# skamann/mcmc-dynamics

Hardware: AMD Instinct MI355X
Metric: star-walker log-L terms/sec (higher is better)
Workload: dtype f64; 1 GPU; C3: 1e6 synthetic stars x 256 walkers, rotation+dispersion + fixed single-Gaussian background mixture (ConstantFit + background.Gaussian), fixed centre; stars_per_gpu=1000000, stars_total=1000000, walkers=256, likelihood=bgfixed, parallelism=1 GPU

## Files before the change

### include/mcd.h

```cpp
#ifndef MCD_H
#define MCD_H

#include <stdint.h>

#ifdef __cplusplus
extern "C" {
#endif

#define MCD_ABI_VERSION 1
#define MCD_UNIQUE_ID_BYTES 128

typedef struct mcd_ctx mcd_ctx;
typedef struct mcd_catalog mcd_catalog;

typedef enum {
    MCD_OK = 0,
    MCD_ERR_INVALID = -1,
    MCD_ERR_HIP = -2,
    MCD_ERR_RCCL = -3,
    MCD_ERR_NO_DEVICE = -4,
    MCD_ERR_NONFINITE = -5,
    MCD_ERR_NOMEM = -6
} mcd_status;

// ... 104 lines not shown
int mcd_stretch_move_seeded(mcd_catalog* cat, const mcd_stretch_desc* desc, int64_t n_steps, double* pos, double* lnp,
                            uint64_t seed, int64_t step0, double* chain, double* lnprob_chain, int64_t* accepted);
int mcd_chain_numbers(uint64_t seed, int64_t step0, int64_t n_steps, int64_t n_bins, int64_t n_walkers, int32_t n_dim,
                      int32_t* order, double* zz, double* thr, int32_t* pick);

int mcd_stretch_info(const mcd_catalog* cat, int64_t* device_blocks, int64_t* host_blocks, int64_t* discarded_blocks,
                     int32_t* last_discard_status);

typedef struct {
    int32_t n_dim;
    const int32_t* kind;
    const double* p0;
    const double* p1;
} mcd_prior_desc;

int mcd_prior_eval(const mcd_prior_desc* prior, int64_t n_rows, const double* x, double* value, double* grad);
int mcd_stretch_move_prior(mcd_catalog* cat, const mcd_stretch_desc* desc, int64_t n_steps, double* pos, double* lnp,
                           const int32_t* order, const double* zz, const double* thr, const int32_t* pick, double* chain,
                           double* lnprob_chain, int64_t* accepted, const mcd_prior_desc* prior);
int mcd_stretch_move_seeded_prior(mcd_catalog* cat, const mcd_stretch_desc* desc, int64_t n_steps, double* pos, double* lnp,
                                  uint64_t seed, int64_t step0, double* chain, double* lnprob_chain, int64_t* accepted,
                                  const mcd_prior_desc* prior);

typedef struct {
    mcd_stretch_desc map;
    const double* chol;
    double step_size;
    double jitter;
    int32_t n_leap;
} mcd_hmc_desc;

int mcd_hmc_block(mcd_catalog* cat, const mcd_hmc_desc* desc, int64_t n_steps, double* pos, double* lnp, uint64_t seed,
                  int64_t step0, double* chain, double* lnprob_chain, int64_t* accepted, double* energy_error);
int mcd_hmc_block_prior(mcd_catalog* cat, const mcd_hmc_desc* desc, int64_t n_steps, double* pos, double* lnp, uint64_t seed,
                        int64_t step0, double* chain, double* lnprob_chain, int64_t* accepted, double* energy_error,
                        const mcd_prior_desc* prior);
int mcd_hmc_numbers(uint64_t seed, int64_t step0, int64_t n_steps, int64_t n_walkers, int32_t n_dim, double* z, double* thr,
                    double* eps_factor);
int mcd_hmc_info(const mcd_catalog* cat, int64_t* device_blocks, int64_t* host_blocks);

typedef struct {
    mcd_stretch_desc map;
    int32_t n_temps;
    const double* betas;
    int32_t n_chain_temps;
} mcd_temper_desc;

int mcd_temper_block(mcd_catalog* cat, const mcd_temper_desc* desc, int64_t n_steps, double* pos, double* lnlike,
                     double* lnprior, uint64_t seed, int64_t step0, double* chain, double* lnlike_chain, int64_t* accepted,
                     int64_t* swap_proposed, int64_t* swap_accepted);
int mcd_temper_block_prior(mcd_catalog* cat, const mcd_temper_desc* desc, int64_t n_steps, double* pos, double* lnlike,
                           double* lnprior, uint64_t seed, int64_t step0, double* chain, double* lnlike_chain,
                           int64_t* accepted, int64_t* swap_proposed, int64_t* swap_accepted,
                           const mcd_prior_desc* prior);
int mcd_temper_numbers(uint64_t seed, int64_t step0, int64_t n_steps, int32_t n_temps, int64_t n_walkers, double* swap_thr);
int mcd_temper_info(const mcd_catalog* cat, int64_t* device_blocks, int64_t* host_blocks);


typedef struct {
    int64_t n_steps, n_groups, n_walkers;
    int32_t n_dim;
    int64_t max_lag;
    double c;
    int64_t scratch_mb;
} mcd_diag_desc;

int mcd_chain_diagnostics(mcd_ctx* ctx, const mcd_diag_desc* d, const double* chain, double* tau, int64_t* window,
                          int32_t* found, double* rhat, double* mean, double* var, double* rho);
int mcd_chain_diagnostics_info(int64_t* tile_groups, int64_t* n_tiles, double* kernel_ms);


const char* mcd_last_error(void);
int mcd_abi_version(void);
double mcd_last_kernel_ms(const mcd_catalog* cat);
double mcd_last_device_ms(const mcd_catalog* cat);
int mcd_set_option(mcd_catalog* cat, const char* key, int64_t value);
int mcd_timing_collect(mcd_catalog* cat, double* total_kernel_ms, int64_t* n_launches);
int64_t mcd_rerun_count(const mcd_catalog* cat);
int mcd_last_prefetch(const mcd_catalog* cat);
int mcd_last_narrow_bounded(const mcd_catalog* cat);
int64_t mcd_last_series_chunks(const mcd_catalog* cat);
int64_t mcd_last_direct_chunks(const mcd_catalog* cat);
int mcd_last_exp_split(const mcd_catalog* cat);
int mcd_last_fast_level(const mcd_catalog* cat);

int mcd_last_f32_domain(const mcd_catalog* cat, double* kappa_v, double* kappa_theta);
int mcd_last_launch_info(const mcd_catalog* cat, int64_t* n_workgroups, int32_t* walker_tile,
                         int64_t* n_chunks, int32_t* record_bytes);

#ifdef __cplusplus
}
#endif
#endif
```

### mcmc_dynamics_amd/_native.py

```python
import atexit
import ctypes
import os
import weakref

import numpy as np

_HERE = os.path.dirname(os.path.abspath(__file__))
LIB_PATH = os.environ.get("MCD_LIB_PATH") or os.path.join(_HERE, "libmcd_hip.so")

MODEL_CONST, MODEL_CONST_BGFIXED, MODEL_CONST_BGGAUSS = 0, 1, 2
MODEL_PROFILE, MODEL_PROFILE_BGGAUSS, MODEL_PROFILE_BGDENS, MODEL_PROFILE_BGFIXED = 3, 4, 5, 6
CENTRE_FIXED, CENTRE_FREE = 0, 1
F64, F32, F32_ACC64 = 0, 1, 2
PRECISIONS = {"f64": F64, "f32": F32, "f32acc64": F32_ACC64}
UNIQUE_ID_BYTES = 128

_c_double_p = ctypes.POINTER(ctypes.c_double)
_c_int64_p = ctypes.POINTER(ctypes.c_int64)

SYMBOLS = {
    "mcd_ctx_create": (ctypes.c_int, [ctypes.c_int, ctypes.POINTER(ctypes.c_int), ctypes.POINTER(ctypes.c_void_p)]),
    "mcd_get_unique_id": (ctypes.c_int, [ctypes.c_void_p]),
    "mcd_ctx_create_rank": (ctypes.c_int, [ctypes.c_int, ctypes.c_int, ctypes.c_int, ctypes.c_void_p,
                                           ctypes.POINTER(ctypes.c_void_p)]),
    "mcd_ctx_destroy": (ctypes.c_int, [ctypes.c_void_p]),
    "mcd_ctx_set_option": (ctypes.c_int, [ctypes.c_void_p, ctypes.c_char_p, ctypes.c_int64]),
    "mcd_ctx_abort": (ctypes.c_int, [ctypes.c_void_p, ctypes.c_char_p]),
    "mcd_ctx_failed": (ctypes.c_int, [ctypes.c_void_p]),
    "mcd_ctx_n_devices": (ctypes.c_int, [ctypes.c_void_p]),
    "mcd_ctx_comm_info": (ctypes.c_int, [ctypes.c_void_p, ctypes.POINTER(ctypes.c_int), ctypes.POINTER(ctypes.c_int),
                                         ctypes.POINTER(ctypes.c_int)]),
    "mcd_catalog_create": (ctypes.c_int, [ctypes.c_void_p, ctypes.c_void_p, ctypes.POINTER(ctypes.c_void_p)]),
    "mcd_catalog_destroy": (ctypes.c_int, [ctypes.c_void_p]),
    "mcd_catalog_param_count": (ctypes.c_int, [ctypes.c_void_p]),
    "mcd_catalog_n_stars": (ctypes.c_int64, [ctypes.c_void_p]),
    "mcd_catalog_n_outputs": (ctypes.c_int64, [ctypes.c_void_p, ctypes.c_int64]),
    "mcd_loglike_batch": (ctypes.c_int, [ctypes.c_void_p, ctypes.c_int64, ctypes.c_int32, _c_double_p, _c_double_p]),
    "mcd_loglike_grad_batch": (ctypes.c_int, [ctypes.c_void_p, ctypes.c_int64, ctypes.c_int32, _c_double_p, _c_double_p,
                                              _c_double_p]),
    "mcd_params_upload": (ctypes.c_int, [ctypes.c_void_p, ctypes.c_int64, ctypes.c_int32, _c_double_p]),
    "mcd_loglike_enqueue": (ctypes.c_int, [ctypes.c_void_p]),
    "mcd_loglike_fetch": (ctypes.c_int, [ctypes.c_void_p, _c_double_p]),
    "mcd_sync": (ctypes.c_int, [ctypes.c_void_p]),
    "mcd_membership": (ctypes.c_int, [ctypes.c_void_p, ctypes.c_int32, _c_double_p, _c_double_p]),
    "mcd_loglike_per_star": (ctypes.c_int, [ctypes.c_void_p, ctypes.c_int32, _c_double_p, _c_double_p]),
    "mcd_pointwise_posterior": (ctypes.c_int, [ctypes.c_void_p, ctypes.c_int64, ctypes.c_int32, _c_double_p, _c_double_p,
                                               _c_double_p, _c_double_p, _c_double_p]),
    "mcd_psis_loo": (ctypes.c_int, [ctypes.c_void_p, ctypes.c_int64, ctypes.c_int32, _c_double_p, ctypes.c_double,
                                    _c_double_p, _c_double_p, _c_double_p, _c_double_p]),
    "mcd_posterior_predictive": (ctypes.c_int, [ctypes.c_void_p, ctypes.c_int64, ctypes.c_int32, _c_double_p, _c_double_p,
                                                _c_double_p]),
    "mcd_kde_background": (ctypes.c_int, [ctypes.c_void_p, ctypes.c_int64, _c_double_p, ctypes.c_int64, _c_double_p,
                                          _c_double_p, ctypes.c_double, _c_double_p, _c_double_p]),
    "mcd_stretch_move": (ctypes.c_int, [ctypes.c_void_p, ctypes.c_void_p, ctypes.c_int64, _c_double_p, _c_double_p,
                                        ctypes.POINTER(ctypes.c_int32), _c_double_p, _c_double_p,
                                        ctypes.POINTER(ctypes.c_int32), _c_double_p, _c_double_p, _c_int64_p]),
    "mcd_stretch_move_seeded": (ctypes.c_int, [ctypes.c_void_p, ctypes.c_void_p, ctypes.c_int64, _c_double_p, _c_double_p,
                                               ctypes.c_uint64, ctypes.c_int64, _c_double_p, _c_double_p, _c_int64_p]),
    "mcd_chain_numbers": (ctypes.c_int, [ctypes.c_uint64, ctypes.c_int64, ctypes.c_int64, ctypes.c_int64, ctypes.c_int64,
                                         ctypes.c_int32, ctypes.POINTER(ctypes.c_int32), _c_double_p, _c_double_p,
                                         ctypes.POINTER(ctypes.c_int32)]),
    "mcd_stretch_info": (ctypes.c_int, [ctypes.c_void_p, _c_int64_p, _c_int64_p, _c_int64_p, ctypes.POINTER(ctypes.c_int32)]),
    "mcd_hmc_block": (ctypes.c_int, [ctypes.c_void_p, ctypes.c_void_p, ctypes.c_int64, _c_double_p, _c_double_p,
                                     ctypes.c_uint64, ctypes.c_int64, _c_double_p, _c_double_p, _c_int64_p, _c_double_p]),
    "mcd_hmc_numbers": (ctypes.c_int, [ctypes.c_uint64, ctypes.c_int64, ctypes.c_int64, ctypes.c_int64, ctypes.c_int32,
                                       _c_double_p, _c_double_p, _c_double_p]),
    "mcd_hmc_info": (ctypes.c_int, [ctypes.c_void_p, _c_int64_p, _c_int64_p]),
    "mcd_prior_eval": (ctypes.c_int, [ctypes.c_void_p, ctypes.c_int64, _c_double_p, _c_double_p, _c_double_p]),
    "mcd_stretch_move_prior": (ctypes.c_int, [ctypes.c_void_p, ctypes.c_void_p, ctypes.c_int64, _c_double_p, _c_double_p,
                                              ctypes.POINTER(ctypes.c_int32), _c_double_p, _c_double_p,
                                              ctypes.POINTER(ctypes.c_int32), _c_double_p, _c_double_p, _c_int64_p,
                                              ctypes.c_void_p]),
    "mcd_stretch_move_seeded_prior": (ctypes.c_int, [ctypes.c_void_p, ctypes.c_void_p, ctypes.c_int64, _c_double_p,
                                                     _c_double_p, ctypes.c_uint64, ctypes.c_int64, _c_double_p, _c_double_p,
                                                     _c_int64_p, ctypes.c_void_p]),
    "mcd_hmc_block_prior": (ctypes.c_int, [ctypes.c_void_p, ctypes.c_void_p, ctypes.c_int64, _c_double_p, _c_double_p,
                                           ctypes.c_uint64, ctypes.c_int64, _c_double_p, _c_double_p, _c_int64_p, _c_double_p,
                                           ctypes.c_void_p]),
    "mcd_temper_block": (ctypes.c_int, [ctypes.c_void_p, ctypes.c_void_p, ctypes.c_int64, _c_double_p, _c_double_p, _c_double_p,
                                        ctypes.c_uint64, ctypes.c_int64, _c_double_p, _c_double_p, _c_int64_p, _c_int64_p,
                                        _c_int64_p]),
    "mcd_temper_block_prior": (ctypes.c_int, [ctypes.c_void_p, ctypes.c_void_p, ctypes.c_int64, _c_double_p, _c_double_p,
                                              _c_double_p, ctypes.c_uint64, ctypes.c_int64, _c_double_p, _c_double_p,
                                              _c_int64_p, _c_int64_p, _c_int64_p, ctypes.c_void_p]),
    "mcd_temper_numbers": (ctypes.c_int, [ctypes.c_uint64, ctypes.c_int64, ctypes.c_int64, ctypes.c_int32, ctypes.c_int64,
                                          _c_double_p]),
    "mcd_temper_info": (ctypes.c_int, [ctypes.c_void_p, _c_int64_p, _c_int64_p]),
    "mcd_chain_diagnostics": (ctypes.c_int, [ctypes.c_void_p, ctypes.c_void_p, _c_double_p, _c_double_p, _c_int64_p,
                                             ctypes.POINTER(ctypes.c_int32), _c_double_p, _c_double_p, _c_double_p,
                                             _c_double_p]),
    "mcd_chain_diagnostics_info": (ctypes.c_int, [_c_int64_p, _c_int64_p, _c_double_p]),
    "mcd_last_error": (ctypes.c_char_p, []),
    "mcd_abi_version": (ctypes.c_int, []),
    "mcd_last_kernel_ms": (ctypes.c_double, [ctypes.c_void_p]),
    "mcd_last_device_ms": (ctypes.c_double, [ctypes.c_void_p]),
    "mcd_timing_collect": (ctypes.c_int, [ctypes.c_void_p, _c_double_p, _c_int64_p]),
    "mcd_rerun_count": (ctypes.c_int64, [ctypes.c_void_p]),
    "mcd_last_prefetch": (ctypes.c_int, [ctypes.c_void_p]),
    "mcd_last_narrow_bounded": (ctypes.c_int, [ctypes.c_void_p]),
    "mcd_last_series_chunks": (ctypes.c_int64, [ctypes.c_void_p]),
    "mcd_last_direct_chunks": (ctypes.c_int64, [ctypes.c_void_p]),
    "mcd_last_exp_split": (ctypes.c_int, [ctypes.c_void_p]),
    "mcd_last_fast_level": (ctypes.c_int, [ctypes.c_void_p]),
    "mcd_last_f32_domain": (ctypes.c_int, [ctypes.c_void_p, _c_double_p, _c_double_p]),
    "mcd_set_option": (ctypes.c_int, [ctypes.c_void_p, ctypes.c_char_p, ctypes.c_int64]),
    "mcd_last_launch_info": (ctypes.c_int, [ctypes.c_void_p, _c_int64_p, ctypes.POINTER(ctypes.c_int32), _c_int64_p,
                                            ctypes.POINTER(ctypes.c_int32)]),
}


class NativeError(RuntimeError):
    """Raised when the HIP library is missing, fails to load, or a call returns an error status."""


class CatalogDesc(ctypes.Structure):
    _fields_ = [
        ("n_stars", ctypes.c_int64),
        ("ra", _c_double_p), ("dec", _c_double_p), ("v", _c_double_p), ("verr", _c_double_p),
        ("lnlike_bg", _c_double_p), ("pmember", _c_double_p), ("density", _c_double_p),
        ("model", ctypes.c_int32), ("centre", ctypes.c_int32), ("precision", ctypes.c_int32),
        ("reserved", ctypes.c_int32),
        ("ra_center", ctypes.c_double), ("dec_center", ctypes.c_double),
        ("n_bins", ctypes.c_int64), ("bin_offsets", _c_int64_p),
    ]


class StretchDesc(ctypes.Structure):
    _fields_ = [
        ("n_walkers", ctypes.c_int64), ("n_dim", ctypes.c_int32), ("k", ctypes.c_int32),
        ("col_source", ctypes.POINTER(ctypes.c_int32)), ("col_const", _c_double_p), ("col_factor", _c_double_p),
        ("lo", _c_double_p), ("hi", _c_double_p), ("fixed_ok", ctypes.c_int32), ("n_bins", ctypes.c_int32),
    ]


class PriorDesc(ctypes.Structure):
    _fields_ = [("n_dim", ctypes.c_int32), ("kind", ctypes.POINTER(ctypes.c_int32)), ("p0", _c_double_p), ("p1", _c_double_p)]


PRIOR_FLAT, PRIOR_NORMAL, PRIOR_LOGNORMAL = 0, 1, 2


def _prior_desc(prior):
    kind = np.ascontiguousarray(prior[0], dtype=np.int32)
    p0, p1 = _f64(prior[1]), _f64(prior[2])
    if kind.ndim != 1 or p0.shape != kind.shape or p1.shape != kind.shape:
        raise ValueError("a prior is three arrays of one length: kind, p0, p1")
    d = PriorDesc()
    d.n_dim = kind.size
    d.kind, d.p0, d.p1 = kind.ctypes.data_as(ctypes.POINTER(ctypes.c_int32)), _ptr(p0), _ptr(p1)
    return d, (kind, p0, p1)


def prior_eval(prior, x, want_grad=False):
    lib = load_library()
    x = _f64(np.atleast_2d(x))
    d, _keep = _prior_desc(prior)
    if x.shape[1] != d.n_dim:
        raise ValueError("prior_eval: x must have shape (n, {0})".format(d.n_dim))
    value = np.empty(x.shape[0])
    grad = np.empty(x.shape) if want_grad else None
    _check(lib, lib.mcd_prior_eval(ctypes.byref(d), x.shape[0], _ptr(x), _ptr(value), _ptr(grad)), "mcd_prior_eval")
    return (value, grad) if want_grad else value


class DiagDesc(ctypes.Structure):
    _fields_ = [("n_steps", ctypes.c_int64), ("n_groups", ctypes.c_int64), ("n_walkers", ctypes.c_int64),
                ("n_dim", ctypes.c_int32), ("max_lag", ctypes.c_int64), ("c", ctypes.c_double), ("scratch_mb", ctypes.c_int64)]


def chain_diagnostics(chain, max_lag, c=5.0, context=None, scratch_mb=0, want_rho=False):
    lib = load_library()
    chain = _f64(chain)
    if chain.ndim != 4:
        raise ValueError("chain_diagnostics: chain must have shape (steps, groups, walkers, parameters)")
    T, G, W, P = chain.shape
    d = DiagDesc(T, G, W, P, int(max_lag), float(c), int(scratch_mb))
    out = {"tau": np.empty((G, P)), "window": np.empty((G, P), dtype=np.int64), "found": np.empty((G, P), dtype=np.int32),
           "rhat": np.empty((G, P)), "mean": np.empty((G, P)), "var": np.empty((G, P))}
    if want_rho:
        out["rho"] = np.empty((G, P, max(int(max_lag), 0) + 1))
    handle = None
    if context is not None:
        handle = getattr(context, "handle", None)
        if not handle:
            raise NativeError("context is closed")
# ... 380 lines not shown
        return out

    def _stretch_args(self, name, plan, pos, lnp, n_steps, chain, lnprob_chain, accepted):
        self._alive()
        for a in (pos, lnp):
            if a.dtype != np.float64 or not a.flags.c_contiguous:
                raise ValueError(name + " needs C-contiguous arrays of the documented dtypes")
        if pos.ndim not in (2, 3) or lnp.shape != pos.shape[:-1]:
            raise ValueError(name + ": inconsistent array shapes")
        lead, (w, p) = pos.shape[:-2], pos.shape[-2:]
        cols = [np.ascontiguousarray(plan["col_source"], dtype=np.int32), _f64(plan["col_const"]), _f64(plan["col_factor"]),
                _f64(plan["lo"]), _f64(plan["hi"])]
        if cols[0].size != self.k or cols[1].size != self.k or cols[2].size != self.k or cols[3].size != p or cols[4].size != p:
            raise ValueError("stretch_move: plan does not match the catalogue / the number of free parameters")
        d = StretchDesc()
        d.n_walkers, d.n_dim, d.k, d.n_bins = w, p, self.k, lead[0] if lead else 1
        d.col_source = cols[0].ctypes.data_as(ctypes.POINTER(ctypes.c_int32))
        d.col_const, d.col_factor, d.lo, d.hi = (_ptr(c) for c in cols[1:])
        d.fixed_ok = 1 if plan.get("fixed_ok", True) else 0
        for a, shape in ((chain, (n_steps,) + lead + (w, p)), (lnprob_chain, (n_steps,) + lead + (w,))):
            if a is not None and (a.dtype != np.float64 or not a.flags.c_contiguous or a.shape != shape):
                raise ValueError("stretch_move: chain buffers must be C-contiguous float64 of shape (steps, [B,] W, P) / (steps, [B,] W)")
        if accepted is not None and (accepted.dtype != np.int64 or accepted.shape != lead + (w,) or not accepted.flags.c_contiguous):
            raise ValueError("stretch_move: accepted must be a C-contiguous int64 array of shape ([B,] W)")
        self._prior_arg = None
        if "prior" in plan:
            pd = None
            if plan["prior"] is not None:
                pd, keep = _prior_desc(plan["prior"])
                cols.append(keep)
            self._prior_arg = (ctypes.byref(pd) if pd is not None else None,)
        return ((self.handle, ctypes.byref(d), n_steps, _ptr(pos), _ptr(lnp)),
                (_ptr(chain), _ptr(lnprob_chain), accepted.ctypes.data_as(_c_int64_p) if accepted is not None else None), cols)

    def stretch_move(self, plan, pos, lnp, order, zz, thr, pick, chain=None, lnprob_chain=None, accepted=None):
        head, tail, _keep = self._stretch_args("stretch_move", plan, pos, lnp, order.shape[0], chain, lnprob_chain, accepted)
        for a, dt in ((zz, np.float64), (thr, np.float64), (order, np.int32), (pick, np.int32)):
            if a.dtype != dt or not a.flags.c_contiguous:
                raise ValueError("stretch_move needs C-contiguous arrays of the documented dtypes")
        half_shape = (order.shape[0], 2) + pos.shape[:-2] + (pos.shape[-2] // 2,)
        if order.shape != order.shape[:1] + lnp.shape or zz.shape != half_shape or thr.shape != half_shape or \
                pick.shape != half_shape:
            raise ValueError("stretch_move: inconsistent array shapes")
        numbers = (order.ctypes.data_as(ctypes.POINTER(ctypes.c_int32)), _ptr(zz), _ptr(thr),
                   pick.ctypes.data_as(ctypes.POINTER(ctypes.c_int32)))
        if self._prior_arg is not None:
            rc = self.lib.mcd_stretch_move_prior(*head, *numbers, *tail, *self._prior_arg)
        else:
            rc = self.lib.mcd_stretch_move(*head, *numbers, *tail)
        _check(self.lib, rc, "mcd_stretch_move")
        self._walkers = pos.shape[-2] // 2

    def stretch_move_seeded(self, plan, pos, lnp, seed, step0, n_steps, chain=None, lnprob_chain=None, accepted=None):
        if n_steps < 0 or step0 < 0:
            raise ValueError("stretch_move_seeded: inconsistent array shapes")
        head, tail, _keep = self._stretch_args("stretch_move_seeded", plan, pos, lnp, n_steps, chain, lnprob_chain, accepted)
        if self._prior_arg is not None:
            rc = self.lib.mcd_stretch_move_seeded_prior(*head, int(seed) & 0xFFFFFFFFFFFFFFFF, int(step0), *tail, *self._prior_arg)
        else:
            rc = self.lib.mcd_stretch_move_seeded(*head, int(seed) & 0xFFFFFFFFFFFFFFFF, int(step0), *tail)
        _check(self.lib, rc, "mcd_stretch_move_seeded")
        self._walkers = pos.shape[-2] // 2

    @property
    def last_prefetch(self):
        return self.lib.mcd_last_prefetch(self.handle)

    @property
    def last_narrow_bounded(self):
        return self.lib.mcd_last_narrow_bounded(self.handle)

    @property
    def last_series_chunks(self):
        return self.lib.mcd_last_series_chunks(self.handle)

    @property
    def last_direct_chunks(self):
        return self.lib.mcd_last_direct_chunks(self.handle)

    @property
    def last_exp_split(self):
        return self.lib.mcd_last_exp_split(self.handle)

    def hmc_block(self, plan, chol, step_size, n_leap, pos, lnp, seed, step0, n_steps, chain=None, lnprob_chain=None,
                  accepted=None, energy_error=None, jitter=0.1):
        if n_steps < 0 or step0 < 0 or pos.ndim != 2:
            raise ValueError("hmc_block: inconsistent array shapes")
        head, tail, _keep = self._stretch_args("hmc_block", plan, pos, lnp, n_steps, chain, lnprob_chain, accepted)
        chol = np.ascontiguousarray(chol, dtype=np.float64)
        if chol.shape != (pos.shape[1], pos.shape[1]):
            raise ValueError("hmc_block: chol must have shape (P, P)")
        if energy_error is not None and (energy_error.dtype != np.float64 or not energy_error.flags.c_contiguous or
                                         energy_error.shape != (n_steps, pos.shape[0])):
            raise ValueError("hmc_block: energy_error must be a C-contiguous float64 array of shape (steps, W)")
        d = HmcDesc()
        d.map = head[1]._obj
        d.chol, d.step_size, d.jitter, d.n_leap = _ptr(chol), float(step_size), float(jitter), int(n_leap)
        if self._prior_arg is not None:
            rc = self.lib.mcd_hmc_block_prior(self.handle, ctypes.byref(d), int(n_steps), head[3], head[4],
                                              int(seed) & 0xFFFFFFFFFFFFFFFF, int(step0), *tail, _ptr(energy_error),
                                              *self._prior_arg)
        else:
            rc = self.lib.mcd_hmc_block(self.handle, ctypes.byref(d), int(n_steps), head[3], head[4],
                                        int(seed) & 0xFFFFFFFFFFFFFFFF, int(step0), *tail, _ptr(energy_error))
        _check(self.lib, rc, "mcd_hmc_block")

    def hmc_info(self):
        a, b = ctypes.c_int64(), ctypes.c_int64()
        _check(self.lib, self.lib.mcd_hmc_info(self.handle, ctypes.byref(a), ctypes.byref(b)), "mcd_hmc_info")
        return {"device_blocks": a.value, "host_blocks": b.value}

    def temper_block(self, plan, betas, pos, lnlike, lnprior, seed, step0, n_steps, chain=None, lnlike_chain=None,
                     accepted=None, swap_proposed=None, swap_accepted=None):
        if n_steps < 0 or step0 < 0 or pos.ndim != 3 or lnlike.shape != pos.shape[:2] or lnprior.shape != pos.shape[:2]:
            raise ValueError("temper_block: inconsistent array shapes")
        t, w, p = pos.shape
        betas = _f64(betas)
        if betas.shape != (t,):
            raise ValueError("temper_block: betas must have one entry per rung")
        if lnprior.dtype != np.float64 or not lnprior.flags.c_contiguous or not pos.flags.c_contiguous or \
                not lnlike.flags.c_contiguous:
            raise ValueError("temper_block needs C-contiguous arrays of the documented dtypes")
        head, _tail, _keep = self._stretch_args("temper_block", plan, pos[0], lnlike[0], n_steps, None, None, None)
        n_chain = 1
        if chain is not None:
            if chain.dtype != np.float64 or not chain.flags.c_contiguous or chain.ndim != 4 or \
                    chain.shape[0] != n_steps or chain.shape[2:] != (w, p):
                raise ValueError("temper_block: chain must be a C-contiguous float64 array of shape (steps, C, W, P)")
            n_chain = chain.shape[1]
        if lnlike_chain is not None and (lnlike_chain.dtype != np.float64 or not lnlike_chain.flags.c_contiguous or
                                         lnlike_chain.shape != (n_steps, t, w)):
            raise ValueError("temper_block: lnlike_chain must be a C-contiguous float64 array of shape (steps, T, W)")
        for a, shape in ((accepted, (t, w)), (swap_proposed, (t - 1,)), (swap_accepted, (t - 1,))):
            if a is not None and (a.dtype != np.int64 or a.shape != shape or not a.flags.c_contiguous):
                raise ValueError("temper_block: accepted (T, W) and the swap counts (T - 1,) are C-contiguous int64 arrays")
        d = TemperDesc()
        d.map = head[1]._obj
        d.n_temps, d.betas, d.n_chain_temps = t, _ptr(betas), n_chain

        def ip(a):
            return a.ctypes.data_as(_c_int64_p) if a is not None else None
        args = (self.handle, ctypes.byref(d), int(n_steps), _ptr(pos), _ptr(lnlike), _ptr(lnprior),
                int(seed) & 0xFFFFFFFFFFFFFFFF, int(step0), _ptr(chain), _ptr(lnlike_chain), ip(accepted), ip(swap_proposed),
                ip(swap_accepted))
        if self._prior_arg is not None:
            rc = self.lib.mcd_temper_block_prior(*args, *self._prior_arg)
        else:
            rc = self.lib.mcd_temper_block(*args)
        _check(self.lib, rc, "mcd_temper_block")
        self._walkers = t * (w // 2)

    def temper_info(self):
        a, b = ctypes.c_int64(), ctypes.c_int64()
        _check(self.lib, self.lib.mcd_temper_info(self.handle, ctypes.byref(a), ctypes.byref(b)), "mcd_temper_info")
        return {"device_blocks": a.value, "host_blocks": b.value}

    def stretch_info(self):
        a, b, c, st = ctypes.c_int64(), ctypes.c_int64(), ctypes.c_int64(), ctypes.c_int32()
        _check(self.lib, self.lib.mcd_stretch_info(self.handle, ctypes.byref(a), ctypes.byref(b), ctypes.byref(c), ctypes.byref(st)),
               "mcd_stretch_info")
        return {"device_blocks": a.value, "host_blocks": b.value, "discarded_blocks": c.value, "last_discard_status": st.value}

    def set_option(self, key, value):
        _check(self.lib, self.lib.mcd_set_option(self.handle, key.encode(), int(value)), "mcd_set_option")
        self.__dict__.setdefault("_options", {})[key] = int(value)

    def get_option(self, key, default=None):
        return self.__dict__.get("_options", {}).get(key, default)

    @property
    def last_kernel_ms(self):
        return self.lib.mcd_last_kernel_ms(self.handle)

    @property
    def last_device_ms(self):
        return self.lib.mcd_last_device_ms(self.handle)

    def timing_collect(self):
        total, n = ctypes.c_double(), ctypes.c_int64()
        _check(self.lib, self.lib.mcd_timing_collect(self.handle, ctypes.byref(total), ctypes.byref(n)),
               "mcd_timing_collect")
        return total.value, n.value

    @property
    def rerun_count(self):
        return self.lib.mcd_rerun_count(self.handle)

    @property
    def fast_level(self):
        return self.lib.mcd_last_fast_level(self.handle)

    @property
    def f32_in_domain(self):
        return bool(self.lib.mcd_last_f32_domain(self.handle, None, None))

    @property
    def f32_condition(self):
        kv, kt = ctypes.c_double(), ctypes.c_double()
        self.lib.mcd_last_f32_domain(self.handle, ctypes.byref(kv), ctypes.byref(kt))
        return kv.value, kt.value

    def launch_info(self):
        wg, ch = ctypes.c_int64(), ctypes.c_int64()
        tile, rb = ctypes.c_int32(), ctypes.c_int32()
        _check(self.lib, self.lib.mcd_last_launch_info(self.handle, ctypes.byref(wg), ctypes.byref(tile),
                                                       ctypes.byref(ch), ctypes.byref(rb)), "mcd_last_launch_info")
        return {"workgroups": wg.value, "walker_tile": tile.value, "chunks": ch.value, "record_bytes": rb.value,
                "series_chunks": self.last_series_chunks, "direct_chunks": self.last_direct_chunks,
                "exp_split": self.last_exp_split}

    def close(self):
        if getattr(self, "handle", None):
            self.lib.mcd_catalog_destroy(self.handle)
            self.handle = None

    def __del__(self):
        try:
            self.close()
        except Exception:
            pass
```

### mcmc_dynamics_amd/csrc/mcd_api_catalog.hip

```cpp
#include "mcd_host.h"

using namespace mcd::host;

namespace {

int param_count(int model, bool free_centre) {
    int k = (mcd::is_profile(model) ? 6 : 4) + (free_centre ? 2 : 0);
    const int bg = mcd::bg_kind(model);
    if (bg == mcd::BG_GAUSS) k += 3;
    if (bg == mcd::BG_FIXED_DENSITY) k += 1;
    return k;
}

void free_workset(WorkSet& w) {
    if (w.d_chunks) (void)hipFree(w.d_chunks);
    if (w.d_offsets) (void)hipFree(w.d_offsets);
    if (w.d_chunk_general) (void)hipFree(w.d_chunk_general);
    if (w.d_split_const) (void)hipFree(w.d_split_const);
    if (w.d_params) (void)hipFree(w.d_params);
    if (w.d_wpar) (void)hipFree(w.d_wpar);
    if (w.d_partials) (void)hipFree(w.d_partials);
    if (w.d_out) (void)hipFree(w.d_out);
    if (w.d_out2) (void)hipFree(w.d_out2);
    if (w.d_partials2) (void)hipFree(w.d_partials2);
// ... 17 lines not shown
int balance_auto_m(const mcd_catalog* cat, int64_t n, int64_t n_walkers) {
    const int64_t n_wtiles = (n_walkers + 63) / 64;
    const double tiles = n_wtiles <= 4 ? (double)n_wtiles : 4.0 * (double)((n_wtiles + 3) / 4);
    const double work = (double)n * tiles / 4.0 * model_cost(cat->model, cat->free_centre);
    const double limit = mcd::bg_kind(cat->model) == mcd::BG_NONE ? 9.0e5 : 1.3e6;
    if (cat->n_psets != 1 || work > limit) return 0;
    return work < 6.0e4 ? 2 : (work <= 3.4e5 ? 4 : 8);
}

bool wants_prefetch(const mcd_catalog* cat, const Shard& sh) {
    if (cat->prefetch >= 0) return cat->prefetch != 0;
    const size_t bytes = (size_t)sh.n * (size_t)mcd::record_bytes(cat->model, cat->free_centre, cat->precision);
    if (mcd::bg_kind(cat->model) == mcd::BG_NONE) return cat->n_psets == 1 && bytes >= ((size_t)128 << 20);
    return bytes >= ((size_t)8 << 20);
}

bool wants_sorted(const mcd_catalog* cat, const Shard& sh) {
    if (cat->model != mcd::MODEL_BGFIXED || cat->free_centre || cat->precision != MCD_F64 || cat->n_psets != 1 || sh.n <= 0)
        return false;
    if (cat->verr_sorted >= 0) return cat->verr_sorted != 0;
    if (cat->chunk_len > 0) return false;
    return (size_t)sh.n * (size_t)mcd::record_bytes(cat->model, cat->free_centre, cat->precision) >= ((size_t)8 << 20);
}

int ensure_sorted_records(mcd_catalog* cat, Shard& sh) {
    if (sh.records_sorted) return MCD_OK;
    const DeviceSlot& slot = cat->ctx->slots[sh.slot];
    constexpr int ND = mcd::record_doubles(mcd::MODEL_BGFIXED, false);
    const size_t n = (size_t)sh.n, bytes = n * ND * sizeof(double);
    MCD_HIP(hipStreamSynchronize(slot.stream));
    std::vector<double> rec(n * ND), out(n * ND);
    MCD_HIP(hipMemcpy(rec.data(), sh.records, bytes, hipMemcpyDeviceToHost));
    const std::vector<int64_t> perm = mcd::verr_order(rec.data(), (int64_t)n, ND);
    sh.sorted_e2.resize(n);
    for (size_t i = 0; i < n; ++i) {
        std::memcpy(&out[i * ND], &rec[(size_t)perm[i] * ND], ND * sizeof(double));
        sh.sorted_e2[i] = out[i * ND + 1];
    }
    sh.sorted_exceptions = mcd::permuted_exceptions(cat->stats.narrow_exceptions, perm, sh.star_begin);
    sh.sorted_nbf.resize(n);
    mcd::exp_split_records(out.data(), (int64_t)n, rec.data(), sh.sorted_nbf.data());
    void* d[2] = {nullptr, nullptr};
    const double* src[2] = {out.data(), rec.data()};
    for (int a = 0; a < 2; ++a) {
        hipError_t e = hipMalloc(&d[a], bytes + 2048);
        if (e == hipSuccess) e = hipMemset(d[a], 0, bytes + 2048);
        if (e == hipSuccess) e = hipMemcpy(d[a], src[a], bytes, hipMemcpyHostToDevice);
        if (e != hipSuccess) {
            for (int b = 0; b <= a; ++b)
                if (d[b]) (void)hipFree(d[b]);
            MCD_HIP(e);
        }
    }
    sh.records_sorted = d[0];
    sh.records_split = d[1];
    return MCD_OK;
}

struct Option {
    const char* key;
    int64_t min, max;
    const char* message;
    bool sync, replan;
    void (*set)(mcd_catalog* c, int64_t v);
    bool (*accepts)(int64_t v) = nullptr;
};
constexpr int64_t kMin = std::numeric_limits<int64_t>::min(), kMax = std::numeric_limits<int64_t>::max();
#define MCD_SET(statement) [](mcd_catalog* c, int64_t v) { statement; }
const Option kOptions[] = {
    {"fast_path", 0, 2, "fast_path: 0 (plain), 1 (guarded, default) or 2 (guarded, no narrow variant)", false, false, MCD_SET(c->allow_fast = (int)v)},
    {"zero_copy", kMin, kMax, nullptr, false, false, MCD_SET(c->zero_copy = v != 0)},
    {"device_chain", 0, 2, "device_chain: 0 (host-driven blocks), 1 (default) or 2 (as 1 with the general step kernel, testing aid)", false, false,
     MCD_SET(c->device_chain = (int)v; c->chain_backoff = 0; c->chain_consecutive = 0; c->chain_hint = -1)},
    {"fused_reduce", kMin, kMax, nullptr, false, false, MCD_SET(c->fused_reduce = v != 0)},
    {"defer_guard", kMin, kMax, nullptr, false, false, MCD_SET(c->defer_guard = v != 0)},
    {"f32_domain", kMin, kMax, nullptr, false, false, MCD_SET(c->f32_domain = v != 0)},
    {"loo_scratch_mb", 1, kMax, "loo_scratch_mb must be >= 1", false, false, MCD_SET(c->loo_scratch_mb = v)},
    {"posterior_pass", 1, kMax, "posterior_pass must be >= 1", false, false, MCD_SET(c->posterior_pass = v)},
    {"two_lanes", kMin, kMax, nullptr, true, false, MCD_SET(c->two_lanes = v != 0)},
    {"narrow_bounded", 0, 1, "narrow_bounded: 1 (where the guard admits it, default) or 0 (never)", false, false, MCD_SET(c->narrow_bounded = (int)v)},
    {"verr_sorted", -1, 1, "verr_sorted: -1 (by record volume, default), 0 (catalogue order) or 1 (sorted by verr)", true, true, MCD_SET(c->verr_sorted = (int)v)},
    {"root_series", 0, 1, "root_series: 1 (series root on the narrow chunks of verr-sorted records, default) or 0 (never)", false, false, MCD_SET(c->root_series = (int)v)},
    {"exp_split", 0, 1, "exp_split: 1 (split exponent offset in the direct chunks where the guard admits it, default) or 0 (never)", false, false, MCD_SET(c->exp_split = (int)v)},
    {"root_direct", 0, 1, "root_direct: 1 (direct form of the series root where a chunk admits it, default) or 0 (delta form only)", false, false, MCD_SET(c->root_direct = (int)v)},
    {"prefetch", -1, 1, "prefetch: -1 (by record volume, default), 0 (off) or 1 (on)", false, false, MCD_SET(c->prefetch = (int)v)},
    {"spin_us", 0, kMax, "spin_us must be >= 0", false, false, MCD_SET(c->spin_us = v)},
    {"tail_split", kMin, kMax, nullptr, true, true, MCD_SET(c->tail_split = (int)v)},
    {"target_waves", 1, kMax, "target_waves must be positive", true, true, MCD_SET(c->target_waves = v)},
    {"chunk_len", 0, kMax, "chunk_len must be >= 0", true, true, MCD_SET(c->chunk_len = v)},
    {"balance", -1, 8, "balance: -1 (auto), 0 (off) or 1 .. 8 workgroups per CU", true, true, MCD_SET(c->balance = (int)v)},
    {"combine", 0, 16, "combine: 0 (never), 1 (largest workgroup the plan allows), 8 or 16 (waves per workgroup at most)", true, true,
     MCD_SET(c->combine = (int)v), [](int64_t v) { return v <= 1 || v == 8 || v == 16; }},
};
#undef MCD_SET
}

MCD_HOST_BEGIN

LaunchShape main_launch_shape(mcd_catalog* cat, const Shard& sh, const WorkSet& w, int level, bool coll, double* out_buf,
                              int64_t n_out) {
    LaunchShape shape{cat->model, cat->free_centre, cat->precision, level, w.uniform_len, sh.n};
    shape.uniform_extra = w.uniform_extra;
    shape.waves = w.waves;
    shape.chunk_general = w.d_chunk_general;
    shape.prefetch = wants_prefetch(cat, sh);
    cat->last_prefetch = shape.prefetch && shape.fast != 0;
    shape.rerun_flag = coll ? nullptr : out_buf + n_out;
    shape.root_series = w.sorted && cat->root_series != 0;
    shape.root_direct = shape.root_series && cat->root_direct != 0;
    return shape;
}

const void* main_records(const Shard& sh, const WorkSet& w) { return w.sorted ? sh.records_sorted : sh.records; }

int64_t series_chunk_count(const mcd_catalog* cat, const WorkSet& w, int level, const double* params, int64_t n_rows) {
    if (!w.sorted || !cat->root_series || level != 2 || w.series_need.empty()) return 0;
    const mcd::ParamRanges pr = mcd::table_ranges(cat->model, cat->free_centre, cat->k, params, n_rows);
    if (!pr.finite) return 0;
    return (int64_t)(std::upper_bound(w.series_need.begin(), w.series_need.end(), pr.s2_min) - w.series_need.begin());
}

int64_t direct_chunk_count(const mcd_catalog* cat, const WorkSet& w, int level, const double* params, int64_t n_rows) {
    if (!w.sorted || !cat->root_series || !cat->root_direct || level != 2 || w.direct_need.empty()) return 0;
    const mcd::ParamRanges pr = mcd::table_ranges(cat->model, cat->free_centre, cat->k, params, n_rows);
    if (!pr.finite) return 0;
    return (int64_t)(std::upper_bound(w.direct_need.begin(), w.direct_need.end(), pr.s2_min) - w.direct_need.begin());
}

const double* fast_pset_const(const mcd_catalog* cat, const Shard& sh, int level) {
    const int bgk = mcd::bg_kind(cat->model);
    return (level && (bgk == mcd::BG_FIXED || bgk == mcd::BG_FIXED_DENSITY)) ? sh.d_pset_const : nullptr;
}

int build_workset(mcd_catalog* cat, Shard& sh, int64_t n_walkers, WorkSet** out) {
    auto it = sh.work.find(n_walkers);
    if (it != sh.work.end()) { *out = &it->second; return MCD_OK; }
    if (sh.work.size() >= 8) {
        for (auto& kv : sh.work) free_workset(kv.second);
        sh.work.clear();
        cat->cur_walkers = 0;
    }
    const DeviceSlot& slot = cat->ctx->slots[sh.slot];
    MCD_HIP(hipSetDevice(slot.device));

    const bool sorted = wants_sorted(cat, sh);
    if (sorted)
        if (int rc = ensure_sorted_records(cat, sh)) return rc;
    const std::vector<int64_t>& exceptions = sorted ? sh.sorted_exceptions : cat->stats.narrow_exceptions;
    mcd::ChunkPlan plan;
    for (int m = cat->balance < 0 ? balance_auto_m(cat, sh.n, n_walkers) : cat->balance;; m /= 2) {
        plan = mcd::plan_chunks(cat->bin_offsets, sh.star_begin, sh.n, n_walkers, cat->target_waves, cat->tail_split,
                                exceptions, cat->chunk_len, m);
        if (m == 0 || plan.balanced_m > 0) break;
    }
    const std::vector<mcd::Chunk>& chunks = plan.chunks;
    const std::vector<int64_t>& offs = plan.offsets;
    const std::vector<uint8_t>& general = plan.general;

    WorkSet w;
    w.n_walkers = n_walkers;
    w.n_chunks = (int64_t)chunks.size();
    w.max_chunks_per_pset = plan.max_chunks_per_pset;
    w.uniform_len = plan.uniform_len;
    w.uniform_extra = plan.uniform_extra;
    w.sorted = sorted;
    if (sorted) {
        w.series_need = mcd::series_thresholds(plan, sh.sorted_e2.data());
        w.direct_need = mcd::direct_thresholds(plan, sh.sorted_e2.data());
    }
    const std::vector<double> split_const = sorted ? mcd::exp_split_chunk_consts(plan, sh.sorted_nbf.data()) : std::vector<double>();
    {
        const int64_t n_wtiles = (n_walkers + 63) / 64;
        const bool shape_ok = plan.balanced_m > 0 && plan.balanced_m % 2 == 0 && (n_wtiles == 1 || n_wtiles == 2 || n_wtiles == 4) &&
                              cat->precision == MCD_F64;
        w.waves = 4;
        if (cat->combine != 0 && shape_ok) {
            const bool can16 = mcd::bg_kind(cat->model) != mcd::BG_GAUSS;
            w.waves = 8;
            if (cat->combine == 16 && plan.balanced_m % 4 == 0 && can16) w.waves = 16;
            if (cat->combine == 1 && plan.balanced_m == 4 && can16) w.waves = 16;
        }
    }
    const int64_t n_out = cat->n_psets * n_walkers;
    const size_t term_bytes = cat->precision == MCD_F64 ? 8 : 4;
    auto allocate = [&]() -> hipError_t {
        hipError_t e;
        if (!general.empty()) {
            if ((e = hipMalloc(&w.d_chunk_general, general.size())) != hipSuccess) return e;
            if ((e = hipMemcpy(w.d_chunk_general, general.data(), general.size(), hipMemcpyHostToDevice)) != hipSuccess) return e;
        }
        if (!split_const.empty()) {
            if ((e = hipMalloc(&w.d_split_const, split_const.size() * sizeof(double))) != hipSuccess) return e;
            if ((e = hipMemcpy(w.d_split_const, split_const.data(), split_const.size() * sizeof(double), hipMemcpyHostToDevice)) != hipSuccess) return e;
        }
        if ((e = hipMalloc(&w.d_chunks, std::max<size_t>(1, chunks.size()) * sizeof(mcd::Chunk))) != hipSuccess) return e;
        if ((e = hipMalloc(&w.d_offsets, offs.size() * sizeof(int64_t))) != hipSuccess) return e;
        if ((e = hipMalloc(&w.d_params, (size_t)n_out * cat->k * sizeof(double))) != hipSuccess) return e;
        if ((e = hipMalloc(&w.d_wpar, (size_t)n_out * mcd::KD * term_bytes)) != hipSuccess) return e;
        if ((e = hipMalloc(&w.d_partials, std::max<size_t>(1, (size_t)mcd::padded_walkers(n_walkers) * w.n_chunks) * sizeof(double))) != hipSuccess) return e;
        if ((e = hipMalloc(&w.d_out, (size_t)(n_out + 1) * sizeof(double))) != hipSuccess) return e;
        if ((e = hipMemset(w.d_out, 0, (size_t)(n_out + 1) * sizeof(double))) != hipSuccess) return e;
        if ((e = hipMalloc(&w.d_out2, (size_t)(n_out + 1) * sizeof(double))) != hipSuccess) return e;
        if ((e = hipMemset(w.d_out2, 0, (size_t)(n_out + 1) * sizeof(double))) != hipSuccess) return e;
        if ((e = hipEventCreateWithFlags(&w.ev_staged, hipEventDisableTiming)) != hipSuccess) return e;
        for (int b = 0; b < 2; ++b) {
            if ((e = hipEventCreateWithFlags(&w.ev_reduced[b], hipEventDisableTiming)) != hipSuccess) return e;
            if ((e = hipEventCreateWithFlags(&w.ev_comm[b], hipEventDisableTiming)) != hipSuccess) return e;
        }
        if ((e = hipHostMalloc(&w.h_params, (size_t)n_out * cat->k * sizeof(double), hipHostMallocMapped)) != hipSuccess) return e;
        if ((e = hipHostMalloc(&w.h_out, (size_t)(n_out + 1) * sizeof(double), hipHostMallocMapped)) != hipSuccess) return e;
        std::memset(w.h_out, 0, (size_t)(n_out + 1) * sizeof(double));
        if ((e = hipHostGetDevicePointer((void**)&w.m_params, w.h_params, 0)) != hipSuccess) return e;
        if ((e = hipHostGetDevicePointer((void**)&w.m_out, w.h_out, 0)) != hipSuccess) return e;
        if (!chunks.empty() &&
            (e = hipMemcpy(w.d_chunks, chunks.data(), chunks.size() * sizeof(mcd::Chunk), hipMemcpyHostToDevice)) != hipSuccess)
            return e;
        return hipMemcpy(w.d_offsets, offs.data(), offs.size() * sizeof(int64_t), hipMemcpyHostToDevice);
    };
    const hipError_t err = allocate();
    if (err != hipSuccess) {
        free_workset(w);
        return fail(MCD_ERR_HIP, std::string("work buffers for this walker count: ") + hipGetErrorString(err));
    }
    auto ins = sh.work.emplace(n_walkers, w);
    *out = &ins.first->second;
    return MCD_OK;
}

MCD_HOST_END

extern "C" {

static int catalog_create_impl(mcd_ctx* ctx, const mcd_catalog_desc* d, std::unique_ptr<mcd_catalog>& cat);

int mcd_catalog_create(mcd_ctx* ctx, const mcd_catalog_desc* d, mcd_catalog** out) {
    try {
    if (!ctx || !d || !out) return fail(MCD_ERR_INVALID, "mcd_catalog_create: null argument");
    std::unique_ptr<mcd_catalog> cat;
    const int rc = catalog_create_impl(ctx, d, cat);
    if (rc != MCD_OK) {
        if (cat) {
            const std::string msg = g_last_error;
            mcd_catalog_destroy(cat.release());
            g_last_error = msg;
        }
        return rc;
    }
    *out = cat.release();
    return MCD_OK;
    } catch (...) { return on_exception("mcd_catalog_create"); }
}

static int catalog_create_impl(mcd_ctx* ctx, const mcd_catalog_desc* d, std::unique_ptr<mcd_catalog>& cat) {
// ... 136 lines not shown
        cat->timing_launches = 0;
        return MCD_OK;
    }
    if (!std::strcmp(key, "timing_stride")) {
        if (value < 1) return fail(MCD_ERR_INVALID, "timing_stride must be >= 1");
        int rc = sync_all(cat);
        if (rc != MCD_OK) return rc;
        cat->timing_stride = value;
        cat->timing_launches = 0;
        return MCD_OK;
    }
    if (!std::strcmp(key, "timing_reserve")) {
        if (value < 0 || value > ((int64_t)1 << 16)) return fail(MCD_ERR_INVALID, "timing_reserve: 0 .. 65536 launches");
        for (Shard& sh : cat->shards) {
            MCD_HIP(hipSetDevice(cat->ctx->slots[sh.slot].device));
            while ((int64_t)sh.ring.size() < value) {
                hipEvent_t a, b;
                MCD_HIP(hipEventCreate(&a));
                if (hipEventCreate(&b) != hipSuccess) { (void)hipEventDestroy(a); return fail(MCD_ERR_HIP, "hipEventCreate"); }
                sh.ring.emplace_back(a, b);
            }
        }
        return MCD_OK;
    }
    for (const Option& o : kOptions) {
        if (std::strcmp(key, o.key)) continue;
        if (value < o.min || value > o.max || (o.accepts && !o.accepts(value))) return fail(MCD_ERR_INVALID, o.message);
        if (o.sync)
            if (int rc = sync_all(cat)) return rc;
        o.set(cat, value);
        if (o.replan) {
            for (Shard& sh : cat->shards) {
                (void)hipSetDevice(cat->ctx->slots[sh.slot].device);
                for (auto& kv : sh.work) free_workset(kv.second);
                sh.work.clear();
            }
            cat->cur_walkers = 0;
        }
        return MCD_OK;
    }
    return fail(MCD_ERR_INVALID, std::string("unknown option: ") + key);
    } catch (...) { return on_exception("mcd_set_option"); }
}

int mcd_timing_collect(mcd_catalog* cat, double* total_kernel_ms, int64_t* n_launches) {
    try {
    if (!cat) return fail(MCD_ERR_INVALID, "null catalogue");
    int rc = sync_all(cat);
    if (rc != MCD_OK) return rc;
    Shard& sh = cat->shards[0];
    double total = 0.0;
    for (size_t i = 0; i < sh.ring_used; ++i) {
        float ms = 0.f;
        MCD_HIP(hipEventElapsedTime(&ms, sh.ring[i].first, sh.ring[i].second));
        total += ms;
    }
    if (total_kernel_ms) *total_kernel_ms = total;
    if (n_launches) *n_launches = (int64_t)sh.ring_used;
    for (Shard& s2 : cat->shards) s2.ring_used = 0;
    cat->timing_launches = 0;
    return MCD_OK;
    } catch (...) { return on_exception("mcd_timing_collect"); }
}

int64_t mcd_rerun_count(const mcd_catalog* cat) { return cat ? cat->n_reruns : MCD_ERR_INVALID; }

int mcd_stretch_info(const mcd_catalog* cat, int64_t* device_blocks, int64_t* host_blocks, int64_t* discarded_blocks,
                     int32_t* last_discard_status) {
    if (!cat) return fail(MCD_ERR_INVALID, "null catalogue");
    if (device_blocks) *device_blocks = cat->chain_device_blocks;
    if (host_blocks) *host_blocks = cat->chain_host_blocks;
    if (discarded_blocks) *discarded_blocks = cat->chain_discarded;
    if (last_discard_status) *last_discard_status = cat->chain_last_status;
    return MCD_OK;
}

int mcd_last_prefetch(const mcd_catalog* cat) { return cat ? cat->last_prefetch : -1; }

int64_t mcd_last_series_chunks(const mcd_catalog* cat) { return cat ? cat->last_series_chunks : -1; }
int64_t mcd_last_direct_chunks(const mcd_catalog* cat) { return cat ? cat->last_direct_chunks : -1; }

int mcd_last_narrow_bounded(const mcd_catalog* cat) { return cat ? cat->last_narrow_bounded : -1; }
int mcd_last_exp_split(const mcd_catalog* cat) { return cat ? cat->last_exp_split : -1; }

int mcd_last_f32_domain(const mcd_catalog* cat, double* kappa_v, double* kappa_theta) {
    if (!cat) return -1;
    if (kappa_v) *kappa_v = cat->last_f32.kappa_v;
    if (kappa_theta) *kappa_theta = cat->last_f32.kappa_theta;
    if (cat->precision == MCD_F64) return 1;
    return cat->last_f32.inside ? 1 : 0;
}

int mcd_last_fast_level(const mcd_catalog* cat) {
    if (!cat || cat->cur_walkers <= 0 || cat->shards.empty()) return -1;
    const auto it = cat->shards.front().work.find(cat->cur_walkers);
    return it == cat->shards.front().work.end() ? -1 : it->second.fast;
}

double mcd_last_kernel_ms(const mcd_catalog* cat) { return cat ? cat->last_kernel_ms : -1.0; }
double mcd_last_device_ms(const mcd_catalog* cat) { return cat ? cat->last_device_ms : -1.0; }

int mcd_last_launch_info(const mcd_catalog* cat, int64_t* n_workgroups, int32_t* walker_tile, int64_t* n_chunks,
                         int32_t* record_bytes) {
    if (!cat) return fail(MCD_ERR_INVALID, "null catalogue");
    if (n_workgroups) *n_workgroups = cat->last_grid;
    if (walker_tile) *walker_tile = 64;
    if (n_chunks) *n_chunks = cat->last_chunks;
    if (record_bytes) *record_bytes = mcd::record_bytes(cat->model, cat->free_centre, cat->precision);
    return MCD_OK;
}

}
```

### mcmc_dynamics_amd/csrc/mcd_api_chain.hip

```cpp
#include "mcd_host.h"
#include "mcd_prior.h"
#include "mcd_rng.h"
#include "mcd_stretch.h"
#include "mcd_grad.h"
#include "mcd_hmc.h"

using namespace mcd::host;

MCD_HOST_BEGIN

int prior_of(const mcd_prior_desc* p, int32_t n_dim, const char* who, PriorHost& out) {
    out.table = mcd::PriorTable();
    if (!p) return MCD_OK;
    if (p->n_dim != n_dim) return fail(MCD_ERR_INVALID, std::string(who) + ": the prior's n_dim differs from the descriptor's");
    if (n_dim < 1 || !p->kind || !p->p0 || !p->p1) return fail(MCD_ERR_INVALID, std::string(who) + ": null prior array");
    out.kind.assign(p->kind, p->kind + n_dim);
    out.loc.resize((size_t)n_dim); out.scale.resize((size_t)n_dim); out.c0.resize((size_t)n_dim);
    bool structured = false;
    if (!mcd::prior_derive(n_dim, p->kind, p->p0, p->p1, out.loc.data(), out.scale.data(), out.c0.data(), &structured))
        return fail(MCD_ERR_INVALID, std::string(who) + ": prior kinds are 0 (flat), 1 (normal: loc, scale > 0) or 2 (lognormal: mu, s > 0) with finite parameters");
    if (structured) {
        out.table.kind = out.kind.data(); out.table.loc = out.loc.data(); out.table.scale = out.scale.data(); out.table.c0 = out.c0.data();
    }
    return MCD_OK;
// ... 121 lines not shown
    std::memset(a.h + o_status, 0, 8);
    std::memcpy(a.h + o_src, d->col_source, (size_t)K * 4);
    std::memcpy(a.h + o_const, d->col_const, (size_t)K * 8);
    std::memcpy(a.h + o_fac, d->col_factor, (size_t)K * 8);
    std::memcpy(a.h + o_lo, d->lo, (size_t)P * 8);
    std::memcpy(a.h + o_hi, d->hi, (size_t)P * 8);
    if (with_prior) {
        std::memcpy(a.h + o_pkind, prior.kind, (size_t)P * 4);
        std::memcpy(a.h + o_ploc, prior.loc, (size_t)P * 8);
        std::memcpy(a.h + o_pscale, prior.scale, (size_t)P * 8);
        std::memcpy(a.h + o_pc0, prior.c0, (size_t)P * 8);
    }
    const size_t moved = (size_t)n_steps * BW * ((gen_device ? 0 : 24) + (chain ? (size_t)P * 8 : 0) + (lnprob_chain ? 8 : 0));
    size_t part_threshold = (size_t)16 << 20;
    if (const char* e = std::getenv("MCD_CHAIN_PART_BYTES")) part_threshold = (size_t)std::strtoull(e, nullptr, 10);
    int64_t max_parts = 16;
    if (const char* e = std::getenv("MCD_CHAIN_PARTS")) max_parts = std::max<long long>(1, std::atoll(e));
    const int64_t n_parts = moved >= part_threshold ? std::min<int64_t>(max_parts, n_steps) : 1;
    auto part_begin = [&](int64_t k) { return n_steps * k / n_parts; };
    auto copy_in = [&](int64_t i0, int64_t i1) {
        if (gen_device) return;
        const size_t at = (size_t)i0 * BW, n = (size_t)(i1 - i0) * BW;
        if (seeded) {
            std::vector<uint64_t> sorter;
            for (int64_t i = i0; i < i1; ++i)
                mcd::chain_numbers_of_step(*seed, step0 + i, B, W, P, (int32_t*)(a.h + o_order) + (size_t)i * BW,
                                           (double*)(a.h + o_zz) + (size_t)i * BW, (double*)(a.h + o_thr) + (size_t)i * BW,
                                           (int32_t*)(a.h + o_pick) + (size_t)i * BW, sorter);
            return;
        }
        big_copy(a.h + o_order + at * 4, order + at, n * 4);
        big_copy(a.h + o_zz + at * 8, zz + at, n * 8);
        big_copy(a.h + o_thr + at * 8, thr + at, n * 8);
        big_copy(a.h + o_pick + at * 4, pick + at, n * 4);
    };
    if (n_parts == 1) copy_in(0, n_steps);

    int level = cat->chain_hint;
    if (level < 0) {
        std::vector<double> table(BW * K);
        for (size_t j = 0; j < BW; ++j)
            for (int c = 0; c < K; ++c) {
                const int src = d->col_source[c];
                table[j * K + c] = src < 0 ? d->col_const[c]
                                           : (d->col_factor[c] == 1.0 ? pos[j * P + src] : pos[j * P + src] * d->col_factor[c]);
            }
        level = fast_level(cat, table.data(), (int64_t)BW);
    }

    mcd::StretchDevice sd;
    sd.n_bins = B;
    sd.n_walkers = W; sd.n_dim = P; sd.k = K; sd.fixed_ok = d->fixed_ok;
    sd.model = cat->model; sd.free_centre = cat->free_centre ? 1 : 0; sd.allow_fast = cat->allow_fast;
    sd.expected_level = level;
    sd.force_general = cat->device_chain == 2;
    sd.stats = cat->stats;
    sd.col_source = (const int32_t*)(a.d + o_src); sd.col_const = (const double*)(a.d + o_const);
    sd.col_factor = (const double*)(a.d + o_fac); sd.lo = (const double*)(a.d + o_lo); sd.hi = (const double*)(a.d + o_hi);
    sd.pos = (double*)(a.d + o_pos); sd.lnp = (double*)(a.d + o_lnp); sd.accepted = (long long*)(a.d + o_acc);
    sd.order = (const int32_t*)(a.d + o_order); sd.zz = (const double*)(a.d + o_zz); sd.thr = (const double*)(a.d + o_thr);
    sd.pick = (const int32_t*)(a.d + o_pick);
    sd.chain = chain ? (double*)(a.d + o_chain) : nullptr;
    sd.lnprob_chain = lnprob_chain ? (double*)(a.d + o_lnpc) : nullptr;
    sd.proposal = (double*)(a.d + o_prop); sd.ok = (uint8_t*)(a.d + o_ok); sd.meta = (int32_t*)(a.d + o_meta);
    sd.n_ok = (int32_t*)(a.d + o_nok); sd.ranges = (double*)(a.d + o_ranges);
    sd.table = w.d_params; sd.wpar = (double*)w.d_wpar;
    if (with_prior) {
        sd.prior.kind = (const int32_t*)(a.d + o_pkind); sd.prior.loc = (const double*)(a.d + o_ploc);
        sd.prior.scale = (const double*)(a.d + o_pscale); sd.prior.c0 = (const double*)(a.d + o_pc0);
        sd.prior_val = (double*)(a.d + o_pval);
    }
    if (defer) {
        sd.defer_guard = 1;
        sd.table_log = (double*)(a.d + o_table_log); sd.n_ok_log = (int32_t*)(a.d + o_nok_log); sd.level_log = (int32_t*)(a.d + o_levels);
    }

    const bool coll = ctx->n_ranks > 1 || ctx->force_collective;
    double* const out_buf = w.d_out;
    mcd::LaunchShape shape = main_launch_shape(cat, sh, w, level, coll, out_buf, (int64_t)Bh);
    cat->last_narrow_bounded = 0;
    cat->last_series_chunks = 0;
    cat->last_direct_chunks = 0;
    cat->last_exp_split = 0;
    const double* pset_const = fast_pset_const(cat, sh, level);
    const int64_t n_slots = mcd::partial_slots(shape, w.n_chunks, half);
    const int64_t max_slots = B == 1 ? n_slots : w.max_chunks_per_pset;
    const bool fused = cat->fused_reduce != 0 && !coll && max_slots <= mcd::kFusedReduceSlots && mcd::stretch_step_fuses(sd);
    sd.fused = fused ? 1 : 0;
    sd.partials = w.d_partials;
    sd.n_slots = n_slots;
    sd.slot_offsets = B == 1 ? nullptr : w.d_offsets;
    sd.pset_const = pset_const;
    cat->chain_last_fused = fused;
    double prev_tag = 0.0;
    int64_t acc_step = -1;
    int acc_h = 0;
#ifdef MCD_CHAIN_STAMPS
    static unsigned long long* d_stamps = nullptr;
    if (!d_stamps) MCD_HIP(hipMalloc((void**)&d_stamps, 8 * 8 * 4096));
    MCD_HIP(hipMemsetAsync(d_stamps, 0, 8 * 8 * 4096, slot.stream));
    sd.stamps = d_stamps;
#endif
    auto enqueue_steps = [&](int64_t i0, int64_t i1, hipEvent_t mark) -> int {
        for (int64_t i = i0; i < i1; ++i)
            for (int h = 0; h < 2; ++h) {
#ifdef MCD_CHAIN_STAMPS
                sd.launch_index = i * 2 + h;
#endif
                MCD_HIP(mcd::launch_stretch_step(slot.stream, sd, acc_step, acc_h, i, h, out_buf, prev_tag));
                if (mark && i == i0 && h == 0) MCD_HIP(hipEventRecord(mark, slot.stream));
                prev_tag = coll ? 0.0 : (double)(++cat->launch_seq);
                shape.launch_tag = prev_tag;
                MCD_HIP(mcd::launch_loglike(slot.stream, shape, main_records(sh, w), w.d_chunks, w.n_chunks, w.d_wpar, w.d_partials, half));
                if (!fused)
                    MCD_HIP(mcd::launch_reduce(slot.stream, w.d_partials, w.d_offsets, B, n_slots, max_slots, half, pset_const,
                                               out_buf));
                if (coll) {
                    if (!ctx->multi_process) MCD_NCCL(g_rccl.GroupStart());
                    MCD_NCCL(g_rccl.AllReduce(out_buf, out_buf, Bh, ncclDouble, ncclSum, slot.comm, slot.stream));
                    if (!ctx->multi_process) MCD_NCCL(g_rccl.GroupEnd());
                }
                acc_step = i;
                acc_h = h;
            }
        return MCD_OK;
    };
    auto finish = [&]() -> int {
        MCD_HIP(mcd::launch_stretch_step(slot.stream, sd, acc_step, acc_h, -1, 0, out_buf, prev_tag));
        if (defer) MCD_HIP(mcd::launch_stretch_judge(slot.stream, sd, (int64_t)n_launches));
        if (coll) {
            double* status = (double*)(a.d + o_status);
            MCD_HIP(mcd::launch_stretch_status(slot.stream, sd.meta, status));
            if (!ctx->multi_process) MCD_NCCL(g_rccl.GroupStart());
            MCD_NCCL(g_rccl.AllReduce(status, status, 1, ncclDouble, ncclSum, slot.comm, slot.stream));
            if (!ctx->multi_process) MCD_NCCL(g_rccl.GroupEnd());
        }
        return MCD_OK;
    };
    struct MidBlockGuard {
        mcd_ctx* ctx; bool armed; bool ok;
        ~MidBlockGuard() {
            if (armed && !ok && !ctx->failed.load()) {
                const std::string cause = g_last_error;
                (void)ctx_fail(ctx, "mcd_stretch_move: this rank failed in the middle of a resident block (" + cause + ")");
            }
        }
    } mid_block{ctx, coll, false};
    bool rows_delivered = false;
    auto generate = [&](hipStream_t s, int64_t i0, int64_t i1) {
        return mcd::launch_chain_numbers(s, *seed, step0, i0, i1, B, W, P, (int32_t*)(a.d + o_order), (double*)(a.d + o_zz),
                                         (double*)(a.d + o_thr), (int32_t*)(a.d + o_pick));
    };
    if (n_parts == 1) {
        MCD_HIP(hipMemcpyAsync(a.d, a.h, gen_device ? o_order : input_end, hipMemcpyHostToDevice, slot.stream));
        if (gen_device) MCD_HIP(generate(slot.stream, 0, n_steps));
        rc = enqueue_steps(0, n_steps, nullptr);
        if (rc != MCD_OK) return rc;
        rc = finish();
        if (rc != MCD_OK) return rc;
        MCD_HIP(hipMemcpyAsync(a.h, a.d, state_end, hipMemcpyDeviceToHost, slot.stream));
        if (total > o_chain)
            MCD_HIP(hipMemcpyAsync(a.h + o_chain, a.d + o_chain, total - o_chain, hipMemcpyDeviceToHost, slot.stream));
        MCD_WAIT(cat->ctx, slot.stream, cat->spin_us, "mcd_stretch_move (resident block)");
    } else {
        while ((int64_t)cat->chain_events.size() < 3 * n_parts) {
            hipEvent_t e;
// ... 466 lines not shown
```

### mcmc_dynamics_amd/csrc/mcd_api_eval.hip

```cpp
#include "mcd_host.h"
#include "mcd_grad.h"

using namespace mcd::host;

MCD_HOST_BEGIN

int fast_level(const mcd_catalog* cat, const double* params, int64_t n_rows) {
    if (!cat->allow_fast) return 0;
    const int level = mcd::fast_level(cat->stats, cat->model, cat->free_centre, cat->precision != MCD_F64, cat->k, params, n_rows);
    return cat->allow_fast == 2 && level > 1 ? 1 : level;
}

int sync_all(mcd_catalog* cat) {
    if (!cat) return fail(MCD_ERR_INVALID, "null catalogue");
    if (int rc = ctx_usable(cat->ctx)) return rc;
    for (Shard& sh : cat->shards) {
        const DeviceSlot& slot = cat->ctx->slots[sh.slot];
        MCD_HIP(hipSetDevice(slot.device));
        MCD_WAIT(cat->ctx, slot.stream, cat->spin_us, "mcd_sync / mcd_loglike_fetch (compute stream)");
        MCD_WAIT(cat->ctx, slot.stream2, cat->spin_us, "mcd_sync / mcd_loglike_fetch (second compute lane)");
        MCD_WAIT(cat->ctx, slot.comm_stream, cat->spin_us, "mcd_sync / mcd_loglike_fetch (communication stream)");
    }
    if (cat->timing && cat->timing_pending) {
        Shard& sh = cat->shards[0];
        float k_ms = 0.f, d_ms = 0.f;
        if (cat->timing_all) {
            if (sh.ring_used > 0)
                MCD_HIP(hipEventElapsedTime(&k_ms, sh.ring[sh.ring_used - 1].first, sh.ring[sh.ring_used - 1].second));
        } else {
            MCD_HIP(hipEventElapsedTime(&k_ms, sh.ev_k0, sh.ev_k1));
        }
        if (!cat->timing_all) MCD_HIP(hipEventElapsedTime(&d_ms, sh.ev_begin, sh.ev_end));
        cat->last_kernel_ms = k_ms;
        cat->last_device_ms = cat->timing_all ? -1.0 : d_ms;
        cat->timing_pending = false;
    }
    return MCD_OK;
}

MCD_HOST_END

namespace {

WorkSet* find_work(Shard& sh, int64_t W) {
    const auto it = sh.work.find(W);
    return it == sh.work.end() ? nullptr : &it->second;
}

bool all_staged(mcd_catalog* cat) {
    if (cat->cur_walkers <= 0) return false;
    for (Shard& sh : cat->shards) {
        const WorkSet* w = find_work(sh, cat->cur_walkers);
        if (!w || !w->staged) return false;
    }
    return true;
}

int stage_params_impl(mcd_catalog* cat, int64_t n_walkers, int32_t k, const double* params, bool zero_copy) {
    if (!cat || !params) return fail(MCD_ERR_INVALID, "null catalogue or params");
    if (int rc = ctx_usable(cat->ctx)) return rc;
    if (n_walkers <= 0) return fail(MCD_ERR_INVALID, "n_walkers must be positive");
    if (k != cat->k) {
        char buf[128];
        snprintf(buf, sizeof buf, "parameter table has %d columns, catalogue expects %d", (int)k, cat->k);
        return fail(MCD_ERR_INVALID, buf);
    }
    const int64_t n_rows = cat->n_psets * n_walkers;
    if (cat->precision != MCD_F64) {
        cat->last_f32 = mcd::f32_domain(cat->stats, cat->model, cat->free_centre, cat->k, params, n_rows);
        if (!cat->last_f32.inside && cat->f32_domain)
            return fail(MCD_ERR_INVALID, std::string("outside the float32 accuracy domain (use an MCD_F64 catalogue, or option "
                                                     "f32_domain = 0 to evaluate regardless): ") + cat->last_f32.reason);
    }
    const int fast = fast_level(cat, params, n_rows);
    const int narrow_rescale = fast == 2 && cat->precision == MCD_F64
                                   ? mcd::bounded_rescale(cat->stats, cat->model, cat->free_centre, cat->k, params, n_rows) : 0;
    for (Shard& sh : cat->shards) {
        WorkSet* w = nullptr;
        int rc = build_workset(cat, sh, n_walkers, &w);
        if (rc != MCD_OK) return rc;
        const DeviceSlot& slot = cat->ctx->slots[sh.slot];
        MCD_HIP(hipSetDevice(slot.device));
        MCD_WAIT(cat->ctx, slot.stream, cat->spin_us, "mcd_params_upload (previous evaluation)");
        if (w->lane1_used) {
            MCD_WAIT(cat->ctx, slot.stream2, cat->spin_us, "mcd_params_upload (previous evaluation, second lane)");
            w->lane1_used = false;
        }
        std::memcpy(w->h_params, params, (size_t)n_rows * k * sizeof(double));
        w->mapped = zero_copy;
        const double* src = w->m_params;
        if (!zero_copy) {
            MCD_HIP(hipMemcpyAsync(w->d_params, w->h_params, (size_t)n_rows * k * sizeof(double), hipMemcpyHostToDevice,
                                   slot.stream));
            src = w->d_params;
        }
        MCD_HIP(mcd::launch_prepare_walkers(slot.stream, src, n_rows, k, cat->model, cat->free_centre,
                                            cat->precision, w->d_wpar));
        MCD_HIP(hipEventRecord(w->ev_staged, slot.stream));
        w->lane1_knows_staging = false;
        w->fast = fast;
        w->narrow_rescale = narrow_rescale;
        for (int b = 0; b < 2; ++b)
            w->exp_split[b] = fast == 2 && cat->precision == MCD_F64 && (b == 0 || narrow_rescale != 0) &&
                              mcd::exp_split_admitted(cat->stats, cat->model, cat->free_centre, cat->k, params, n_rows,
                                                      b ? narrow_rescale : 0);
        w->series_chunks = series_chunk_count(cat, *w, fast, params, n_rows);
        w->direct_chunks = direct_chunk_count(cat, *w, fast, params, n_rows);
        w->staged = true;
    }
    cat->cur_walkers = n_walkers;
    return MCD_OK;
}

int stage_params(mcd_catalog* cat, int64_t n_walkers, int32_t k, const double* params, bool zero_copy) {
    const int rc = stage_params_impl(cat, n_walkers, k, params, zero_copy);
    if (rc != MCD_OK && cat) cat->cur_walkers = 0;
    return rc;
}

int timing_pair(const mcd_catalog* cat, Shard& sh, bool sampled, hipEvent_t* k0, hipEvent_t* k1) {
    *k0 = sh.ev_k0;
    *k1 = sh.ev_k1;
    if (!(cat->timing_all && sampled)) return MCD_OK;
    if (sh.ring_used >= (size_t)1 << 16) sh.ring_used = 0;
    if (sh.ring_used == sh.ring.size()) {
        hipEvent_t a, b;
        MCD_HIP(hipEventCreate(&a));
        MCD_HIP(hipEventCreate(&b));
        sh.ring.emplace_back(a, b);
    }
    *k0 = sh.ring[sh.ring_used].first;
    *k1 = sh.ring[sh.ring_used].second;
    ++sh.ring_used;
    return MCD_OK;
}

int timing_end(mcd_catalog* cat) {
    if (cat->timing_all) ++cat->timing_launches;
    if (!cat->timing) return MCD_OK;
    if (!cat->timing_all) {
        for (Shard& sh : cat->shards) {
            const DeviceSlot& slot = cat->ctx->slots[sh.slot];
            MCD_HIP(hipSetDevice(slot.device));
            MCD_HIP(hipEventRecord(sh.ev_end, slot.stream));
        }
    }
    cat->timing_pending = true;
    return MCD_OK;
}

int enqueue(mcd_catalog* cat, bool pipelined) {
    if (!cat) return fail(MCD_ERR_INVALID, "null catalogue");
    if (int rc = ctx_usable(cat->ctx)) return rc;
    if (cat->cur_walkers <= 0) return fail(MCD_ERR_INVALID, "no parameters staged (call mcd_params_upload first)");
    if (!all_staged(cat)) return fail(MCD_ERR_INVALID, "no parameters staged for this walker count (the last upload failed?)");
    const int64_t W = cat->cur_walkers;
    const int64_t n_out = cat->n_psets * W;
    mcd_ctx* ctx = cat->ctx;
    for (Shard& sh : cat->shards) {
        WorkSet& w = (*find_work(sh, W));
        const DeviceSlot& slot = ctx->slots[sh.slot];
        MCD_HIP(hipSetDevice(slot.device));
        const bool coll = ctx->has_comm();
        double* out_buf = w.mapped ? w.m_out : w.d_out;
        const bool two_lanes = pipelined && cat->two_lanes && !(cat->timing && !cat->timing_all);
        hipStream_t lane_stream = slot.stream;
        double* lane_partials = w.d_partials;
        if (coll || two_lanes) {
            w.buf ^= 1;
            out_buf = w.buf ? w.d_out2 : w.d_out;
            if (two_lanes && w.buf) {
                if (!w.d_partials2) {
                    MCD_HIP(hipMalloc(&w.d_partials2, std::max<size_t>(1, (size_t)mcd::padded_walkers(W) * w.n_chunks) * sizeof(double)));
                }
                if (!w.lane1_knows_staging) {
                    MCD_HIP(hipStreamWaitEvent(slot.stream2, w.ev_staged, 0));
                    w.lane1_knows_staging = true;
                }
                lane_stream = slot.stream2;
                lane_partials = w.d_partials2;
                w.lane1_used = true;
            }
        } else {
            w.buf = 0;
        }
        mcd::LaunchShape shape = main_launch_shape(cat, sh, w, w.fast, coll, out_buf, n_out);
        shape.narrow_rescale = cat->narrow_bounded ? w.narrow_rescale : 0;
        cat->last_narrow_bounded = mcd::narrow_bounded_launch(shape) ? shape.narrow_rescale : 0;
        if (cat->exp_split && w.sorted && w.d_split_const && w.exp_split[cat->last_narrow_bounded ? 1 : 0]) {
            shape.records_split = sh.records_split;
            shape.split_const = w.d_split_const;
        }
        cat->last_exp_split = mcd::exp_split_launch(shape) ? 1 : 0;
        if (&sh == &cat->shards.front()) cat->last_series_chunks = cat->last_direct_chunks = 0;
        cat->last_series_chunks += shape.root_series && shape.fast == 2 ? w.series_chunks : 0;
        cat->last_direct_chunks += shape.root_direct && shape.fast == 2 ? w.direct_chunks : 0;
        w.launch_tag = coll ? 0.0 : (double)(++cat->launch_seq);
        shape.launch_tag = w.launch_tag;
        const bool sampled = !cat->timing_all || (cat->timing_launches % cat->timing_stride) == 0;
        hipEvent_t k0, k1;
        if (int rc = timing_pair(cat, sh, sampled, &k0, &k1)) return rc;
        if (cat->timing && !cat->timing_all) MCD_HIP(hipEventRecord(sh.ev_begin, slot.stream));
        if (cat->timing && sampled) MCD_HIP(hipEventRecord(k0, lane_stream));
        MCD_HIP(mcd::launch_loglike(lane_stream, shape, main_records(sh, w), w.d_chunks, w.n_chunks, w.d_wpar, lane_partials, W));
        if (cat->timing && sampled) MCD_HIP(hipEventRecord(k1, lane_stream));
        const double* pset_const = fast_pset_const(cat, sh, w.fast);
        if (coll && w.comm_pending[w.buf]) {
            MCD_HIP(hipStreamWaitEvent(lane_stream, w.ev_comm[w.buf], 0));
            w.comm_pending[w.buf] = false;
        }
        {
            const int64_t n_slots = mcd::partial_slots(shape, w.n_chunks, W);
            MCD_HIP(mcd::launch_reduce(lane_stream, lane_partials, w.d_offsets, cat->n_psets, n_slots,
                                       cat->n_psets == 1 ? n_slots : w.max_chunks_per_pset, W, pset_const, out_buf));
        }
        if (coll && pipelined) MCD_HIP(hipEventRecord(w.ev_reduced[w.buf], lane_stream));
    }
    if (ctx->has_comm()) {
        if (!ctx->multi_process) MCD_NCCL(g_rccl.GroupStart());
        for (Shard& sh : cat->shards) {
            WorkSet& w = (*find_work(sh, W));
            const DeviceSlot& slot = ctx->slots[sh.slot];
            MCD_HIP(hipSetDevice(slot.device));
            double* buf = w.buf ? w.d_out2 : w.d_out;
            if (pipelined) {
                MCD_HIP(hipStreamWaitEvent(slot.comm_stream, w.ev_reduced[w.buf], 0));
                MCD_NCCL(g_rccl.AllReduce(buf, buf, (size_t)n_out, ncclDouble, ncclSum, slot.comm, slot.comm_stream));
            } else {
                if (w.comm_pending[w.buf ^ 1]) {
                    MCD_HIP(hipStreamWaitEvent(slot.stream, w.ev_comm[w.buf ^ 1], 0));
                    w.comm_pending[w.buf ^ 1] = false;
                }
                MCD_NCCL(g_rccl.AllReduce(buf, buf, (size_t)n_out, ncclDouble, ncclSum, slot.comm, slot.stream));
            }
        }
        if (!ctx->multi_process) MCD_NCCL(g_rccl.GroupEnd());
        if (pipelined) {
            for (Shard& sh : cat->shards) {
                WorkSet& w = (*find_work(sh, W));
                const DeviceSlot& slot = ctx->slots[sh.slot];
                MCD_HIP(hipSetDevice(slot.device));
                MCD_HIP(hipEventRecord(w.ev_comm[w.buf], slot.comm_stream));
                w.comm_pending[w.buf] = true;
            }
        }
    }
    if (int rc = timing_end(cat)) return rc;
    {
        WorkSet& w0 = (*find_work(cat->shards[0], W));
        cat->last_chunks = w0.n_chunks;
        mcd::LaunchShape sh0{cat->model, cat->free_centre, cat->precision, w0.fast};
        sh0.waves = w0.waves;
        const int64_t slots = mcd::partial_slots(sh0, w0.n_chunks, W);
        cat->last_grid = slots != w0.n_chunks ? slots : mcd::main_grid(w0.n_chunks, W);
    }
    return MCD_OK;
}

int fetch_once(mcd_catalog* cat, bool* rerun) {
    const int64_t W = cat->cur_walkers;
    const int64_t n_out = cat->n_psets * W;
    *rerun = false;
    const bool coll = cat->ctx->has_comm();
    bool any_fast = false;
    for (Shard& sh : cat->shards) {
        WorkSet& w = (*find_work(sh, W));
        any_fast = any_fast || w.fast != 0;
        const DeviceSlot& slot = cat->ctx->slots[sh.slot];
        MCD_HIP(hipSetDevice(slot.device));
        if (!w.mapped && &sh == &cat->shards[0]) {
            const double* res = w.buf ? w.d_out2 : w.d_out;
            if (w.comm_pending[w.buf]) MCD_HIP(hipStreamWaitEvent(slot.stream, w.ev_comm[w.buf], 0));
            hipStream_t copy_stream = (!coll && w.buf && w.lane1_used) ? slot.stream2 : slot.stream;
            MCD_HIP(hipMemcpyAsync(w.h_out, res, (size_t)(n_out + 1) * sizeof(double), hipMemcpyDeviceToHost, copy_stream));
        }
    }
    int rc = sync_all(cat);
// ... 172 lines not shown
```

### mcmc_dynamics_amd/csrc/mcd_api_temper.hip

```cpp
#include "mcd_host.h"
#include "mcd_prior.h"
#include "mcd_rng.h"
#include "mcd_temper.h"

using namespace mcd::host;

namespace {

constexpr size_t kTemperResidentMaxBytes = (size_t)512 << 20;

size_t temper_block_bytes(int64_t T, int64_t W, int P, int64_t n_steps, int32_t n_chain_temps, bool chain, bool lnlike_chain) {
    return (size_t)n_steps * ((size_t)T * W * 24 + (chain ? (size_t)n_chain_temps * W * P * 8 : 0) + (lnlike_chain ? (size_t)T * W * 8 : 0));
}

bool temper_resident_covers(const mcd_catalog* cat, int64_t T, int64_t W, int P, int64_t n_steps, int32_t n_chain_temps,
                            bool chain, bool lnlike_chain) {
    if (!cat->device_chain || cat->shards.size() != 1 || cat->ctx->has_comm() || cat->timing || n_steps < 1) return false;
    if (!mcd::chain_numbers_on_device(W)) return false;
    return temper_block_bytes(T, W, P, n_steps, n_chain_temps, chain, lnlike_chain) <= kTemperResidentMaxBytes;
}

int temper_block_device(mcd_catalog* cat, const mcd::TemperShared& ts, int64_t n_steps, double* pos, double* ll, double* lp,
                        uint64_t seed, int64_t step0, int32_t n_chain_temps, double* chain, double* lnlike_chain,
                        int64_t* accepted, int64_t* swap_proposed, int64_t* swap_accepted, bool* done) {
// ... 42 lines not shown
        a = ChainArena();
        const size_t want = total + total / 2;
        if (hipMalloc((void**)&a.d, want) != hipSuccess) { (void)hipGetLastError(); a = ChainArena(); return MCD_OK; }
        if (hipHostMalloc((void**)&a.h, want, hipHostMallocDefault) != hipSuccess) {
            (void)hipGetLastError();
            (void)hipFree(a.d);
            a = ChainArena();
            return MCD_OK;
        }
        a.bytes = want;
    }
    std::memcpy(a.h + o_pos, pos, TW * P * 8);
    std::memcpy(a.h + o_ll, ll, TW * 8);
    std::memcpy(a.h + o_lp, lp0.data(), TW * 8);
    std::memset(a.h + o_acc, 0, TW * 8);
    std::memset(a.h + o_swap, 0, TW * 8);
    std::memset(a.h + o_status, 0, 8);
    std::memcpy(a.h + o_src, ts.col_source, (size_t)K * 4);
    std::memcpy(a.h + o_const, ts.col_const, (size_t)K * 8);
    std::memcpy(a.h + o_fac, ts.col_factor, (size_t)K * 8);
    std::memcpy(a.h + o_lo, ts.lo, (size_t)P * 8);
    std::memcpy(a.h + o_hi, ts.hi, (size_t)P * 8);
    std::memcpy(a.h + o_betas, ts.betas, (size_t)T * 8);
    if (with_prior) {
        std::memcpy(a.h + o_pkind, ts.prior.kind, (size_t)P * 4);
        std::memcpy(a.h + o_ploc, ts.prior.loc, (size_t)P * 8);
        std::memcpy(a.h + o_pscale, ts.prior.scale, (size_t)P * 8);
        std::memcpy(a.h + o_pc0, ts.prior.c0, (size_t)P * 8);
    }

    mcd::TemperDevice td;
    td.s = ts;
    td.s.col_source = (const int32_t*)(a.d + o_src); td.s.col_const = (const double*)(a.d + o_const);
    td.s.col_factor = (const double*)(a.d + o_fac); td.s.lo = (const double*)(a.d + o_lo); td.s.hi = (const double*)(a.d + o_hi);
    td.s.betas = (const double*)(a.d + o_betas);
    if (with_prior) {
        td.s.prior.kind = (const int32_t*)(a.d + o_pkind); td.s.prior.loc = (const double*)(a.d + o_ploc);
        td.s.prior.scale = (const double*)(a.d + o_pscale); td.s.prior.c0 = (const double*)(a.d + o_pc0);
    }
    td.seed = seed;
    td.pos = (double*)(a.d + o_pos); td.ll = (double*)(a.d + o_ll); td.lp = (double*)(a.d + o_lp);
    td.accepted = (long long*)(a.d + o_acc); td.swap_accepted = (long long*)(a.d + o_swap); td.status = (int32_t*)(a.d + o_status);
    td.order = (const int32_t*)(a.d + o_order); td.zz = (const double*)(a.d + o_zz); td.thr = (const double*)(a.d + o_thr);
    td.pick = (const int32_t*)(a.d + o_pick);
    td.proposal = (double*)(a.d + o_prop); td.ok = (uint8_t*)(a.d + o_ok); td.lp_new = (double*)(a.d + o_lpn);
    td.table = w.d_params;
    td.out = w.d_out;
    td.chain = chain ? (double*)(a.d + o_chain) : nullptr;
    td.lnlike_chain = lnlike_chain ? (double*)(a.d + o_llc) : nullptr;
    td.n_chain_temps = n_chain_temps;

    w.staged = false;
    mcd::LaunchShape shape = main_launch_shape(cat, sh, w, 0, false, w.d_out, rows);
    const int64_t n_slots = mcd::partial_slots(shape, w.n_chunks, rows);
    MCD_HIP(hipMemcpyAsync(a.d, a.h, input_end, hipMemcpyHostToDevice, slot.stream));
    MCD_HIP(mcd::launch_chain_numbers(slot.stream, seed, step0, 0, n_steps, T, W, P, (int32_t*)(a.d + o_order),
                                      (double*)(a.d + o_zz), (double*)(a.d + o_thr), (int32_t*)(a.d + o_pick)));
    auto evaluate = [&]() -> int {
        MCD_HIP(mcd::launch_prepare_walkers(slot.stream, w.d_params, rows, K, cat->model, cat->free_centre, cat->precision, w.d_wpar));
        MCD_HIP(mcd::launch_loglike(slot.stream, shape, main_records(sh, w), w.d_chunks, w.n_chunks, w.d_wpar, w.d_partials, rows));
        MCD_HIP(mcd::launch_reduce(slot.stream, w.d_partials, w.d_offsets, 1, n_slots, n_slots, rows, nullptr, w.d_out));
        return MCD_OK;
    };
    for (int64_t i = 0; i < n_steps; ++i) {
        MCD_HIP(mcd::launch_temper_step(slot.stream, td, -1, 0, i, 0));
        if ((rc = evaluate()) != MCD_OK) return rc;
        MCD_HIP(mcd::launch_temper_step(slot.stream, td, i, 0, i, 1));
        if ((rc = evaluate()) != MCD_OK) return rc;
        MCD_HIP(mcd::launch_temper_step(slot.stream, td, i, 1, -1, 0));
        MCD_HIP(mcd::launch_temper_swap(slot.stream, td, step0 + i, i));
    }
    MCD_HIP(hipMemcpyAsync(a.h, a.d, state_end, hipMemcpyDeviceToHost, slot.stream));
    if (total > o_rows) MCD_HIP(hipMemcpyAsync(a.h + o_rows, a.d + o_rows, total - o_rows, hipMemcpyDeviceToHost, slot.stream));
    MCD_WAIT(cat->ctx, slot.stream, cat->spin_us, "mcd_temper_block (resident block)");

    w.fast = 0;
    cat->cur_walkers = rows;
    cat->last_chunks = w.n_chunks;
    cat->last_grid = n_slots != w.n_chunks ? n_slots : mcd::main_grid(w.n_chunks, rows);
    cat->last_narrow_bounded = 0;
    cat->last_series_chunks = 0;
    cat->last_direct_chunks = 0;
    cat->last_exp_split = 0;
    if (*(const int32_t*)(a.h + o_status) != 0)
        return fail(MCD_ERR_NONFINITE, "mcd_temper_block: the log-likelihood returned NaN");
    ++cat->temper_device_blocks;
    std::memcpy(pos, a.h + o_pos, TW * P * 8);
    std::memcpy(ll, a.h + o_ll, TW * 8);
    std::memcpy(lp, a.h + o_lp, TW * 8);
    const int64_t* acc = (const int64_t*)(a.h + o_acc);
    if (accepted) for (size_t x = 0; x < TW; ++x) accepted[x] += acc[x];
    const int64_t* sw = (const int64_t*)(a.h + o_swap);
    for (int64_t t = 0; t + 1 < T; ++t) {
        if (swap_proposed) swap_proposed[t] += mcd::temper_swaps_proposed(step0, n_steps, t, T, W);
        if (!swap_accepted) continue;
        for (int64_t x = 0; x < W; ++x) swap_accepted[t] += sw[t * W + x];
    }
    if (chain) big_copy(chain, a.h + o_chain, n_in * (size_t)n_chain_temps * W * P * 8);
    if (lnlike_chain) big_copy(lnlike_chain, a.h + o_llc, n_in * TW * 8);
    *done = true;
    return MCD_OK;
}

int run_temper(mcd_catalog* cat, const mcd_temper_desc* d, int64_t n_steps, double* pos, double* lnlike, double* lnprior,
               uint64_t seed, int64_t step0, double* chain, double* lnlike_chain, int64_t* accepted, int64_t* swap_proposed,
               int64_t* swap_accepted, const mcd_prior_desc* prior) {
    if (!cat || !d || !pos || !lnlike || !lnprior) return fail(MCD_ERR_INVALID, "mcd_temper_block: null argument");
    if (int urc = ctx_usable(cat->ctx)) return urc;
    const mcd_stretch_desc& m = d->map;
    if (m.n_bins > 1 || cat->n_psets != 1)
        return fail(MCD_ERR_INVALID, "mcd_temper_block: binned catalogues are not covered (the rungs take the ensemble index of the bins)");
    if (cat->precision != MCD_F64) return fail(MCD_ERR_INVALID, "mcd_temper_block: tempered blocks need an MCD_F64 catalogue");
    if (m.k != cat->k) return fail(MCD_ERR_INVALID, "mcd_temper_block: descriptor has the wrong number of kernel columns");
    if (n_steps < 0 || step0 < 0) return fail(MCD_ERR_INVALID, "mcd_temper_block: steps non-negative");
    if (!m.col_source || !m.col_const || !m.col_factor || !m.lo || !m.hi || !d->betas) return fail(MCD_ERR_INVALID, "mcd_temper_block: null descriptor array");
    for (int c = 0; c < m.k; ++c)
        if (m.col_source[c] >= m.n_dim) return fail(MCD_ERR_INVALID, "mcd_temper_block: col_source outside the free parameters");
    mcd::TemperShared ts;
    ts.n_dim = m.n_dim; ts.k = m.k; ts.col_source = m.col_source; ts.col_const = m.col_const; ts.col_factor = m.col_factor;
    ts.lo = m.lo; ts.hi = m.hi; ts.fixed_ok = m.fixed_ok; ts.n_temps = d->n_temps; ts.n_walkers = m.n_walkers; ts.betas = d->betas;
    PriorHost ph;
    if (int prc = prior_of(prior, m.n_dim, "mcd_temper_block", ph)) return prc;
    ts.prior = ph.table;
    if (!mcd::temper_args_ok(ts, d->n_chain_temps))
        return fail(MCD_ERR_INVALID, "mcd_temper_block: n_walkers even and >= 2, 1 <= n_dim <= 12, n_temps >= 1, betas[0] == 1 and "
                                     "strictly decreasing within [0, 1], 1 <= n_chain_temps <= n_temps");
    if (temper_resident_covers(cat, ts.n_temps, ts.n_walkers, ts.n_dim, n_steps, d->n_chain_temps, chain != nullptr, lnlike_chain != nullptr)) {
        bool done = false;
        const int rc = temper_block_device(cat, ts, n_steps, pos, lnlike, lnprior, seed, step0, d->n_chain_temps, chain, lnlike_chain,
                                           accepted, swap_proposed, swap_accepted, &done);
        if (rc != MCD_OK) return rc;
        if (done) return MCD_OK;
    }
    struct PlainKernels {
        mcd_catalog* cat; int saved;
        explicit PlainKernels(mcd_catalog* c) : cat(c), saved(c->allow_fast) { c->allow_fast = 0; }
        ~PlainKernels() { cat->allow_fast = saved; }
    } plain(cat);
    int eval_rc = MCD_OK;
    const int rc = mcd::temper_block(ts, n_steps, pos, lnlike, lnprior, seed, step0, d->n_chain_temps, chain, lnlike_chain, accepted,
                                     swap_proposed, swap_accepted, [&](const double* table, int64_t n, double* out) {
                                         eval_rc = mcd_loglike_batch(cat, n, m.k, table, out);
                                         return eval_rc;
                                     });
    if (rc == mcd::TEMPER_EVAL_FAILED) return eval_rc;
    if (rc == mcd::TEMPER_OUTSIDE)
        return fail(MCD_ERR_NONFINITE, "mcd_temper_block: a walker starts outside the prior or with a non-finite log-likelihood");
    if (rc == mcd::TEMPER_NAN) return fail(MCD_ERR_NONFINITE, "mcd_temper_block: the log-likelihood returned NaN");
    if (rc != mcd::TEMPER_OK) return fail(MCD_ERR_INVALID, "mcd_temper_block: bad arguments");
    ++cat->temper_host_blocks;
    return MCD_OK;
}

}

extern "C" {

int mcd_temper_block(mcd_catalog* cat, const mcd_temper_desc* d, int64_t n_steps, double* pos, double* lnlike, double* lnprior,
                     uint64_t seed, int64_t step0, double* chain, double* lnlike_chain, int64_t* accepted,
                     int64_t* swap_proposed, int64_t* swap_accepted) {
    try {
    return run_temper(cat, d, n_steps, pos, lnlike, lnprior, seed, step0, chain, lnlike_chain, accepted, swap_proposed,
                      swap_accepted, nullptr);
    } catch (...) { return on_exception("mcd_temper_block"); }
}

// ... 31 lines not shown
```

### mcmc_dynamics_amd/csrc/mcd_chunks.h

```cpp
#pragma once

#include <algorithm>
#include <cmath>
#include <cstdint>
#include <limits>
#include <vector>

namespace mcd {

struct Chunk {
    int64_t begin;
    int32_t count;
    int32_t pset;
};

struct ShardRange { int64_t begin, n; };
inline ShardRange shard_range(int64_t n_stars, int i, int n_shards) {
    const int64_t b = n_stars * i / n_shards;
    return ShardRange{b, n_stars * (i + 1) / n_shards - b};
}

constexpr int64_t kMaxChunkLen = (int64_t)1 << 20;

struct ChunkPlan {
// ... 89 lines not shown
        }
        plan.max_chunks_per_pset = std::max<int64_t>(plan.max_chunks_per_pset, (int64_t)plan.chunks.size() - plan.offsets[p]);
    }
    plan.offsets[n_psets] = (int64_t)plan.chunks.size();
    if (n_psets == 1 && !plan.chunks.empty() && len < (int64_t)1 << 30) {
        bool uniform = true;
        for (size_t i = 0; i < plan.chunks.size() && uniform; ++i) {
            const Chunk u = uniform_chunk((int64_t)i, len, 0, n, (int64_t)plan.chunks.size());
            uniform = plan.chunks[i].begin == u.begin && plan.chunks[i].count == u.count;
        }
        if (uniform) plan.uniform_len = (int)len;
    }
    }
    if (!narrow_exceptions.empty()) {
        plan.general.assign(plan.chunks.size(), 0);
        bool any = false;
        for (size_t i = 0; i < plan.chunks.size(); ++i) {
            const int64_t lo = star_begin + plan.chunks[i].begin, hi = lo + plan.chunks[i].count;
            const auto it = std::lower_bound(narrow_exceptions.begin(), narrow_exceptions.end(), lo);
            if (it != narrow_exceptions.end() && *it < hi) { plan.general[i] = 1; any = true; }
        }
        if (!any) plan.general.clear();
    }
    return plan;
}

inline std::vector<int64_t> verr_order(const double* records, int64_t n, int nd) {
    std::vector<int64_t> perm((size_t)n);
    for (int64_t i = 0; i < n; ++i) perm[(size_t)i] = i;
    std::stable_sort(perm.begin(), perm.end(), [&](int64_t a, int64_t b) {
        const double x = records[a * nd + 1], y = records[b * nd + 1];
        return x < y || (y != y && x == x);
    });
    return perm;
}

inline std::vector<int64_t> permuted_exceptions(const std::vector<int64_t>& narrow_exceptions, const std::vector<int64_t>& perm,
                                                int64_t star_begin) {
    std::vector<int64_t> out;
    if (narrow_exceptions.empty()) return out;
    const int64_t n = (int64_t)perm.size();
    std::vector<int64_t> inverse((size_t)n);
    for (int64_t i = 0; i < n; ++i) inverse[(size_t)perm[(size_t)i]] = i;
    for (int64_t g : narrow_exceptions)
        if (g >= star_begin && g < star_begin + n) out.push_back(star_begin + inverse[(size_t)(g - star_begin)]);
    std::sort(out.begin(), out.end());
    return out;
}

inline double series_threshold(double e_first, double e_last) {
    const double need = 0.5 * (e_last - e_first) * 0x1p13 - (0.5 * e_first + 0.5 * e_last);
    return need == need ? need : std::numeric_limits<double>::infinity();
}

inline std::vector<double> series_thresholds(const ChunkPlan& plan, const double* sorted_e2) {
    std::vector<double> need;
    need.reserve(plan.chunks.size());
    for (size_t c = 0; c < plan.chunks.size(); ++c) {
        const Chunk& ch = plan.chunks[c];
        if (ch.count <= 0 || (!plan.general.empty() && plan.general[c])) continue;
        need.push_back(series_threshold(sorted_e2[ch.begin], sorted_e2[ch.begin + ch.count - 1]));
    }
    std::sort(need.begin(), need.end());
    return need;
}

inline double direct_threshold(double e_first, double e_last) {
    const double need = std::max(series_threshold(e_first, e_last), 7.0 * (0.5 * e_first + 0.5 * e_last));
    return need == need ? need : std::numeric_limits<double>::infinity();
}

inline std::vector<double> direct_thresholds(const ChunkPlan& plan, const double* sorted_e2) {
    std::vector<double> need;
    need.reserve(plan.chunks.size());
    for (size_t c = 0; c < plan.chunks.size(); ++c) {
        const Chunk& ch = plan.chunks[c];
        if (ch.count <= 0 || (!plan.general.empty() && plan.general[c])) continue;
        need.push_back(direct_threshold(sorted_e2[ch.begin], sorted_e2[ch.begin + ch.count - 1]));
    }
    std::sort(need.begin(), need.end());
    return need;
}

inline std::vector<double> pset_background_sums(const double* lnlike_bg, const std::vector<int64_t>& bin_offsets,
                                                int64_t star_begin, int64_t n) {
    const int64_t n_psets = (int64_t)bin_offsets.size() - 1;
    std::vector<double> sums(n_psets, 0.0);
    for (int64_t p = 0; p < n_psets; ++p) {
        const int64_t b0 = std::max(bin_offsets[p], star_begin);
        const int64_t b1 = std::min(bin_offsets[p + 1], star_begin + n);
        double sum = 0.0, comp = 0.0;
        for (int64_t i = b0; i < b1; ++i) {
            const double x = lnlike_bg[i], t = sum + x;
            comp += (std::fabs(sum) >= std::fabs(x)) ? (sum - t) + x : (x - t) + sum;
            sum = t;
        }
        sums[p] = sum + comp;
    }
    return sums;
}

inline int64_t main_grid(int64_t n_chunks, int64_t n_walkers) {
    const int64_t n_wtiles = (n_walkers + 63) / 64;
    if (n_wtiles <= 4) return (n_chunks * n_wtiles + 3) / 4;
    return (n_chunks + 7) / 8 * 8 * ((n_wtiles + 3) / 4);
}

}
```

### mcmc_dynamics_amd/csrc/mcd_exp_split.h

```cpp
#pragma once

#include <cmath>
#include <cstdint>
#include <vector>

#include "mcd_chunks.h"
#include "mcd_math.h"

namespace mcd {

constexpr long double kExpSplitInvStepL = 1.44269504088896340735992468100189214L * kExpTabSize;
constexpr long double kExpSplitStepL = 0.693147180559945309417232121458176568L / kExpTabSize;
constexpr double kExpSplitMagic = 6755399441055744.0;

struct ExpSplitRecord {
    double M, ompk, nbf;
};
inline ExpSplitRecord exp_split_record(double nbp, double omp) {
    const long double t = (long double)nbp * kExpSplitInvStepL;
    const long double nbi = rintl(t);
    const double nbf = (double)(t - nbi);
    const long double kappa = ((long double)kExpSplitC / (1 << kExpSplitShift)) * expl(-(long double)nbf * kExpSplitStepL);
    ExpSplitRecord out;
    out.M = (double)((long double)kExpSplitMagic + (nbi - (long double)(kExpSplitShift * kExpTabSize)));
    out.ompk = (double)((long double)omp * kappa);
    out.nbf = nbf;
    return out;
}

inline double exp_split_chunk_const(const double* nbf, int64_t count) {
    long double s = 0.0L;
    for (int64_t i = 0; i < count; ++i) s += (long double)nbf[i];
    return (double)(s * kExpSplitStepL - (long double)count * logl((long double)kExpSplitC / (1 << kExpSplitShift)));
}

inline void exp_split_records(const double* rec, int64_t n, double* out, double* nbf) {
    constexpr int ND = record_doubles(MODEL_BGFIXED, false), XB = geometry_doubles(MODEL_BGFIXED, false);
    for (int64_t i = 0; i < n; ++i) {
        const double* r = rec + i * ND;
        double* o = out + i * ND;
        for (int j = 0; j < XB; ++j) o[j] = r[j];
        const ExpSplitRecord s = exp_split_record(r[XB + 3], r[XB + 2]);
        o[XB] = s.M;
        o[XB + 1] = s.ompk;
        o[XB + 2] = o[XB + 3] = 0.0;
        nbf[i] = s.nbf;
    }
}

inline std::vector<double> exp_split_chunk_consts(const ChunkPlan& plan, const double* nbf) {
    std::vector<double> out(plan.chunks.size());
    for (size_t c = 0; c < plan.chunks.size(); ++c)
        out[c] = exp_split_chunk_const(nbf + plan.chunks[c].begin, plan.chunks[c].count);
    return out;
}

}
```

### mcmc_dynamics_amd/csrc/mcd_host.h

```cpp
#pragma once

#include <hip/hip_runtime.h>
#include <rccl/rccl.h>

#include <algorithm>
#include <atomic>
#include <chrono>
#include <cmath>
#include <cstdio>
#include <cstdlib>
#include <cstring>
#include <limits>
#include <map>
#include <memory>
#include <mutex>
#include <string>
#include <thread>
#include <vector>

#include "../../include/mcd.h"
#include "mcd_exp_split.h"
#include "mcd_internal.h"
#include "mcd_guard.h"
#include "mcd_math.h"
// ... 11 lines not shown

#define MCD_HIP(call)                                                                                   \
    do {                                                                                                \
        hipError_t e_ = (call);                                                                         \
        if (e_ != hipSuccess)                                                                           \
            return ::mcd::host::fail(MCD_ERR_HIP, std::string(#call) + ": " + hipGetErrorString(e_));   \
    } while (0)

struct Rccl {
    void* handle = nullptr;
    decltype(&ncclGetUniqueId) GetUniqueId = nullptr;
    decltype(&ncclCommInitRank) CommInitRank = nullptr;
    decltype(&ncclCommInitAll) CommInitAll = nullptr;
    decltype(&ncclCommDestroy) CommDestroy = nullptr;
    decltype(&ncclAllReduce) AllReduce = nullptr;
    decltype(&ncclGroupStart) GroupStart = nullptr;
    decltype(&ncclGroupEnd) GroupEnd = nullptr;
    decltype(&ncclGetErrorString) GetErrorString = nullptr;
    decltype(&ncclCommCount) CommCount = nullptr;
    decltype(&ncclCommUserRank) CommUserRank = nullptr;
    decltype(&ncclGetVersion) GetVersion = nullptr;
};
extern Rccl g_rccl;
int load_rccl();

#define MCD_NCCL(call)                                                                                  \
    do {                                                                                                \
        ncclResult_t r_ = (call);                                                                       \
        if (r_ != ncclSuccess)                                                                          \
            return ::mcd::host::fail(MCD_ERR_RCCL,                                                      \
                                   std::string(#call) + ": " + ::mcd::host::g_rccl.GetErrorString(r_)); \
    } while (0)

struct DeviceSlot {
    int device = 0;
    hipStream_t stream = nullptr;
    hipStream_t stream2 = nullptr;
    hipStream_t comm_stream = nullptr;
    ncclComm_t comm = nullptr;
};

struct WorkSet {
    int64_t n_walkers = 0;
    int64_t n_chunks = 0;
    int64_t max_chunks_per_pset = 0;
    int uniform_len = 0;
    int uniform_extra = 0;
    int waves = 4;
    mcd::Chunk* d_chunks = nullptr;
    int64_t* d_offsets = nullptr;
    uint8_t* d_chunk_general = nullptr;
    double* d_split_const = nullptr;
    double* d_params = nullptr;
    void* d_wpar = nullptr;
    double* d_partials = nullptr;
    double* d_out = nullptr;
    double* d_out2 = nullptr;
    int buf = 0;
    double* d_partials2 = nullptr;
    double* d_grad_partials = nullptr;
    double* d_grad_out = nullptr;
    double* h_grad_out = nullptr;
    hipEvent_t ev_staged = nullptr;
    bool lane1_knows_staging = false;
    bool lane1_used = false;
    hipEvent_t ev_reduced[2] = {nullptr, nullptr};
    hipEvent_t ev_comm[2] = {nullptr, nullptr};
    bool comm_pending[2] = {false, false};
    double* h_params = nullptr;
    double* h_out = nullptr;
    double* m_params = nullptr;
    double* m_out = nullptr;
    bool mapped = false;
    double launch_tag = 0.0;
    int fast = 0;
    int narrow_rescale = 0;
    bool exp_split[2] = {false, false};
    bool staged = false;
    bool sorted = false;
    std::vector<double> series_need;
    int64_t series_chunks = 0;
    std::vector<double> direct_need;
    int64_t direct_chunks = 0;
};

struct ChainArena {
    char* d = nullptr;
    char* h = nullptr;
    size_t bytes = 0;
};

struct Shard {
    int slot = 0;
    int64_t star_begin = 0;
    int64_t n = 0;
    void* records = nullptr;
    void* records_sorted = nullptr;
    std::vector<double> sorted_e2;
    void* records_split = nullptr;
    std::vector<double> sorted_nbf;
    std::vector<int64_t> sorted_exceptions;
    double* d_pset_const = nullptr;
    std::map<int64_t, WorkSet> work;
    hipEvent_t ev_begin = nullptr, ev_k0 = nullptr, ev_k1 = nullptr, ev_end = nullptr;
    std::vector<std::pair<hipEvent_t, hipEvent_t>> ring;
    size_t ring_used = 0;
};

struct DeviceScratch {
    std::vector<void*> blocks;
    hipEvent_t e0 = nullptr, e1 = nullptr;
    DeviceScratch() = default;
    DeviceScratch(const DeviceScratch&) = delete;
    template <class T>
    hipError_t malloc(T** p, size_t bytes) {
        blocks.push_back(nullptr);
        const hipError_t e = hipMalloc(&blocks.back(), bytes);
        *p = static_cast<T*>(blocks.back());
        return e;
    }
    hipError_t create_events() {
        const hipError_t e = hipEventCreate(&e0);
        return e != hipSuccess ? e : hipEventCreate(&e1);
    }
    ~DeviceScratch() {
        for (void* p : blocks) (void)hipFree(p);
        if (e0) (void)hipEventDestroy(e0);
        if (e1) (void)hipEventDestroy(e1);
    }
};

struct PriorHost {
    std::vector<int32_t> kind;
    std::vector<double> loc, scale, c0;
    mcd::PriorTable table;
};

int ctx_fail(mcd_ctx* ctx, const std::string& what);
int ctx_usable(mcd_ctx* ctx);
int wait_ctx_stream(mcd_ctx* ctx, hipStream_t s, int64_t spin_us, const char* stage);
int build_workset(mcd_catalog* cat, Shard& sh, int64_t n_walkers, WorkSet** out);
LaunchShape main_launch_shape(mcd_catalog* cat, const Shard& sh, const WorkSet& w, int level, bool coll, double* out_buf,
                              int64_t n_out);
const double* fast_pset_const(const mcd_catalog* cat, const Shard& sh, int level);
const void* main_records(const Shard& sh, const WorkSet& w);
int64_t series_chunk_count(const mcd_catalog* cat, const WorkSet& w, int level, const double* params, int64_t n_rows);
int64_t direct_chunk_count(const mcd_catalog* cat, const WorkSet& w, int level, const double* params, int64_t n_rows);
int prior_of(const mcd_prior_desc* p, int32_t n_dim, const char* who, PriorHost& out);
void big_copy(void* dst, const void* src, size_t bytes);
int fast_level(const mcd_catalog* cat, const double* params, int64_t n_rows);
int sync_all(mcd_catalog* cat);

MCD_HOST_END

struct mcd_ctx {
    std::vector<mcd::host::DeviceSlot> slots;
    int rank = 0;
    int n_ranks = 1;
    bool multi_process = false;
    bool force_collective = false;
    int64_t collective_timeout_ms = 120000;
    std::atomic<int> abort_flag{0};
    std::atomic<int> failed{0};
    std::mutex note_mutex;
    std::string abort_reason;
    std::string failure;
    bool has_comm() const { return n_ranks > 1 || slots.size() > 1 || force_collective; }
};

struct mcd_catalog {
    mcd_ctx* ctx = nullptr;
    int model = 0;
    bool free_centre = false;
    int precision = 0;
    int k = 4;
    int64_t n_stars = 0;
    int64_t n_psets = 1;
    std::vector<int64_t> bin_offsets;
    std::vector<mcd::host::Shard> shards;
    mcd::CatalogStats stats;
    bool timing = false;
    bool timing_all = false;
    int allow_fast = 1;
    bool zero_copy = true;
    int64_t timing_stride = 1;
    int64_t timing_launches = 0;
    int64_t spin_us = 20000;
    int tail_split = 1;
    int64_t target_waves = 10240;
    int64_t chunk_len = 0;
    int prefetch = -1;
    int narrow_bounded = 1;
    int verr_sorted = -1;
    int root_series = 1;
    int exp_split = 1;
    int root_direct = 1;
    int balance = -1;
    int two_lanes = 1;
    int f32_domain = 1;
    mcd::F32Domain last_f32;
    int64_t posterior_pass = 65536;
    int64_t loo_scratch_mb = 2048;
    int combine = 1;
    int64_t cur_walkers = 0;
    double last_kernel_ms = -1.0, last_device_ms = -1.0;
    bool timing_pending = false;
    int64_t last_grid = 0, last_chunks = 0;
    uint64_t launch_seq = 0;
    int64_t n_reruns = 0;
    int device_chain = 1;
    int fused_reduce = 1;
    int defer_guard = 1;
    bool chain_last_fused = false;
    mcd::host::ChainArena chain;
    int chain_hint = -1;
    int64_t chain_backoff = 0;
    int chain_consecutive = 0;
    int64_t chain_device_blocks = 0, chain_host_blocks = 0, chain_discarded = 0;
    int chain_last_status = 0;
    std::vector<hipEvent_t> chain_events;
    mcd::host::ChainArena hmc;
    int64_t hmc_device_blocks = 0, hmc_host_blocks = 0;
    mcd::host::ChainArena temper;
    int64_t temper_device_blocks = 0, temper_host_blocks = 0;
    int last_prefetch = -1;
    int64_t last_series_chunks = -1;
    int64_t last_direct_chunks = -1;
    int last_exp_split = -1;
    int last_narrow_bounded = -1;
};

#define MCD_WAIT(ctx, stream, spin, stage)                                                              \
    do {                                                                                                \
        const int w_rc_ = ::mcd::host::wait_ctx_stream((ctx), (stream), (spin), (stage));               \
        if (w_rc_ != MCD_OK) return w_rc_;                                                              \
    } while (0)
```

### mcmc_dynamics_amd/csrc/mcd_internal.h

```cpp
#pragma once

#include <hip/hip_runtime.h>
#include <cstdint>

#include "mcd_chunks.h"
#include "mcd_guard.h"
#include "mcd_launch.h"
#include "mcd_prior.h"

namespace mcd {

struct LaunchShape {
    int model;
    bool free_centre;
    int precision;
    int fast;
    int uniform_len = 0;
    int64_t n_records = 0;
    int uniform_extra = 0;
    int waves = 4;
    const uint8_t* chunk_general = nullptr;
    bool prefetch = false;
    int narrow_rescale = 0;
    bool root_series = false;
    bool root_direct = false;
    const void* records_split = nullptr;
    const double* split_const = nullptr;
    double* rerun_flag = nullptr;
    double launch_tag = 0.0;
};

struct RawColumns {
    const double* ra;
    const double* dec;
    const double* v;
    const double* verr;
    const double* lnbg;
    const double* pmember;
    const double* density;
};

hipError_t launch_prepare_records(hipStream_t s, const RawColumns& raw, int64_t n, int model, bool free_centre,
                                  int precision, double ra_c_deg, double dec_c_deg, void* records);

hipError_t launch_prepare_walkers(hipStream_t s, const double* params, int64_t n_rows, int k, int model,
                                  bool free_centre, int precision, void* wpar);

inline bool narrow_bounded_launch(const LaunchShape& sh) {
    return sh.fast == 2 && sh.model == MODEL_BGFIXED && !sh.free_centre && sh.precision == 0 && sh.prefetch &&
           (sh.narrow_rescale == 16 || sh.narrow_rescale == 32);
}

inline bool exp_split_launch(const LaunchShape& sh) {
    return sh.fast == 2 && sh.model == MODEL_BGFIXED && !sh.free_centre && sh.precision == 0 && sh.root_series &&
           sh.root_direct && sh.records_split != nullptr && sh.split_const != nullptr;
}

hipError_t launch_loglike(hipStream_t s, const LaunchShape& shape, const void* records, const Chunk* chunks,
                          int64_t n_chunks, const void* wpar, double* partials, int64_t n_walkers);

hipError_t launch_reduce(hipStream_t s, const double* partials, const int64_t* pset_slot_offsets,
                         int64_t n_psets, int64_t n_slots, int64_t max_slots_per_pset, int64_t n_walkers,
                         const double* pset_const, double* out);
int64_t partial_slots(const LaunchShape& shape, int64_t n_chunks, int64_t n_walkers);
constexpr int64_t kFusedReduceSlots = 256;

hipError_t launch_per_star(hipStream_t s, const LaunchShape& shape, const void* records, int64_t n,
                           const void* wpar_row, int mode, double* out);

int record_bytes(int model, bool free_centre, int precision);

enum ChainMeta : int { META_N_OK = 0, META_STATUS = 1, META_LEVEL = 2, META_WORDS = 4 };
enum ChainStatus : int {
    CHAIN_NAN = 1,
    CHAIN_RERUN = 2,
    CHAIN_LEVEL = 4,
    CHAIN_NO_PROPOSAL = 8
};
struct StretchDevice {
    int64_t n_bins = 1;
    int64_t n_walkers = 0;
    int32_t n_dim = 0, k = 0;
    int32_t fixed_ok = 1;
    int32_t model = 0, free_centre = 0;
    int32_t allow_fast = 1;
    int32_t expected_level = 0;
#ifdef MCD_CHAIN_STAMPS
    unsigned long long* stamps = nullptr;
    long long launch_index = 0;
#endif
    int32_t force_general = 0;
    int32_t fused = 0;
    const double* partials = nullptr;
    int64_t n_slots = 0;
    const int64_t* slot_offsets = nullptr;
    const double* pset_const = nullptr;
    StatsScalars stats;
    const int32_t* col_source = nullptr;
    const double* col_const = nullptr;
    const double* col_factor = nullptr;
    const double* lo = nullptr;
    const double* hi = nullptr;
    PriorTable prior;
    double* prior_val = nullptr;
    double* pos = nullptr;
    double* lnp = nullptr;
    long long* accepted = nullptr;
    const int32_t* order = nullptr;
    const double* zz = nullptr;
    const double* thr = nullptr;
    const int32_t* pick = nullptr;
    double* chain = nullptr;
    double* lnprob_chain = nullptr;
    double* proposal = nullptr;
    uint8_t* ok = nullptr;
    int32_t* meta = nullptr;
    int32_t* n_ok = nullptr;
    double* ranges = nullptr;
    double* table = nullptr;
    int32_t defer_guard = 0;
    double* table_log = nullptr;
    int32_t* n_ok_log = nullptr;
    int32_t* level_log = nullptr;
    double* wpar = nullptr;
};

hipError_t launch_stretch_step(hipStream_t s, const StretchDevice& d, int64_t acc_step, int acc_h, int64_t prop_step,
                               int prop_h, const double* ll, double rerun_tag);
hipError_t launch_stretch_status(hipStream_t s, const int32_t* meta, double* out);
hipError_t launch_stretch_judge(hipStream_t s, const StretchDevice& d, int64_t n_launches);
bool chain_numbers_on_device(int64_t n_walkers);
hipError_t launch_chain_numbers(hipStream_t s, uint64_t seed, int64_t step0, int64_t i0, int64_t i1, int64_t n_bins,
                                int64_t n_walkers, int n_dim, int32_t* order, double* zz, double* thr, int32_t* pick);
bool stretch_step_handles(const StretchDevice& d);
bool stretch_step_fuses(const StretchDevice& d);

int kde_slices(int64_t n, int64_t m, int* slice_len);
hipError_t launch_kde(hipStream_t s, const double* comp, int64_t m, const double* v, const double* verr, int64_t n,
                      double sigma_int, int slice_len, int n_slices, double* part_dmin, double* part_sum,
// ... 4 lines not shown
```

### mcmc_dynamics_amd/csrc/mcd_kernels.hip

```cpp
#include <type_traits>

#include "mcd_internal.h"
#include "mcd_dispatch.h"
#include "mcd_math.h"
#include "mcd_prep.h"
#include "mcd_reduce.h"

namespace mcd {

namespace {

constexpr double kR0Arcmin = 3437.7467707849392526;

template <class T>
__global__ __launch_bounds__(kBlock) void prepare_records_kernel(RawColumns raw, int64_t n, int model,
                                                                  int free_centre, double ra_c, double dec_c,
                                                                  T* __restrict__ rec) {
    int64_t i = (int64_t)blockIdx.x * kBlock + threadIdx.x;
    if (i >= n) return;
    const int nd = record_doubles(model, free_centre != 0);
    T* r = rec + i * nd;
    const double verr = raw.verr[i];
    r[0] = (T)raw.v[i];
    r[1] = (T)(verr * verr);
    const double ra = raw.ra[i], dec = raw.dec[i];
    const int k = geometry_doubles(model, free_centre != 0);
    if (free_centre) {
        double sa, ca, sd, cd;
        sincos(ra * kDeg2Rad, &sa, &ca);
        sincos(dec * kDeg2Rad, &sd, &cd);
        r[2] = (T)(cd * sa); r[3] = (T)(cd * ca); r[4] = (T)sd; r[5] = (T)0;
    } else {
        const double dra = (ra - ra_c) * kDeg2Rad;
        const double dec_r = dec * kDeg2Rad, dec_cr = dec_c * kDeg2Rad;
        const double dx = -kR0Arcmin * cos(dec_r) * sin(dra);
        const double dy = kR0Arcmin * (sin(dec_r) * cos(dec_cr) - cos(dec_r) * sin(dec_cr) * cos(dra));
        if (is_profile(model)) {
            const double xs = 60.0 * dx, ys = 60.0 * dy;
            r[2] = (T)xs; r[3] = (T)ys; r[4] = (T)(xs * xs + ys * ys); r[5] = (T)0;
        } else {
            const double rr = hypot(dx, dy);
            double s, c;
            if (rr > 0.0) { s = dy / rr; c = dx / rr; }
            else { s = 0.0; c = signbit(dx) ? -1.0 : 1.0; }
            r[2] = (T)s; r[3] = (T)c;
        }
    }
    const int bg = bg_kind(model);
    if (bg == BG_FIXED) {
        const double b = raw.lnbg[i], pm = raw.pmember[i];
        r[k] = (T)b; r[k + 1] = (T)pm; r[k + 2] = (T)(1.0 - pm); r[k + 3] = (T)fmax(log(pm) - (b + kHalfLn2Pi), -2000.0);
    } else if (bg == BG_GAUSS) {
        r[k] = (T)raw.density[i]; r[k + 1] = (T)0;
    } else if (bg == BG_FIXED_DENSITY) {
        const double b = raw.lnbg[i];
        r[k] = (T)b; r[k + 1] = (T)fmax(log(raw.density[i]) - (b + kHalfLn2Pi), -2000.0); r[k + 2] = (T)raw.density[i];
        r[k + 3] = (T)0;
    }
}

template <class T>
__global__ __launch_bounds__(kBlock) void prepare_walkers_kernel(const double* __restrict__ params, int64_t n_rows,
                                                                  int k, int model, int free_centre,
                                                                  T* __restrict__ wpar) {
    int64_t i = (int64_t)blockIdx.x * kBlock + threadIdx.x;
    if (i >= n_rows) return;
    walker_constants<T>(params + i * k, model, free_centre != 0, wpar + i * KD);
}

#ifdef MCD_MAIN_STAMPS
constexpr int kStampBlocks = 1 << 16;
__device__ unsigned long long g_main_stamps[kStampBlocks][4];
#endif

__device__ const double kExpTabDevice[kExpTabSize] = {MCD_EXP_TABLE_VALUES};
__device__ const double kExpTabSqrt2Device[kExpTabSize] = {MCD_EXP_TABLE_SQRT2_VALUES};

template <int MODEL, bool FREE, class T, class A, int FAST, bool PF, int WAVES, bool BOUNDED = false>
__global__ __launch_bounds__(WAVES * kWave, WAVES > 4 ? 4 : 1) void loglike_kernel(const T* __restrict__ recs,
                                                                 const Chunk* __restrict__ chunks,
                                                                 const T* __restrict__ wpar,
                                                                 double* __restrict__ partials, int64_t n_tasks,
                                                                 int n_wtiles, int64_t n_walkers, int64_t n_chunks,
                                                                 int uniform_len, int uniform_extra, int64_t n_records,
                                                                 double* __restrict__ rerun_flag, double launch_tag,
                                                                 const uint8_t* __restrict__ chunk_general,
                                                                 int64_t n_slots, int narrow_iters, int root_series,
                                                                 const T* __restrict__ recs_split,
                                                                 const double* __restrict__ split_const) {
    constexpr int ND = record_doubles(MODEL, FREE);
    constexpr int kThreads = WAVES * kWave;
    constexpr bool kCombine = WAVES > kWavesPerBlock;
#ifdef MCD_MAIN_STAMPS
    const unsigned long long stamp_entry = __builtin_amdgcn_s_memrealtime();
#endif
    constexpr bool kUsesExpTab = FAST && bg_kind(MODEL) != BG_NONE && sizeof(T) == 8;
    __shared__ double exptab_lds[kUsesExpTab ? kExpTabSize : 1];
    constexpr bool kTabBiased = kUsesExpTab && FAST == 2 && MODEL == MODEL_BGFIXED;
    __shared__ double combine_lds[kCombine ? WAVES : 1][kCombine ? kWave : 1];
    if constexpr (kUsesExpTab) {
        static_assert(kExpTabSize % kThreads == 0, "whole table entries per thread");
        const double* __restrict__ src = exp_table_is_sqrt2_scaled(MODEL) ? kExpTabSqrt2Device : kExpTabDevice;
#pragma unroll
        for (int i = 0; i < kExpTabSize / kThreads; ++i) {
            const int j = i * kThreads + threadIdx.x;
            exptab_lds[j] = kTabBiased ? exp_tab_bias(src[j], j) : src[j];
        }
        __syncthreads();
    }
    const int wave = __builtin_amdgcn_readfirstlane((int)(threadIdx.x >> 6));
    const int lane = threadIdx.x & (kWave - 1);
    int64_t chunk_id;
    int wtile;
    bool live = true;
    if (kCombine || n_wtiles <= kWavesPerBlock) {
        const int64_t task = (int64_t)blockIdx.x * WAVES + wave;
        if (task >= n_tasks) {
            if constexpr (!kCombine) return;
            live = false;
        }
        chunk_id = task / n_wtiles;
        wtile = (int)(task - chunk_id * n_wtiles);
        if (!live) { chunk_id = 0; wtile = wave % n_wtiles; }
    } else {
        const int m = (n_wtiles + kWavesPerBlock - 1) / kWavesPerBlock;
        const int64_t group = blockIdx.x / (8 * m);
        const int j = (int)(blockIdx.x - group * (8 * m));
        chunk_id = group * 8 + (j & 7);
        wtile = (j >> 3) * kWavesPerBlock + wave;
        if (chunk_id >= n_chunks || wtile >= n_wtiles) return;
    }
    Chunk ch;
    if (uniform_len > 0) {
        const int64_t shifted = chunk_id < (int64_t)uniform_extra ? chunk_id : (int64_t)uniform_extra;
        ch.begin = chunk_id * uniform_len + 8 * shifted;
        const int64_t left = n_records - ch.begin;
        ch.count = chunk_id == n_chunks - 1 ? (int32_t)left : uniform_len + (chunk_id < (int64_t)uniform_extra ? 8 : 0);
        ch.pset = 0;
    } else {
        ch = chunks[chunk_id];
    }
    const int64_t w_raw = (int64_t)wtile * kWave + lane;
    const bool active = w_raw < n_walkers;
    const int64_t w_idx = active ? w_raw : n_walkers - 1;

    double result = 0.0;
    if (live) {
        const T* __restrict__ wp = wpar + ((int64_t)ch.pset * n_walkers + w_idx) * KD;
        WalkerConsts<T> w;
        w.load(wp);

        const RecPtr<T> chunk_recs = (RecPtr<T>)(recs + ch.begin * ND);
        bool denormal;
        if constexpr (FAST == 2) {
            const bool general = bg_kind(MODEL) != BG_NONE && chunk_general != nullptr && chunk_general[chunk_id] != 0;
            if (general) result = chunk_loglike<MODEL, FREE, T, A, 1, PF, kTabBiased>(chunk_recs, ch.count, w, denormal, exptab_lds);
            else result = chunk_loglike<MODEL, FREE, T, A, 2, PF, kTabBiased, BOUNDED>(
                     chunk_recs, ch.count, w, denormal, exptab_lds, narrow_iters, root_series != 0, root_series > 1,
                     recs_split ? (RecPtr<T>)(recs_split + ch.begin * ND) : (RecPtr<T>) nullptr, split_const + chunk_id);
        } else {
            result = chunk_loglike<MODEL, FREE, T, A, FAST, PF>(chunk_recs, ch.count, w, denormal, exptab_lds);
        }
        if (FAST && denormal && active) {
            if (rerun_flag) *rerun_flag = launch_tag;
            else result = __builtin_nan("");
        }
    }
    if constexpr (kCombine) {
        combine_lds[wave][lane] = result;
        __syncthreads();
        if (wave < n_wtiles) {
            double sum = combine_lds[wave][lane];
            for (int c = n_wtiles; c < WAVES; c += n_wtiles) sum += combine_lds[c + wave][lane];
            partials[partial_index(w_raw, n_slots, blockIdx.x)] = sum;
        }
    } else {
        partials[partial_index(w_raw, n_slots, chunk_id)] = result;
    }
#ifdef MCD_MAIN_STAMPS
    if (threadIdx.x == 0 && blockIdx.x < kStampBlocks) {
        g_main_stamps[blockIdx.x][0] = stamp_entry;
        g_main_stamps[blockIdx.x][1] = __builtin_amdgcn_s_memrealtime();
        g_main_stamps[blockIdx.x][2] = ((unsigned long long)__builtin_amdgcn_s_getreg((31 << 11) | 20) << 32) |
                                       (unsigned)__builtin_amdgcn_s_getreg((31 << 11) | 4);
        g_main_stamps[blockIdx.x][3] = (unsigned long long)ch.count;
    }
#endif
}

template <int SUB, int U, bool ONE_ROUND, bool SEVERAL>
__global__ __launch_bounds__(kPartialGroup * SUB) void reduce_group_kernel(const double* __restrict__ partials,
                                                                            const int64_t* __restrict__ offs,
                                                                            int64_t n_slots, int64_t n_walkers,
                                                                            int64_t n_groups,
                                                                            const double* __restrict__ pset_const,
                                                                            double* __restrict__ out, int64_t single0) {
    constexpr int kThreads = kPartialGroup * SUB;
    constexpr int kWaves = kThreads / kWave;
    __shared__ double lds[kWaves > 1 ? kWaves : 1][kPartialGroup];
    const int64_t pset = blockIdx.x / n_groups, g = blockIdx.x - pset * n_groups;
    const int q = threadIdx.x & 3, s = threadIdx.x >> 2;
    const int64_t c0 = single0 >= 0 ? 0 : offs[pset], c1 = single0 >= 0 ? single0 : offs[pset + 1];
    const double add = pset_const ? pset_const[pset] : 0.0;
    const double2* __restrict__ col = reinterpret_cast<const double2*>(partials + g * n_slots * kPartialGroup) + q;
    double ax = 0.0, ay = 0.0;
    const int64_t count = c1 - c0;
    if (SEVERAL && SUB > 8 && count <= 2 * 8 * U) {
        if (s < 2 * 8) reduce_sublane_sum<8, U, true>(col, c0, c1, s, ax, ay);
    } else if (SEVERAL && SUB > 32 && count <= 2 * 32 * U) {
        if (s < 2 * 32) reduce_sublane_sum<32, U, true>(col, c0, c1, s, ax, ay);
    } else if (SEVERAL && !ONE_ROUND && count <= 2 * SUB * U) {
        reduce_sublane_sum<SUB, U, true>(col, c0, c1, s, ax, ay);
    } else {
        reduce_sublane_sum<SUB, U, ONE_ROUND>(col, c0, c1, s, ax, ay);
    }
    reduce_wave_combine(ax, ay);
    const int lane = threadIdx.x & (kWave - 1);
    if constexpr (kWaves > 1) {
        if (lane < 4) { lds[threadIdx.x >> 6][2 * q] = ax; lds[threadIdx.x >> 6][2 * q + 1] = ay; }
        __syncthreads();
        if (threadIdx.x < kPartialGroup) {
            double acc = lds[0][threadIdx.x];
#pragma unroll
            for (int w = 1; w < kWaves; ++w) acc += lds[w][threadIdx.x];
            const int64_t w = g * kPartialGroup + threadIdx.x;
            if (w < n_walkers) out[pset * n_walkers + w] = acc + add;
        }
    } else {
        if (lane < 4) {
            const int64_t w = g * kPartialGroup + 2 * q;
            if (w < n_walkers) out[pset * n_walkers + w] = ax + add;
            if (w + 1 < n_walkers) out[pset * n_walkers + w + 1] = ay + add;
        }
    }
}

template <int MODEL, bool FREE, class T>
__global__ __launch_bounds__(kBlock) void per_star_kernel(const T* __restrict__ recs, int64_t n,
                                                           const T* __restrict__ wp, int mode,
                                                           double* __restrict__ out) {
    constexpr int ND = record_doubles(MODEL, FREE);
    const int64_t i = (int64_t)blockIdx.x * kBlock + threadIdx.x;
    if (i >= n) return;
    WalkerConsts<T> w;
    w.load(wp);
    T lc, lb, m;
    star_components<MODEL, FREE, T>((RecPtr<T>)(recs + i * ND), w, lc, lb, m);
    if (mode == 1) { out[i] = (double)mixture_lnl(lc, lb, m); return; }
    const T shift = is_profile(MODEL) ? max_(lc, lb) : T(0);
    const T ec = m * exp_(lc - shift), eb = (T(1) - m) * exp_(lb - shift);
    out[i] = (double)(ec / (ec + eb));
}

template <int MODEL, bool FREE, class T, class A, int FAST>
hipError_t launch_one(hipStream_t s, const LaunchShape& sh, const void* records, const Chunk* chunks, int64_t n_chunks,
                      const void* wpar, double* partials, int64_t n_walkers) {
    const int n_wtiles = (int)((n_walkers + kWave - 1) / kWave);
    const int64_t n_tasks = n_chunks * n_wtiles;
    constexpr bool kCanCombine = FAST != 0 && sizeof(T) == 8 && sizeof(A) == 8;
    const bool combine = kCanCombine && sh.waves > kWavesPerBlock;
    const int64_t grid = combine ? (n_tasks + sh.waves - 1) / sh.waves
                                 : main_grid(n_chunks, n_walkers);
    if (grid <= 0) return hipSuccess;
    const int64_t n_slots = combine ? grid : n_chunks;
    constexpr bool kCanBound = FAST == 2 && MODEL == MODEL_BGFIXED && !FREE && sizeof(T) == 8 && sizeof(A) == 8;
    const bool bounded = kCanBound && sh.prefetch && narrow_bounded_launch(sh);
    const int narrow_iters = bounded ? sh.narrow_rescale / 8 : 1;
#define MCD_LAUNCH_MAIN(PF_, WAVES_, BOUNDED_)                                                                               \
    hipLaunchKernelGGL((loglike_kernel<MODEL, FREE, T, A, FAST, PF_, WAVES_, BOUNDED_>), dim3((unsigned)grid),               \
                       dim3(WAVES_ * kWave), 0, s, (const T*)records, chunks, (const T*)wpar, partials, n_tasks, n_wtiles,   \
                       n_walkers, n_chunks, sh.uniform_len, sh.uniform_extra, sh.n_records, sh.rerun_flag, sh.launch_tag,    \
                       sh.chunk_general, n_slots, narrow_iters, sh.root_series ? (sh.root_direct ? 2 : 1) : 0,                \
                       (const T*)(exp_split_launch(sh) ? sh.records_split : nullptr), sh.split_const)
    auto launch = [&](auto waves) {
        constexpr int W = decltype(waves)::value;
        if (bounded) MCD_LAUNCH_MAIN(true, W, kCanBound);
        else if (FAST != 0 && sh.prefetch) MCD_LAUNCH_MAIN((FAST != 0), W, false);
        else MCD_LAUNCH_MAIN(false, W, false);
        return hipGetLastError();
    };
#undef MCD_LAUNCH_MAIN
    if constexpr (kCanCombine) {
        if (combine && sh.waves == 8) return launch(std::integral_constant<int, 8>());
        if constexpr (bg_kind(MODEL) != BG_GAUSS) {
            if (combine && sh.waves == 16) return launch(std::integral_constant<int, 16>());
        }
        if (combine) return hipErrorInvalidValue;
    }
    return launch(std::integral_constant<int, kWavesPerBlock>());
}

template <int MODEL, bool FREE>
hipError_t launch_precision(hipStream_t s, const LaunchShape& sh, const void* records, const Chunk* chunks,
                            int64_t n_chunks, const void* wpar, double* partials, int64_t n_walkers) {
    switch (sh.precision) {
        case 0:
            if constexpr (bg_kind(MODEL) != BG_NONE || (MODEL == MODEL_PROFILE && !FREE)) {
                if (sh.fast == 2)
                    return launch_one<MODEL, FREE, double, double, 2>(s, sh, records, chunks, n_chunks, wpar, partials, n_walkers);
            }
            if (sh.fast) return launch_one<MODEL, FREE, double, double, 1>(s, sh, records, chunks, n_chunks, wpar, partials, n_walkers);
            return launch_one<MODEL, FREE, double, double, 0>(s, sh, records, chunks, n_chunks, wpar, partials, n_walkers);
        case 1:
            if (sh.fast) return launch_one<MODEL, FREE, float, float, 1>(s, sh, records, chunks, n_chunks, wpar, partials, n_walkers);
            return launch_one<MODEL, FREE, float, float, 0>(s, sh, records, chunks, n_chunks, wpar, partials, n_walkers);
        case 2:
            if (sh.fast) return launch_one<MODEL, FREE, float, double, 1>(s, sh, records, chunks, n_chunks, wpar, partials, n_walkers);
            return launch_one<MODEL, FREE, float, double, 0>(s, sh, records, chunks, n_chunks, wpar, partials, n_walkers);
    }
    return hipErrorInvalidValue;
}

}

#ifdef MCD_MAIN_STAMPS
extern "C" int mcd_debug_main_stamps(unsigned long long* out, long long n_blocks) {
    if (n_blocks > kStampBlocks) n_blocks = kStampBlocks;
    return (int)hipMemcpyFromSymbol(out, HIP_SYMBOL(g_main_stamps), (size_t)n_blocks * 4 * sizeof(unsigned long long));
}
#endif

int record_bytes(int model, bool free_centre, int precision) {
    return record_doubles(model, free_centre) * (precision == 0 ? 8 : 4);
}

hipError_t launch_prepare_records(hipStream_t s, const RawColumns& raw, int64_t n, int model, bool free_centre,
                                  int precision, double ra_c_deg, double dec_c_deg, void* records) {
    if (n <= 0) return hipSuccess;
    const unsigned grid = (unsigned)((n + kBlock - 1) / kBlock);
    return dispatch_term_type(precision, [&](auto t) {
        using T = decltype(t);
        hipLaunchKernelGGL(prepare_records_kernel<T>, dim3(grid), dim3(kBlock), 0, s, raw, n, model, (int)free_centre,
                           ra_c_deg, dec_c_deg, (T*)records);
        return hipGetLastError();
    });
}

hipError_t launch_prepare_walkers(hipStream_t s, const double* params, int64_t n_rows, int k, int model,
                                  bool free_centre, int precision, void* wpar) {
    if (n_rows <= 0) return hipSuccess;
    const unsigned grid = (unsigned)((n_rows + kBlock - 1) / kBlock);
    return dispatch_term_type(precision, [&](auto t) {
        using T = decltype(t);
        hipLaunchKernelGGL(prepare_walkers_kernel<T>, dim3(grid), dim3(kBlock), 0, s, params, n_rows, k, model,
                           (int)free_centre, (T*)wpar);
        return hipGetLastError();
    });
}

hipError_t launch_loglike(hipStream_t s, const LaunchShape& sh, const void* records, const Chunk* chunks,
                          int64_t n_chunks, const void* wpar, double* partials, int64_t n_walkers) {
    return dispatch_model(sh.model, sh.free_centre, [&](auto M, auto FREE) {
        return launch_precision<decltype(M)::value, decltype(FREE)::value>(s, sh, records, chunks, n_chunks, wpar, partials,
                                                                           n_walkers);
    }, hipErrorInvalidValue);
// ... 50 lines not shown
```

### mcmc_dynamics_amd/csrc/mcd_math.h

```cpp
#pragma once

#include <cmath>
#include <cstdint>
#include <cstring>
#include <type_traits>

#include "mcd_exp_table.h"

#if defined(__HIPCC__)
#define MCD_HD __host__ __device__ __forceinline__
#else
#define MCD_HD inline
#endif
#if defined(__HIP_DEVICE_COMPILE__)
#define MCD_CONST_AS __attribute__((address_space(4)))
#else
#define MCD_CONST_AS
#endif
namespace mcd { template <class T> using RecPtr = const T MCD_CONST_AS*; }

#if defined(__HIP_DEVICE_COMPILE__)
#define MCD_KEEP_BRANCH() asm volatile("")
#else
#define MCD_KEEP_BRANCH() ((void)0)
// ... 399 lines not shown
    }
};

struct RootSeries {
    static constexpr double kMaxT = 0x1p-13;
    double eb, b0, b1, b2, b3;
    MCD_HD bool setup(double eb_, double half, double s2) {
        eb = eb_;
        RootCentre c;
        c.setup(eb, s2);
        const double m0 = c.m0, G0 = c.G0, q = c.q;
        b0 = fma_(G0, c.corr, G0);
        b1 = -0.5 * (G0 * q);
        b2 = -0.75 * (b1 * q);
        b3 = (-5.0 / 6.0) * (b2 * q);
        return half >= 0.0 && 8.0 * half <= kMaxT * m0;
    }
    MCD_HD bool setup_chunk(double e_first, double e_last, double s2) {
        return setup(0.5 * e_first + 0.5 * e_last, 0.5 * (e_last - e_first), s2);
    }
    MCD_HD double g(double e) const {
        const double delta = e - eb;
        return fma_(fma_(fma_(b3, delta, b2), delta, b1), delta, b0);
    }
};

MCD_HD double fma_sgpr_factor(double a, double s, double c) {
#if defined(__HIP_DEVICE_COMPILE__)
    double r;
    asm("v_fma_f64 %0, %1, %2, %3" : "=v"(r) : "v"(a), "s"(s), "v"(c));
    return r;
#else
    return std::fma(a, s, c);
#endif
}

struct RootDirect {
    static constexpr double kRhoMax = 0.125;
    static constexpr double kErrorBound = 4.6e-16;
    double c0, c1, c2, c3;
    static MCD_HD bool direct_ok(double eb, double s2) { return (1.0 / kRhoMax - 1.0) * eb <= s2; }
    MCD_HD void setup(double eb, double s2) {
        RootCentre c;
        c.setup(eb, s2);
        const double G0 = c.G0, q = c.q;
        const double rho = c.p * c.inv;
        const double P = rho * fma_(rho, fma_(rho, 0.3125, 0.375), 0.5);
        c0 = fma_(G0, c.corr + P, G0);
        const double gq = G0 * q;
        c1 = -gq * fma_(rho, fma_(rho, 0.9375, 0.75), 0.5);
        const double gq2 = gq * q;
        c2 = gq2 * fma_(rho, 0.9375, 0.375);
        c3 = -0.3125 * (gq2 * q);
    }
    MCD_HD double g_direct(double e) const {
        return fma_sgpr_factor(fma_sgpr_factor(fma_sgpr_factor(c3, e, c2), e, c1), e, c0);
    }
};

static_assert(kExpTabBits == 10 || kExpTabBits == 8, "kExpSplitC is written for N = 1024 (and halved exactly for N = 256)");
constexpr double kExpSplitC = 0x1.337cc2183b050p+5 / (kExpTabBits == 10 ? 1.0 : 2.0);
constexpr int kExpSplitShift = 5;
constexpr double kExpSplitS1 = kExpTabStepHi + kExpTabStepLo;
constexpr double kExpSplitS2 = kExpPolyC2 * kExpSplitS1 * kExpSplitS1;
constexpr double kExpSplitS3 = kExpPolyC3 * kExpSplitS1 * kExpSplitS1 * kExpSplitS1;
constexpr double kExpSplitS4 = kExpPolyC4 * kExpSplitS1 * kExpSplitS1 * kExpSplitS1 * kExpSplitS1;
MCD_HD double exp_split_reduce(double dgs, double M, int& k) {
    const double shifted = fnma_sgpr_addend(dgs, dgs, M);
    const double w = shifted - M;
    uint64_t bits;
    std::memcpy(&bits, &shifted, sizeof bits);
    k = (int)(uint32_t)bits;
    return fma_(-dgs, dgs, -w);
}
MCD_HD double exp_poly_steps(double rv, double s1) {
    double p;
    if constexpr (kExpPolyDegree == 4) p = fma_(fma_(rv, kExpSplitS4, kExpSplitS3), rv, kExpSplitS2);
    else p = fma_(rv, kExpSplitS3, kExpSplitS2);
    p = fma_sgpr_addend(p, rv, s1);
    return fma_(p, rv, 1.0);
}

struct RootDirectSplit : RootDirect {
    MCD_HD void setup_scaled(double eb, double s2, double scale) {
        RootCentre c;
        c.setup(eb, s2);
        const double q = c.q;
        const double G0s = c.G0 * scale;
        const double eg = fma_(c.G0, scale, -G0s);
        const double rho = c.p * c.inv;
        const double P = rho * fma_(rho, fma_(rho, 0.3125, 0.375), 0.5);
        c0 = fma_(G0s, (c.corr + P) + eg * ((0.25 / scale) * (c.m0 * c.G0)), G0s);
        const double gq = G0s * q;
        c1 = -gq * fma_(rho, fma_(rho, 0.9375, 0.75), 0.5);
        const double gq2 = gq * q;
        c2 = gq2 * fma_(rho, 0.9375, 0.375);
        c3 = -0.3125 * (gq2 * q);
    }
};

MCD_HD bool wave_all(bool ok) {
#if defined(__HIP_DEVICE_COMPILE__)
    return __builtin_amdgcn_ballot_w64(!ok) == 0;
#else
    return ok;
#endif
}

MCD_HD bool is_zero_bits(double x) {
    uint64_t b;
    __builtin_memcpy(&b, &x, sizeof b);
    return (b << 1) == 0;
}

struct BgFixedAcc {
    LogProduct l;
    LogProduct lden;
    int emin;
    MCD_HD void init() { l.init(); lden.init(); emin = LogProduct::kTrackInit; }
    MCD_HD bool denormal() const { return emin < LogProduct::kTrackFloor; }
    template <bool NARROW = false>
    MCD_HD void add_density(double d, double n, double rho, double f, double nbp, const double* __restrict__ exptab) {
        add<false, false, NARROW>(d, n, f, nbp, exptab);
        lden.mul(rho + f);
    }
    template <bool UNIFORM_OMP = true, bool HALVED = false, bool NARROW = false, bool TAB_BIASED = false, bool CLAMP = true>
    MCD_HD void add(double d, double n, double omp, double nbp, const double* __restrict__ exptab) {
        const double g = (NARROW && HALVED) ? rsqrt2_newton(n) : rsqrt_nr(n);
        add_g<UNIFORM_OMP, HALVED, NARROW, TAB_BIASED, CLAMP>(d, g, omp, nbp, exptab);
    }
    template <bool UNIFORM_OMP = true, bool HALVED = false, bool NARROW = false, bool TAB_BIASED = false, bool CLAMP = true>
    MCD_HD void add_g(double d, double g, double omp, double nbp, const double* __restrict__ exptab) {
        const double dg = d * g;
        const double u0 = HALVED ? fnma_sgpr_addend(dg, dg, nbp) : fma_sgpr_addend(-0.5 * dg, dg, nbp);
        const double u = NARROW ? u0 : fmax_raw(u0, -1100.0);
        if constexpr (NARROW && TAB_BIASED) {
            const double es = exp_tab_scaled<false, CLAMP>(u, exptab);
            const double y = UNIFORM_OMP ? fma_sgpr_addend(g, es, omp) : fma_(g, es, omp);
            l.mul(y);
            return;
        }
        int k;
        const double er = exp_tab<!NARROW, TAB_BIASED>(u, k, exptab);
        if constexpr (NARROW) {
            const double y = UNIFORM_OMP ? fma_sgpr_addend(g, ldexp_(er, k), omp) : fma_(g, ldexp_(er, k), omp);
            l.mul(y);
            return;
        }
        const int kc = k > 1000 ? 1000 : k;
        const double y = UNIFORM_OMP ? fma_sgpr_addend(g, ldexp_(er, kc), omp) : fma_(g, ldexp_(er, kc), omp);
        l.mul_any_track(y, emin);
        l.e32 += k - kc;
    }
    template <bool TAB_BIASED = false, bool CLAMP = true>
    MCD_HD void add_gs(double d, double gs, double M, double ompk, double s1, const double* __restrict__ exptab) {
        int k;
        const double p = exp_poly_steps(exp_split_reduce(d * gs, M, k), s1);
        if constexpr (CLAMP) k = k > kExpTabKMin ? k : kExpTabKMin;
        double es;
        if constexpr (TAB_BIASED) {
            const double t = exptab[k & (kExpTabSize - 1)];
            const int32_t kh = (int32_t)((uint32_t)k << kExpTabHiShift);
#if defined(__HIP_DEVICE_COMPILE__)
            typedef uint32_t word2 __attribute__((ext_vector_type(2)));
            word2 tw = __builtin_bit_cast(word2, t);
            tw.y += (uint32_t)kh;
            es = __builtin_bit_cast(double, tw) * p;
#else
            es = add_hi_word(t, kh) * p;
#endif
        } else {
            es = ldexp_(exptab[k & (kExpTabSize - 1)] * p, k >> kExpTabBits);
        }
        l.mul(fma_sgpr_addend(gs, es, ompk));
    }
    MCD_HD void rescale() { l.rescale(); }
    MCD_HD void rescale_density() { l.rescale(); lden.rescale(); }
    MCD_HD void rescale_narrow() { l.rescale_narrow(); }
    MCD_HD void rescale_density_narrow() { l.rescale_narrow(); lden.rescale_narrow(); }
    MCD_HD double finish() { return l.value(); }
    MCD_HD double finish_density() { return l.value() - lden.value(); }
};
// ... 315 lines not shown
    }
    return acc.finish(count);
}

template <bool PF>
MCD_HD double chunk_profile_narrow(RecPtr<double> r, int count, const WalkerConsts<double>& w) {
    constexpr int ND = record_doubles(MODEL_PROFILE, false);
    ProfileNarrowAcc acc;
    acc.init();
    const double hs2a = 0.5 * w.s2a;
    auto one = [&](RecPtr<double> rr, double& q1, double& n1, double& m1) {
        m1 = w.rp2 + rr[4];
        const double t2 = rsqrt2_newton(w.a2 + rr[4]);
        const double n = fma_(hs2a, t2, rr[1]);
        const double cross = fma_(w.vx, rr[3], -(w.vy * rr[2]));
        const double nd = fma_(rr[0] - w.vsys, m1, -(w.rp_2 * cross));
        q1 = nd * nd;
        n1 = (m1 * m1) * n;
    };
    const int n8 = count >> 3;
    for (int g = 0; g < n8; ++g, r += 8 * ND) {
        RecordPrefetch<8 * ND * 8, PF> pf;
        pf.issue(r + 8 * ND);
        double qq[8], nn[8], mm[8];
#pragma unroll
        for (int j = 0; j < 8; ++j) one(r + j * ND, qq[j], nn[j], mm[j]);
        const double m_prod = ((mm[0] * mm[1]) * (mm[2] * mm[3])) * ((mm[4] * mm[5]) * (mm[6] * mm[7]));
        acc.add8(qq, nn, m_prod);
        pf.retire(acc.q);
    }
    for (int j = count & ~7; j < count; ++j, r += ND) {
        double q1, n1, m1;
        one(r, q1, n1, m1);
        acc.add1(q1, n1, m1);
    }
    return acc.finish(count);
}

template <int MODEL, bool FREE, bool PF>
MCD_HD double chunk_const_fast(RecPtr<double> r, int count, const WalkerConsts<double>& w) {
    constexpr int ND = record_doubles(MODEL, FREE);
    ConstAcc acc;
    acc.init();
    constexpr bool TREE16 = MODEL == MODEL_CONST && !FREE;
    const int n16 = TREE16 ? count >> 4 : 0;
    for (int g = 0; g < n16; ++g, r += 16 * ND) {
        RecordPrefetch<16 * ND * 8, PF> pf;
        pf.issue(r + 16 * ND);
        double qq[16], nn[16];
#pragma unroll
        for (int j = 0; j < 16; ++j) {
            double d;
            star_d_n<MODEL, double, FREE, true>(r + j * ND, w, d, nn[j]);
            qq[j] = d * d;
        }
        acc.add16(qq, nn);
        pf.retire(acc.q);
    }
    const int n8 = TREE16 ? (count >> 3) & 1 : count >> 3;
    for (int g = 0; g < n8; ++g, r += 8 * ND) {
        RecordPrefetch<8 * ND * 8, PF> pf;
        pf.issue(r + 8 * ND);
        double qq[8], nn[8];
#pragma unroll
        for (int j = 0; j < 8; ++j) {
            double d;
            star_d_n<MODEL, double, FREE, true>(r + j * ND, w, d, nn[j]);
            qq[j] = d * d;
        }
        acc.add8(qq, nn);
        pf.retire(acc.q);
    }
    for (int j = count & ~7; j < count; ++j, r += ND) {
        double d, n;
        star_d_n<MODEL, double, FREE, true>(r, w, d, n);
        acc.add1(d * d, n);
    }
    return acc.finish(count);
}

template <int MODEL, bool FREE, int FAST, bool PF, bool TAB_BIASED, bool BOUNDED>
MCD_HD double chunk_bgfixed_fast(RecPtr<double> r, int count, const WalkerConsts<double>& w, bool& denormal,
                                 const double* __restrict__ exptab, int rescale_iters, bool series, bool direct,
                                 RecPtr<double> r_split, const double* __restrict__ split_const) {
    constexpr int ND = record_doubles(MODEL, FREE);
    constexpr int XB = geometry_doubles(MODEL, FREE);
    constexpr bool HALVED = MODEL == MODEL_BGFIXED;
    constexpr bool NARROW = FAST == 2 && MODEL == MODEL_BGFIXED;
    constexpr double kScale = NARROW ? 8.0 : 2.0;
    const double s2x = kScale * w.s2;
    const double scale = BOUNDED ? vgpr_constant(kScale) : kScale;
    BgFixedAcc acc;
    acc.init();
    RootSeries sr;
    auto one = [&](RecPtr<double> rr, auto SERIES, double sc) {
        double d, n;
        star_d_n<MODEL, double, FREE, true>(rr, w, d, n);
        if constexpr (std::is_same<decltype(SERIES), RootDirectSplit>::value) {
            acc.add_gs<TAB_BIASED, !BOUNDED>(d, SERIES.g_direct(rr[1]), rr[XB], rr[XB + 1], sc, exptab);
        } else if constexpr (std::is_same<decltype(SERIES), RootDirect>::value) {
            acc.add_g<true, HALVED, NARROW, TAB_BIASED, !BOUNDED>(d, SERIES.g_direct(rr[1]), rr[XB + 2], rr[XB + 3], exptab);
        } else if constexpr (decltype(SERIES)::value) {
            acc.add_g<true, HALVED, NARROW, TAB_BIASED, !BOUNDED>(d, sr.g(rr[1]), rr[XB + 2], rr[XB + 3], exptab);
        } else {
            if constexpr (HALVED) n = fma_(sc, rr[1], s2x);
            acc.add<true, HALVED, NARROW, TAB_BIASED, !BOUNDED>(d, n, rr[XB + 2], rr[XB + 3], exptab);
        }
    };
    const int n4 = count >> 2;
    static_assert(!BOUNDED || (NARROW && PF && TAB_BIASED && !FREE), "the bounded loop is the prefetching BGFIXED one");
    auto four = [&](RecPtr<double> r4, auto SERIES) {
        if constexpr (std::is_same<decltype(SERIES), RootDirectSplit>::value) {
#pragma unroll
            for (int j = 0; j < 4; ++j) one(r4 + j * ND, SERIES, kExpSplitS1);
        } else {
#pragma unroll
            for (int j = 0; j < 4; ++j) one(r4 + j * ND, SERIES, scale);
        }
    };
    auto run = [&](auto SERIES) {
        if constexpr (BOUNDED) {
            int until = rescale_iters;
            for (int g = 0; g < (count >> 3); ++g, r += 8 * ND) {
                RecordPrefetch<8 * ND * 8, PF> pf;
                pf.issue(r + 8 * ND);
                four(r, SERIES);
                four(r + 4 * ND, SERIES);
                pf.retire(acc.l.p);
                if (--until == 0) { until = rescale_iters; MCD_KEEP_BRANCH(); acc.rescale_narrow(); }
            }
            acc.rescale_narrow();
            if (n4 & 1) {
                four(r, SERIES);
                r += 4 * ND;
                acc.rescale_narrow();
            }
        } else if constexpr (NARROW && PF) {
            for (int g = 0; g < (count >> 3); ++g, r += 8 * ND) {
                RecordPrefetch<8 * ND * 8, PF> pf;
                pf.issue(r + 8 * ND);
                four(r, SERIES);
                four(r + 4 * ND, SERIES);
                pf.retire(acc.l.p);
                acc.rescale_narrow();
            }
            if (n4 & 1) {
                four(r, SERIES);
                r += 4 * ND;
                acc.rescale_narrow();
            }
        } else if constexpr (NARROW) {
            for (int g = 0; g < n4; ++g, r += 4 * ND) {
                four(r, SERIES);
                if (g & 1) { MCD_KEEP_BRANCH(); acc.rescale_narrow(); }
            }
            if (n4 & 1) acc.rescale_narrow();
        } else {
            for (int g = 0; g < n4; ++g, r += 4 * ND) {
                RecordPrefetch<4 * ND * 8, PF> pf;
                pf.issue(r + 4 * ND);
                four(r, SERIES);
                pf.retire(acc.l.p);
                acc.rescale();
            }
        }
        for (int j = n4 * 4; j < count; ++j, r += ND) {
            one(r, SERIES, std::is_same<decltype(SERIES), RootDirectSplit>::value ? kExpSplitS1 : kScale);
            acc.rescale();
        }
    };
    constexpr bool kCanSeries = NARROW && MODEL == MODEL_BGFIXED && !FREE;
    bool use_series = false, use_direct = false;
    const bool split = kCanSeries && r_split != nullptr;
    if constexpr (kCanSeries) {
        if (series && count > 0) {
            RootSeries vote;
            const RecPtr<double> rv = split ? r_split : r;
            const bool ok = vote.setup_chunk(rv[1], rv[(int64_t)(count - 1) * ND + 1], w.s2);
            use_series = wave_all(ok);
            if (use_series && direct) use_direct = wave_all(RootDirect::direct_ok(vote.eb, w.s2));
        }
    }
    if constexpr (kCanSeries) {
        if (use_direct && split) {
            r = r_split;
            const double e_first = vgpr_pinned(r[1]), e_last = vgpr_pinned(r[(int64_t)(count - 1) * ND + 1]);
            RootDirectSplit sd;
            sd.setup_scaled(0.5 * e_first + 0.5 * e_last, vgpr_pinned((1.0 / kScale) * s2x), kExpSplitC);
            run(sd);
            const double result = acc.finish() + *split_const;
            denormal = acc.denormal();
            return result;
        } else if (use_direct) {
            const double e_first = vgpr_pinned(r[1]), e_last = vgpr_pinned(r[(int64_t)(count - 1) * ND + 1]);
            RootDirect sd;
            sd.setup(0.5 * e_first + 0.5 * e_last, vgpr_pinned((1.0 / kScale) * s2x));
            run(sd);
        } else if (use_series) {
            const double e_first = vgpr_pinned(r[1]), e_last = vgpr_pinned(r[(int64_t)(count - 1) * ND + 1]);
            sr.setup_chunk(e_first, e_last, vgpr_pinned((1.0 / kScale) * s2x));
            run(std::true_type());
        }
        else run(std::false_type());
    } else {
        run(std::false_type());
    }
    const double result = acc.finish();
    denormal = acc.denormal();
    return result;
}

template <int MODEL, bool FREE, class T, class A, int FAST, bool PF = false, bool TAB_BIASED = false, bool BOUNDED = false>
MCD_HD double chunk_loglike(RecPtr<T> r, int count, const WalkerConsts<T>& w, bool& denormal,
                            const double* __restrict__ exptab, int rescale_iters = 1, bool series = false, bool direct = false,
                            RecPtr<T> r_split = nullptr, const double* __restrict__ split_const = nullptr) {
    constexpr int BG = bg_kind(MODEL);
    denormal = false;
    if constexpr (!FAST) {
        if constexpr (BG == BG_NONE) return chunk_plain<MODEL, FREE, T, A>(r, count, w);
        else return chunk_plain_mixture<MODEL, FREE, T, A>(r, count, w);
    } else if constexpr (sizeof(T) == 4) {
        if constexpr (BG == BG_NONE) return chunk_const_f32<MODEL, FREE, A, PF>(r, count, w);
        else return chunk_mixture_f32<MODEL, FREE, A, PF>(r, count, w);
    } else if constexpr (BG == BG_NONE) {
        if constexpr (FAST == 2 && MODEL == MODEL_PROFILE && !FREE) return chunk_profile_narrow<PF>(r, count, w);
        else return chunk_const_fast<MODEL, FREE, PF>(r, count, w);
    } else if constexpr (BG == BG_FIXED) {
        return chunk_bgfixed_fast<MODEL, FREE, FAST, PF, TAB_BIASED, BOUNDED>(r, count, w, denormal, exptab, rescale_iters, series, direct, r_split, split_const);
    } else if constexpr (BG == BG_FIXED_DENSITY) {
        constexpr int ND = record_doubles(MODEL, FREE);
        constexpr int XB = geometry_doubles(MODEL, FREE);
        constexpr bool NARROW = FAST == 2;
        BgFixedAcc acc;
        acc.init();
        auto four = [&](RecPtr<double> r4) {
#pragma unroll
            for (int j = 0; j < 4; ++j) {
                RecPtr<double> rr = r4 + j * ND;
                double d, n;
                star_d_n<MODEL, double, FREE, true, NARROW>(rr, w, d, n);
                acc.add_density<NARROW>(d, n, rr[XB + 2], w.fb, rr[XB + 1], exptab);
            }
        };
        const int n4 = count >> 2;
        if constexpr (NARROW) {
            for (int g = 0; g < n4; ++g, r += 4 * ND) {
                RecordPrefetch<4 * ND * 8, PF> pf;
                pf.issue(r + 4 * ND);
                four(r);
                pf.retire(acc.l.p);
                if (g & 1) { MCD_KEEP_BRANCH(); acc.rescale_density_narrow(); }
            }
            if (n4 & 1) acc.rescale_density_narrow();
        } else {
            for (int g = 0; g < n4; ++g, r += 4 * ND) {
                RecordPrefetch<4 * ND * 8, PF> pf;
                pf.issue(r + 4 * ND);
                four(r);
                pf.retire(acc.l.p);
                acc.rescale_density();
            }
        }
        for (int j = n4 * 4; j < count; ++j, r += ND) {
            double d, n;
            star_d_n<MODEL, double, FREE, true, NARROW>(r, w, d, n);
            acc.add_density<NARROW>(d, n, r[XB + 2], w.fb, r[XB + 1], exptab);
            acc.rescale_density();
        }
        const double result = acc.finish_density();
        denormal = acc.denormal();
        return result;
    } else {
        constexpr int ND = record_doubles(MODEL, FREE);
        constexpr int XB = geometry_doubles(MODEL, FREE);
        constexpr bool HALVED = MODEL == MODEL_BGGAUSS;
        constexpr bool NARROW = FAST == 2;
        constexpr double kScale = NARROW ? 8.0 : 2.0;
        const double s2x = kScale * w.s2, sb2x = kScale * w.sb2;
        BgGaussAcc acc;
        acc.init();
        auto one = [&](RecPtr<double> rr) {
            double d, n;
            star_d_n<MODEL, double, FREE, true, NARROW>(rr, w, d, n);
            if constexpr (HALVED) acc.add<true, NARROW>(d, fma_(kScale, rr[1], s2x), rr[0] - w.vb, fma_(kScale, rr[1], sb2x), rr[XB], w.fb, exptab);
            else acc.add<false, NARROW>(d, n, rr[0] - w.vb, rr[1] + w.sb2, rr[XB], w.fb, exptab);
        };
        auto four = [&](RecPtr<double> r4) {
#pragma unroll
            for (int j = 0; j < 4; ++j) one(r4 + j * ND);
        };
        const int n4 = count >> 2;
        if constexpr (NARROW) {
            for (int g = 0; g < n4; ++g, r += 4 * ND) {
                RecordPrefetch<4 * ND * 8, PF> pf;
                pf.issue(r + 4 * ND);
                four(r);
                pf.retire(acc.ly.p);
                if (g & 1) { MCD_KEEP_BRANCH(); acc.rescale_narrow(); }
            }
            if (n4 & 1) acc.rescale_narrow();
        } else {
            for (int g = 0; g < n4; ++g, r += 4 * ND) {
                RecordPrefetch<4 * ND * 8, PF> pf;
                pf.issue(r + 4 * ND);
                four(r);
                pf.retire(acc.ly.p);
                acc.rescale();
            }
        }
        for (int j = n4 * 4; j < count; ++j, r += ND) {
            one(r);
// ... 23 lines not shown
```

Before: 1716 billion terms/s.

## Add quadratic series root on 32-star bands for direct bgfixed chunks

Adds a quadratic-polynomial form of the series root for the split-exponent direct path. The host precomputes per-32-star band coefficients into the split records and derives per-chunk width thresholds. The kernel picks this path when every lane of the wave admits it, parks per-lane centre constants in LDS, and refolds at band boundaries. The aim is to cut the per-star root arithmetic, at the cost of extra LDS, boundary bookkeeping, one more vote, and possible register pressure.

```diff
diff --git a/include/mcd.h b/include/mcd.h
--- a/include/mcd.h
+++ b/include/mcd.h
@@ -210,6 +210,8 @@
 int64_t mcd_last_series_chunks(const mcd_catalog* cat);
 int64_t mcd_last_direct_chunks(const mcd_catalog* cat);
 int mcd_last_exp_split(const mcd_catalog* cat);
+int mcd_last_root_quad(const mcd_catalog* cat);
+int64_t mcd_last_quad_chunks(const mcd_catalog* cat);
 int mcd_last_fast_level(const mcd_catalog* cat);
 
 int mcd_last_f32_domain(const mcd_catalog* cat, double* kappa_v, double* kappa_theta);
diff --git a/mcmc_dynamics_amd/_native.py b/mcmc_dynamics_amd/_native.py
--- a/mcmc_dynamics_amd/_native.py
+++ b/mcmc_dynamics_amd/_native.py
@@ -101,6 +101,8 @@
     "mcd_last_series_chunks": (ctypes.c_int64, [ctypes.c_void_p]),
     "mcd_last_direct_chunks": (ctypes.c_int64, [ctypes.c_void_p]),
     "mcd_last_exp_split": (ctypes.c_int, [ctypes.c_void_p]),
+    "mcd_last_root_quad": (ctypes.c_int, [ctypes.c_void_p]),
+    "mcd_last_quad_chunks": (ctypes.c_int64, [ctypes.c_void_p]),
     "mcd_last_fast_level": (ctypes.c_int, [ctypes.c_void_p]),
     "mcd_last_f32_domain": (ctypes.c_int, [ctypes.c_void_p, _c_double_p, _c_double_p]),
     "mcd_set_option": (ctypes.c_int, [ctypes.c_void_p, ctypes.c_char_p, ctypes.c_int64]),
@@ -647,6 +649,14 @@
     def last_exp_split(self):
         return self.lib.mcd_last_exp_split(self.handle)
 
+    @property
+    def last_root_quad(self):
+        return self.lib.mcd_last_root_quad(self.handle)
+
+    @property
+    def last_quad_chunks(self):
+        return self.lib.mcd_last_quad_chunks(self.handle)
+
     def hmc_block(self, plan, chol, step_size, n_leap, pos, lnp, seed, step0, n_steps, chain=None, lnprob_chain=None,
                   accepted=None, energy_error=None, jitter=0.1):
         if n_steps < 0 or step0 < 0 or pos.ndim != 2:
@@ -772,7 +782,7 @@
                                                        ctypes.byref(ch), ctypes.byref(rb)), "mcd_last_launch_info")
         return {"workgroups": wg.value, "walker_tile": tile.value, "chunks": ch.value, "record_bytes": rb.value,
                 "series_chunks": self.last_series_chunks, "direct_chunks": self.last_direct_chunks,
-                "exp_split": self.last_exp_split}
+                "exp_split": self.last_exp_split, "root_quad": self.last_root_quad, "quad_chunks": self.last_quad_chunks}
 
     def close(self):
         if getattr(self, "handle", None):
diff --git a/mcmc_dynamics_amd/csrc/mcd_api_catalog.hip b/mcmc_dynamics_amd/csrc/mcd_api_catalog.hip
--- a/mcmc_dynamics_amd/csrc/mcd_api_catalog.hip
+++ b/mcmc_dynamics_amd/csrc/mcd_api_catalog.hip
@@ -123,6 +123,7 @@
     {"verr_sorted", -1, 1, "verr_sorted: -1 (by record volume, default), 0 (catalogue order) or 1 (sorted by verr)", true, true, MCD_SET(c->verr_sorted = (int)v)},
     {"root_series", 0, 1, "root_series: 1 (series root on the narrow chunks of verr-sorted records, default) or 0 (never)", false, false, MCD_SET(c->root_series = (int)v)},
     {"exp_split", 0, 1, "exp_split: 1 (split exponent offset in the direct chunks where the guard admits it, default) or 0 (never)", false, false, MCD_SET(c->exp_split = (int)v)},
+    {"root_quad", 0, 1, "root_quad: 1 (quadratic series root on 32-star bands where a direct chunk admits it, default) or 0 (never)", false, false, MCD_SET(c->root_quad = (int)v)},
     {"root_direct", 0, 1, "root_direct: 1 (direct form of the series root where a chunk admits it, default) or 0 (delta form only)", false, false, MCD_SET(c->root_direct = (int)v)},
     {"prefetch", -1, 1, "prefetch: -1 (by record volume, default), 0 (off) or 1 (on)", false, false, MCD_SET(c->prefetch = (int)v)},
     {"spin_us", 0, kMax, "spin_us must be >= 0", false, false, MCD_SET(c->spin_us = v)},
@@ -149,6 +150,7 @@
     shape.rerun_flag = coll ? nullptr : out_buf + n_out;
     shape.root_series = w.sorted && cat->root_series != 0;
     shape.root_direct = shape.root_series && cat->root_direct != 0;
+    shape.root_quad = shape.root_direct && cat->root_quad != 0;
     return shape;
 }
 
@@ -166,6 +168,13 @@
     const mcd::ParamRanges pr = mcd::table_ranges(cat->model, cat->free_centre, cat->k, params, n_rows);
     if (!pr.finite) return 0;
     return (int64_t)(std::upper_bound(w.direct_need.begin(), w.direct_need.end(), pr.s2_min) - w.direct_need.begin());
+}
+
+int64_t quad_chunk_count(const mcd_catalog* cat, const WorkSet& w, int level, const double* params, int64_t n_rows) {
+    if (!w.sorted || !cat->root_series || !cat->root_direct || !cat->root_quad || level != 2 || w.quad_need.empty()) return 0;
+    const mcd::ParamRanges pr = mcd::table_ranges(cat->model, cat->free_centre, cat->k, params, n_rows);
+    if (!pr.finite) return 0;
+    return (int64_t)(std::upper_bound(w.quad_need.begin(), w.quad_need.end(), pr.s2_min) - w.quad_need.begin());
 }
 
 const double* fast_pset_const(const mcd_catalog* cat, const Shard& sh, int level) {
@@ -209,7 +218,9 @@
         w.series_need = mcd::series_thresholds(plan, sh.sorted_e2.data());
         w.direct_need = mcd::direct_thresholds(plan, sh.sorted_e2.data());
     }
-    const std::vector<double> split_const = sorted ? mcd::exp_split_chunk_consts(plan, sh.sorted_nbf.data()) : std::vector<double>();
+    const std::vector<double> split_const =
+        sorted ? mcd::exp_split_chunk_consts(plan, sh.sorted_nbf.data(), sh.sorted_e2.data(), sh.n) : std::vector<double>();
+    if (sorted) w.quad_need = mcd::quad_thresholds(plan, sh.sorted_e2.data(), split_const.data() + 1, 2);
     {
         const int64_t n_wtiles = (n_walkers + 63) / 64;
         const bool shape_ok = plan.balanced_m > 0 && plan.balanced_m % 2 == 0 && (n_wtiles == 1 || n_wtiles == 2 || n_wtiles == 4) &&
@@ -512,6 +523,8 @@
 
 int mcd_last_narrow_bounded(const mcd_catalog* cat) { return cat ? cat->last_narrow_bounded : -1; }
 int mcd_last_exp_split(const mcd_catalog* cat) { return cat ? cat->last_exp_split : -1; }
+int mcd_last_root_quad(const mcd_catalog* cat) { return cat ? cat->last_root_quad : -1; }
+int64_t mcd_last_quad_chunks(const mcd_catalog* cat) { return cat ? cat->last_quad_chunks : -1; }
 
 int mcd_last_f32_domain(const mcd_catalog* cat, double* kappa_v, double* kappa_theta) {
     if (!cat) return -1;
diff --git a/mcmc_dynamics_amd/csrc/mcd_api_chain.hip b/mcmc_dynamics_amd/csrc/mcd_api_chain.hip
--- a/mcmc_dynamics_amd/csrc/mcd_api_chain.hip
+++ b/mcmc_dynamics_amd/csrc/mcd_api_chain.hip
@@ -227,6 +227,8 @@
     cat->last_series_chunks = 0;
     cat->last_direct_chunks = 0;
     cat->last_exp_split = 0;
+    cat->last_root_quad = 0;
+    cat->last_quad_chunks = 0;
     const double* pset_const = fast_pset_const(cat, sh, level);
     const int64_t n_slots = mcd::partial_slots(shape, w.n_chunks, half);
     const int64_t max_slots = B == 1 ? n_slots : w.max_chunks_per_pset;
diff --git a/mcmc_dynamics_amd/csrc/mcd_api_eval.hip b/mcmc_dynamics_amd/csrc/mcd_api_eval.hip
--- a/mcmc_dynamics_amd/csrc/mcd_api_eval.hip
+++ b/mcmc_dynamics_amd/csrc/mcd_api_eval.hip
@@ -106,6 +106,7 @@
                                                       b ? narrow_rescale : 0);
         w->series_chunks = series_chunk_count(cat, *w, fast, params, n_rows);
         w->direct_chunks = direct_chunk_count(cat, *w, fast, params, n_rows);
+        w->quad_chunks = quad_chunk_count(cat, *w, fast, params, n_rows);
         w->staged = true;
     }
     cat->cur_walkers = n_walkers;
@@ -192,7 +193,9 @@
             shape.split_const = w.d_split_const;
         }
         cat->last_exp_split = mcd::exp_split_launch(shape) ? 1 : 0;
-        if (&sh == &cat->shards.front()) cat->last_series_chunks = cat->last_direct_chunks = 0;
+        cat->last_root_quad = mcd::root_quad_launch(shape) ? 1 : 0;
+        if (&sh == &cat->shards.front()) cat->last_series_chunks = cat->last_direct_chunks = cat->last_quad_chunks = 0;
+        cat->last_quad_chunks += cat->last_root_quad && shape.fast == 2 ? w.quad_chunks : 0;
         cat->last_series_chunks += shape.root_series && shape.fast == 2 ? w.series_chunks : 0;
         cat->last_direct_chunks += shape.root_direct && shape.fast == 2 ? w.direct_chunks : 0;
         w.launch_tag = coll ? 0.0 : (double)(++cat->launch_seq);
diff --git a/mcmc_dynamics_amd/csrc/mcd_api_temper.hip b/mcmc_dynamics_amd/csrc/mcd_api_temper.hip
--- a/mcmc_dynamics_amd/csrc/mcd_api_temper.hip
+++ b/mcmc_dynamics_amd/csrc/mcd_api_temper.hip
@@ -148,6 +148,8 @@
     cat->last_series_chunks = 0;
     cat->last_direct_chunks = 0;
     cat->last_exp_split = 0;
+    cat->last_root_quad = 0;
+    cat->last_quad_chunks = 0;
     if (*(const int32_t*)(a.h + o_status) != 0)
         return fail(MCD_ERR_NONFINITE, "mcd_temper_block: the log-likelihood returned NaN");
     ++cat->temper_device_blocks;
diff --git a/mcmc_dynamics_amd/csrc/mcd_chunks.h b/mcmc_dynamics_amd/csrc/mcd_chunks.h
--- a/mcmc_dynamics_amd/csrc/mcd_chunks.h
+++ b/mcmc_dynamics_amd/csrc/mcd_chunks.h
@@ -195,6 +195,24 @@
     return need;
 }
 
+inline double quad_threshold(double e_first, double e_last, double H) {
+    const double need = std::max(direct_threshold(e_first, e_last), H * 0x1.6a09e667f3bcdp+17 - (0.5 * e_first + 0.5 * e_last));
+    return need == need ? need : std::numeric_limits<double>::infinity();
+}
+
+inline std::vector<double> quad_thresholds(const ChunkPlan& plan, const double* sorted_e2, const double* chunk_width,
+                                           size_t width_stride = 1) {
+    std::vector<double> need;
+    need.reserve(plan.chunks.size());
+    for (size_t c = 0; c < plan.chunks.size(); ++c) {
+        const Chunk& ch = plan.chunks[c];
+        if (ch.count <= 0 || (!plan.general.empty() && plan.general[c])) continue;
+        need.push_back(quad_threshold(sorted_e2[ch.begin], sorted_e2[ch.begin + ch.count - 1], chunk_width[c * width_stride]));
+    }
+    std::sort(need.begin(), need.end());
+    return need;
+}
+
 inline std::vector<double> pset_background_sums(const double* lnlike_bg, const std::vector<int64_t>& bin_offsets,
                                                 int64_t star_begin, int64_t n) {
     const int64_t n_psets = (int64_t)bin_offsets.size() - 1;
diff --git a/mcmc_dynamics_amd/csrc/mcd_exp_split.h b/mcmc_dynamics_amd/csrc/mcd_exp_split.h
--- a/mcmc_dynamics_amd/csrc/mcd_exp_split.h
+++ b/mcmc_dynamics_amd/csrc/mcd_exp_split.h
@@ -1,7 +1,9 @@
 #pragma once
 
+#include <algorithm>
 #include <cmath>
 #include <cstdint>
+#include <limits>
 #include <vector>
 
 #include "mcd_chunks.h"
@@ -34,6 +36,47 @@
     return (double)(s * kExpSplitStepL - (long double)count * logl((long double)kExpSplitC / (1 << kExpSplitShift)));
 }
 
+constexpr int64_t kQuadBlock = 32;
+inline int64_t quad_blocks(int64_t n) { return n / kQuadBlock; }
+inline int64_t quad_block_of(int64_t i, int64_t n) { return std::min(i / kQuadBlock, quad_blocks(n) - 1); }
+struct QuadBlock {
+    double a2, a1, a0, h;
+};
+inline QuadBlock quad_block(double e_lo, double e_hi) {
+    const long double m = 0.5L * ((long double)e_lo + (long double)e_hi), h = 0.5L * ((long double)e_hi - (long double)e_lo);
+    QuadBlock out;
+    out.a2 = (double)(3.0L * m);
+    out.a1 = (double)(0.75L * h * h - 3.0L * m * m);
+    out.a0 = (double)(m * m * m - 0.75L * h * h * m);
+    out.h = (double)h;
+    return out;
+}
+inline QuadBlock quad_block_consts(const double* e2, int64_t n, int64_t b) {
+    const int64_t last = b == quad_blocks(n) - 1 ? n - 1 : kQuadBlock * b + kQuadBlock - 1;
+    return quad_block(e2[kQuadBlock * b], e2[last]);
+}
+inline void quad_fill_records(double* split, int64_t n) {
+    constexpr int ND = record_doubles(MODEL_BGFIXED, false), XB = geometry_doubles(MODEL_BGFIXED, false);
+    for (int64_t b = 0; b < quad_blocks(n); ++b) {
+        const int64_t first = kQuadBlock * b, last = b == quad_blocks(n) - 1 ? n - 1 : first + kQuadBlock - 1;
+        const QuadBlock q = quad_block(split[first * ND + 1], split[last * ND + 1]);
+        split[first * ND + XB + 2] = q.a2;
+        split[first * ND + XB + 3] = q.a1;
+        split[(first + 1) * ND + XB + 2] = q.a0;
+    }
+}
+inline double quad_chunk_width(const double* e2, int64_t n, int64_t begin, int64_t count) {
+    const double inf = std::numeric_limits<double>::infinity();
+    if (quad_blocks(n) <= 0 || count <= 0 || begin % 8 != 0) return inf;
+    double H = 0.0;
+    for (int64_t b = quad_block_of(begin, n); b <= quad_block_of(begin + count - 1, n); ++b) {
+        const double h = quad_block_consts(e2, n, b).h;
+        if (!(h >= 0.0)) return inf;
+        H = std::max(H, h);
+    }
+    return H;
+}
+
 inline void exp_split_records(const double* rec, int64_t n, double* out, double* nbf) {
     constexpr int ND = record_doubles(MODEL_BGFIXED, false), XB = geometry_doubles(MODEL_BGFIXED, false);
     for (int64_t i = 0; i < n; ++i) {
@@ -46,12 +89,15 @@
         o[XB + 2] = o[XB + 3] = 0.0;
         nbf[i] = s.nbf;
     }
+    quad_fill_records(out, n);
 }
 
-inline std::vector<double> exp_split_chunk_consts(const ChunkPlan& plan, const double* nbf) {
-    std::vector<double> out(plan.chunks.size());
-    for (size_t c = 0; c < plan.chunks.size(); ++c)
-        out[c] = exp_split_chunk_const(nbf + plan.chunks[c].begin, plan.chunks[c].count);
+inline std::vector<double> exp_split_chunk_consts(const ChunkPlan& plan, const double* nbf, const double* e2, int64_t n) {
+    std::vector<double> out(2 * plan.chunks.size());
+    for (size_t c = 0; c < plan.chunks.size(); ++c) {
+        out[2 * c] = exp_split_chunk_const(nbf + plan.chunks[c].begin, plan.chunks[c].count);
+        out[2 * c + 1] = quad_chunk_width(e2, n, plan.chunks[c].begin, plan.chunks[c].count);
+    }
     return out;
 }
 
diff --git a/mcmc_dynamics_amd/csrc/mcd_host.h b/mcmc_dynamics_amd/csrc/mcd_host.h
--- a/mcmc_dynamics_amd/csrc/mcd_host.h
+++ b/mcmc_dynamics_amd/csrc/mcd_host.h
@@ -117,6 +117,8 @@
     int64_t series_chunks = 0;
     std::vector<double> direct_need;
     int64_t direct_chunks = 0;
+    std::vector<double> quad_need;
+    int64_t quad_chunks = 0;
 };
 
 struct ChainArena {
@@ -181,6 +183,7 @@
 const void* main_records(const Shard& sh, const WorkSet& w);
 int64_t series_chunk_count(const mcd_catalog* cat, const WorkSet& w, int level, const double* params, int64_t n_rows);
 int64_t direct_chunk_count(const mcd_catalog* cat, const WorkSet& w, int level, const double* params, int64_t n_rows);
+int64_t quad_chunk_count(const mcd_catalog* cat, const WorkSet& w, int level, const double* params, int64_t n_rows);
 int prior_of(const mcd_prior_desc* p, int32_t n_dim, const char* who, PriorHost& out);
 void big_copy(void* dst, const void* src, size_t bytes);
 int fast_level(const mcd_catalog* cat, const double* params, int64_t n_rows);
@@ -230,6 +233,7 @@
     int root_series = 1;
     int exp_split = 1;
     int root_direct = 1;
+    int root_quad = 1;
     int balance = -1;
     int two_lanes = 1;
     int f32_domain = 1;
@@ -262,6 +266,8 @@
     int64_t last_series_chunks = -1;
     int64_t last_direct_chunks = -1;
     int last_exp_split = -1;
+    int last_root_quad = -1;
+    int64_t last_quad_chunks = -1;
     int last_narrow_bounded = -1;
 };
 
diff --git a/mcmc_dynamics_amd/csrc/mcd_internal.h b/mcmc_dynamics_amd/csrc/mcd_internal.h
--- a/mcmc_dynamics_amd/csrc/mcd_internal.h
+++ b/mcmc_dynamics_amd/csrc/mcd_internal.h
@@ -26,6 +26,7 @@
     bool root_direct = false;
     const void* records_split = nullptr;
     const double* split_const = nullptr;
+    bool root_quad = false;
     double* rerun_flag = nullptr;
     double launch_tag = 0.0;
 };
@@ -55,6 +56,8 @@
     return sh.fast == 2 && sh.model == MODEL_BGFIXED && !sh.free_centre && sh.precision == 0 && sh.root_series &&
            sh.root_direct && sh.records_split != nullptr && sh.split_const != nullptr;
 }
+
+inline bool root_quad_launch(const LaunchShape& sh) { return sh.root_quad && exp_split_launch(sh); }
 
 hipError_t launch_loglike(hipStream_t s, const LaunchShape& shape, const void* records, const Chunk* chunks,
                           int64_t n_chunks, const void* wpar, double* partials, int64_t n_walkers);
diff --git a/mcmc_dynamics_amd/csrc/mcd_kernels.hip b/mcmc_dynamics_amd/csrc/mcd_kernels.hip
--- a/mcmc_dynamics_amd/csrc/mcd_kernels.hip
+++ b/mcmc_dynamics_amd/csrc/mcd_kernels.hip
@@ -98,6 +98,8 @@
     __shared__ double exptab_lds[kUsesExpTab ? kExpTabSize : 1];
     constexpr bool kTabBiased = kUsesExpTab && FAST == 2 && MODEL == MODEL_BGFIXED;
     __shared__ double combine_lds[kCombine ? WAVES : 1][kCombine ? kWave : 1];
+    constexpr bool kQuad = kTabBiased && !FREE && FAST == 2;
+    __shared__ double quad_lds[kQuad ? 5 * kThreads : 1];
     if constexpr (kUsesExpTab) {
         static_assert(kExpTabSize % kThreads == 0, "whole table entries per thread");
         const double* __restrict__ src = exp_table_is_sqrt2_scaled(MODEL) ? kExpTabSqrt2Device : kExpTabDevice;
@@ -154,10 +156,19 @@
         bool denormal;
         if constexpr (FAST == 2) {
             const bool general = bg_kind(MODEL) != BG_NONE && chunk_general != nullptr && chunk_general[chunk_id] != 0;
-            if (general) result = chunk_loglike<MODEL, FREE, T, A, 1, PF, kTabBiased>(chunk_recs, ch.count, w, denormal, exptab_lds);
-            else result = chunk_loglike<MODEL, FREE, T, A, 2, PF, kTabBiased, BOUNDED>(
-                     chunk_recs, ch.count, w, denormal, exptab_lds, narrow_iters, root_series != 0, root_series > 1,
-                     recs_split ? (RecPtr<T>)(recs_split + ch.begin * ND) : (RecPtr<T>) nullptr, split_const + chunk_id);
+            if (general) {
+                result = chunk_loglike<MODEL, FREE, T, A, 1, PF, kTabBiased>(chunk_recs, ch.count, w, denormal, exptab_lds);
+            } else {
+                QuadArgs quad;
+                if constexpr (kQuad) {
+                    quad = quad_args(ch.begin, n_records, root_series > 2);
+                    quad.park = (QuadParkPtr)quad_lds + wave * kWave;
+                    quad.stride = kThreads;
+                }
+                result = chunk_loglike<MODEL, FREE, T, A, 2, PF, kTabBiased, BOUNDED>(
+                         chunk_recs, ch.count, w, denormal, exptab_lds, narrow_iters, root_series != 0, root_series > 1,
+                         recs_split ? (RecPtr<T>)(recs_split + ch.begin * ND) : (RecPtr<T>) nullptr, split_const + 2 * chunk_id, quad);
+            }
         } else {
             result = chunk_loglike<MODEL, FREE, T, A, FAST, PF>(chunk_recs, ch.count, w, denormal, exptab_lds);
         }
@@ -266,11 +277,12 @@
     constexpr bool kCanBound = FAST == 2 && MODEL == MODEL_BGFIXED && !FREE && sizeof(T) == 8 && sizeof(A) == 8;
     const bool bounded = kCanBound && sh.prefetch && narrow_bounded_launch(sh);
     const int narrow_iters = bounded ? sh.narrow_rescale / 8 : 1;
+    const int root_level = sh.root_series ? (sh.root_direct ? (root_quad_launch(sh) ? 3 : 2) : 1) : 0;
 #define MCD_LAUNCH_MAIN(PF_, WAVES_, BOUNDED_)                                                                               \
     hipLaunchKernelGGL((loglike_kernel<MODEL, FREE, T, A, FAST, PF_, WAVES_, BOUNDED_>), dim3((unsigned)grid),               \
                        dim3(WAVES_ * kWave), 0, s, (const T*)records, chunks, (const T*)wpar, partials, n_tasks, n_wtiles,   \
                        n_walkers, n_chunks, sh.uniform_len, sh.uniform_extra, sh.n_records, sh.rerun_flag, sh.launch_tag,    \
-                       sh.chunk_general, n_slots, narrow_iters, sh.root_series ? (sh.root_direct ? 2 : 1) : 0,                \
+                       sh.chunk_general, n_slots, narrow_iters, root_level,                                                   \
                        (const T*)(exp_split_launch(sh) ? sh.records_split : nullptr), sh.split_const)
     auto launch = [&](auto waves) {
         constexpr int W = decltype(waves)::value;
diff --git a/mcmc_dynamics_amd/csrc/mcd_math.h b/mcmc_dynamics_amd/csrc/mcd_math.h
--- a/mcmc_dynamics_amd/csrc/mcd_math.h
+++ b/mcmc_dynamics_amd/csrc/mcd_math.h
@@ -505,22 +505,71 @@
 }
 
 struct RootDirectSplit : RootDirect {
-    MCD_HD void setup_scaled(double eb, double s2, double scale) {
+    MCD_HD double setup_parts(double eb, double s2, double scale, double& G0s, double& A) {
         RootCentre c;
         c.setup(eb, s2);
         const double q = c.q;
-        const double G0s = c.G0 * scale;
+        G0s = c.G0 * scale;
         const double eg = fma_(c.G0, scale, -G0s);
         const double rho = c.p * c.inv;
         const double P = rho * fma_(rho, fma_(rho, 0.3125, 0.375), 0.5);
-        c0 = fma_(G0s, (c.corr + P) + eg * ((0.25 / scale) * (c.m0 * c.G0)), G0s);
+        A = (c.corr + P) + eg * ((0.25 / scale) * (c.m0 * c.G0));
         const double gq = G0s * q;
         c1 = -gq * fma_(rho, fma_(rho, 0.9375, 0.75), 0.5);
         const double gq2 = gq * q;
         c2 = gq2 * fma_(rho, 0.9375, 0.375);
         c3 = -0.3125 * (gq2 * q);
-    }
-};
+        return q;
+    }
+    MCD_HD void setup_scaled(double eb, double s2, double scale) {
+        double G0s, A;
+        setup_parts(eb, s2, scale, G0s, A);
+        c0 = fma_(G0s, A, G0s);
+    }
+};
+
+struct RootQuadCentre : RootDirectSplit {
+    double G0s, A, k3;
+    MCD_HD void setup_quad(double eb, double s2, double scale) {
+        const double q = setup_parts(eb, s2, scale, G0s, A);
+        k3 = -0.3125 * ((q * q) * q);
+    }
+};
+struct RootQuad {
+    static constexpr double kMaxT = 0x1.6a09e667f3bcdp-18;
+    static constexpr double kErrorBound = 4.9e-16;
+    double q0, q1, q2;
+    static MCD_HD bool quad_ok(double H, double eb, double s2) { return H <= kMaxT * (eb + s2); }
+    MCD_HD void fold(const RootQuadCentre& c, double a2, double a1, double a0) {
+        q2 = fma_sgpr_factor(c.c3, a2, c.c2);
+        q1 = fma_sgpr_factor(c.c3, a1, c.c1);
+        q0 = fma_(c.G0s, fma_sgpr_factor(c.k3, a0, c.A), c.G0s);
+    }
+    MCD_HD double g_quad(double e) const { return fma_sgpr_factor(fma_sgpr_factor(q2, e, q1), e, q0); }
+};
+#if defined(__HIP_DEVICE_COMPILE__)
+typedef __attribute__((address_space(3))) double* QuadParkPtr;
+#else
+typedef double* QuadParkPtr;
+#endif
+struct QuadArgs {
+    bool on = false;
+    int back = 0;
+    int to_boundary = 32;
+    int folds = 0;
+    QuadParkPtr park = nullptr;
+    int stride = 0;
+};
+MCD_HD QuadArgs quad_args(int64_t begin, int64_t n_records, bool enabled) {
+    QuadArgs q;
+    const int64_t n_blocks = n_records >> 5, b = begin >> 5;
+    const int64_t b0 = b < n_blocks ? b : n_blocks - 1;
+    q.on = enabled && n_blocks > 0 && (begin & 7) == 0;
+    q.back = (int)(begin - 32 * b0);
+    q.to_boundary = 32 - (int)(begin & 31);
+    q.folds = b < n_blocks ? (int)(n_blocks - 1 - b) : 0;
+    return q;
+}
 
 MCD_HD bool wave_all(bool ok) {
 #if defined(__HIP_DEVICE_COMPILE__)
@@ -1002,7 +1051,7 @@
 template <int MODEL, bool FREE, int FAST, bool PF, bool TAB_BIASED, bool BOUNDED>
 MCD_HD double chunk_bgfixed_fast(RecPtr<double> r, int count, const WalkerConsts<double>& w, bool& denormal,
                                  const double* __restrict__ exptab, int rescale_iters, bool series, bool direct,
-                                 RecPtr<double> r_split, const double* __restrict__ split_const) {
+                                 RecPtr<double> r_split, const double* __restrict__ split_const, const QuadArgs& quad) {
     constexpr int ND = record_doubles(MODEL, FREE);
     constexpr int XB = geometry_doubles(MODEL, FREE);
     constexpr bool HALVED = MODEL == MODEL_BGFIXED;
@@ -1016,7 +1065,9 @@
     auto one = [&](RecPtr<double> rr, auto SERIES, double sc) {
         double d, n;
         star_d_n<MODEL, double, FREE, true>(rr, w, d, n);
-        if constexpr (std::is_same<decltype(SERIES), RootDirectSplit>::value) {
+        if constexpr (std::is_same<decltype(SERIES), const RootQuad*>::value) {
+            acc.add_gs<TAB_BIASED, !BOUNDED>(d, SERIES->g_quad(rr[1]), rr[XB], rr[XB + 1], sc, exptab);
+        } else if constexpr (std::is_same<decltype(SERIES), RootDirectSplit>::value) {
             acc.add_gs<TAB_BIASED, !BOUNDED>(d, SERIES.g_direct(rr[1]), rr[XB], rr[XB + 1], sc, exptab);
         } else if constexpr (std::is_same<decltype(SERIES), RootDirect>::value) {
             acc.add_g<true, HALVED, NARROW, TAB_BIASED, !BOUNDED>(d, SERIES.g_direct(rr[1]), rr[XB + 2], rr[XB + 3], exptab);
@@ -1030,7 +1081,7 @@
     const int n4 = count >> 2;
     static_assert(!BOUNDED || (NARROW && PF && TAB_BIASED && !FREE), "the bounded loop is the prefetching BGFIXED one");
     auto four = [&](RecPtr<double> r4, auto SERIES) {
-        if constexpr (std::is_same<decltype(SERIES), RootDirectSplit>::value) {
+        if constexpr (std::is_same<decltype(SERIES), RootDirectSplit>::value || std::is_same<decltype(SERIES), const RootQuad*>::value) {
 #pragma unroll
             for (int j = 0; j < 4; ++j) one(r4 + j * ND, SERIES, kExpSplitS1);
         } else {
@@ -1038,10 +1089,40 @@
             for (int j = 0; j < 4; ++j) one(r4 + j * ND, SERIES, scale);
         }
     };
+    RootQuad sq;
+    RootQuadCentre qc;
+    int to_boundary = quad.to_boundary, folds = quad.folds;
+    auto fold_at = [&](RecPtr<double> rb) {
+        RootQuadCentre c;
+        c.c3 = qc.c3;
+#if defined(__HIP_DEVICE_COMPILE__)
+        int column;
+        asm volatile("v_mbcnt_lo_u32_b32 %0, -1, 0\n\tv_mbcnt_hi_u32_b32 %0, -1, %0" : "=v"(column));
+        const volatile __attribute__((address_space(3))) double* park = quad.park + column;
+        c.c1 = park[0];
+        c.c2 = park[quad.stride];
+        c.G0s = park[2 * quad.stride];
+        c.A = park[3 * quad.stride];
+        c.k3 = park[4 * quad.stride];
+#else
+        c.c1 = qc.c1; c.c2 = qc.c2; c.G0s = qc.G0s; c.A = qc.A; c.k3 = qc.k3;
+#endif
+        sq.fold(c, rb[XB + 2], rb[XB + 3], rb[ND + XB + 2]);
+    };
+    auto boundary = [&](RecPtr<double> rb, int step) {
+        if (to_boundary == 0) {
+            to_boundary = 32;
+            MCD_KEEP_BRANCH();
+            if (folds > 0) { --folds; fold_at(rb); }
+        }
+        to_boundary -= step;
+    };
     auto run = [&](auto SERIES) {
+        constexpr bool QUAD = std::is_same<decltype(SERIES), const RootQuad*>::value;
         if constexpr (BOUNDED) {
             int until = rescale_iters;
             for (int g = 0; g < (count >> 3); ++g, r += 8 * ND) {
+                if constexpr (QUAD) boundary(r, 8);
                 RecordPrefetch<8 * ND * 8, PF> pf;
                 pf.issue(r + 8 * ND);
                 four(r, SERIES);
@@ -1051,12 +1132,14 @@
             }
             acc.rescale_narrow();
             if (n4 & 1) {
+                if constexpr (QUAD) boundary(r, 4);
                 four(r, SERIES);
                 r += 4 * ND;
                 acc.rescale_narrow();
             }
         } else if constexpr (NARROW && PF) {
             for (int g = 0; g < (count >> 3); ++g, r += 8 * ND) {
+                if constexpr (QUAD) boundary(r, 8);
                 RecordPrefetch<8 * ND * 8, PF> pf;
                 pf.issue(r + 8 * ND);
                 four(r, SERIES);
@@ -1065,12 +1148,14 @@
                 acc.rescale_narrow();
             }
             if (n4 & 1) {
+                if constexpr (QUAD) boundary(r, 4);
                 four(r, SERIES);
                 r += 4 * ND;
                 acc.rescale_narrow();
             }
         } else if constexpr (NARROW) {
             for (int g = 0; g < n4; ++g, r += 4 * ND) {
+                if constexpr (QUAD) boundary(r, 4);
                 four(r, SERIES);
                 if (g & 1) { MCD_KEEP_BRANCH(); acc.rescale_narrow(); }
             }
@@ -1085,12 +1170,13 @@
             }
         }
         for (int j = n4 * 4; j < count; ++j, r += ND) {
-            one(r, SERIES, std::is_same<decltype(SERIES), RootDirectSplit>::value ? kExpSplitS1 : kScale);
+            if constexpr (QUAD) boundary(r, 1);
+            one(r, SERIES, (std::is_same<decltype(SERIES), RootDirectSplit>::value || QUAD) ? kExpSplitS1 : kScale);
             acc.rescale();
         }
     };
     constexpr bool kCanSeries = NARROW && MODEL == MODEL_BGFIXED && !FREE;
-    bool use_series = false, use_direct = false;
+    bool use_series = false, use_direct = false, use_quad = false;
     const bool split = kCanSeries && r_split != nullptr;
     if constexpr (kCanSeries) {
         if (series && count > 0) {
@@ -1099,10 +1185,31 @@
             const bool ok = vote.setup_chunk(rv[1], rv[(int64_t)(count - 1) * ND + 1], w.s2);
             use_series = wave_all(ok);
             if (use_series && direct) use_direct = wave_all(RootDirect::direct_ok(vote.eb, w.s2));
+            if (use_direct && split && quad.on)
+                use_quad = wave_all(RootQuad::quad_ok(kScale * split_const[1], kScale * vote.eb, s2x));
         }
     }
     if constexpr (kCanSeries) {
-        if (use_direct && split) {
+        if (use_quad) {
+            r = r_split;
+            const double e_first = vgpr_pinned(r[1]), e_last = vgpr_pinned(r[(int64_t)(count - 1) * ND + 1]);
+            qc.setup_quad(0.5 * e_first + 0.5 * e_last, vgpr_pinned((1.0 / kScale) * s2x), kExpSplitC);
+#if defined(__HIP_DEVICE_COMPILE__)
+            {
+                const QuadParkPtr park = quad.park + (int)__builtin_amdgcn_mbcnt_hi(~0u, __builtin_amdgcn_mbcnt_lo(~0u, 0u));
+                park[0] = qc.c1;
+                park[quad.stride] = qc.c2;
+                park[2 * quad.stride] = qc.G0s;
+                park[3 * quad.stride] = qc.A;
+                park[4 * quad.stride] = qc.k3;
+            }
+#endif
+            fold_at(r - (int64_t)quad.back * ND);
+            run((const RootQuad*)&sq);
+            const double result = acc.finish() + *split_const;
+            denormal = acc.denormal();
+            return result;
+        } else if (use_direct && split) {
             r = r_split;
             const double e_first = vgpr_pinned(r[1]), e_last = vgpr_pinned(r[(int64_t)(count - 1) * ND + 1]);
             RootDirectSplit sd;
@@ -1133,7 +1240,8 @@
 template <int MODEL, bool FREE, class T, class A, int FAST, bool PF = false, bool TAB_BIASED = false, bool BOUNDED = false>
 MCD_HD double chunk_loglike(RecPtr<T> r, int count, const WalkerConsts<T>& w, bool& denormal,
                             const double* __restrict__ exptab, int rescale_iters = 1, bool series = false, bool direct = false,
-                            RecPtr<T> r_split = nullptr, const double* __restrict__ split_const = nullptr) {
+                            RecPtr<T> r_split = nullptr, const double* __restrict__ split_const = nullptr,
+                            const QuadArgs& quad = QuadArgs()) {
     constexpr int BG = bg_kind(MODEL);
     denormal = false;
     if constexpr (!FAST) {
@@ -1146,7 +1254,7 @@
         if constexpr (FAST == 2 && MODEL == MODEL_PROFILE && !FREE) return chunk_profile_narrow<PF>(r, count, w);
         else return chunk_const_fast<MODEL, FREE, PF>(r, count, w);
     } else if constexpr (BG == BG_FIXED) {
-        return chunk_bgfixed_fast<MODEL, FREE, FAST, PF, TAB_BIASED, BOUNDED>(r, count, w, denormal, exptab, rescale_iters, series, direct, r_split, split_const);
+        return chunk_bgfixed_fast<MODEL, FREE, FAST, PF, TAB_BIASED, BOUNDED>(r, count, w, denormal, exptab, rescale_iters, series, direct, r_split, split_const, quad);
     } else if constexpr (BG == BG_FIXED_DENSITY) {
         constexpr int ND = record_doubles(MODEL, FREE);
         constexpr int XB = geometry_doubles(MODEL, FREE);
```

Measured after the change: 1778 billion terms/s (median of 6 runs). 3.7% higher.
